# ansonb/RECON

Measured on NVIDIA B200. Metric: SpKBGAT fwd+bwd edges/sec, higher is better.
Workload: dtype f32

## Files before the change

### include/spkbgat.h

```cpp
#ifndef SPKBGAT_H
#define SPKBGAT_H
#include <stdint.h>

#ifdef __cplusplus
extern "C" {
#endif

typedef void* spk_stream_t;

#define SPK_ABI_VERSION 6
int spk_abi_version(void);
const char* spk_last_error(void);
int64_t spk_launch_count(void);

typedef struct {
    int32_t n_heads;
    int32_t d_head;
    int32_t d_pad;
    int32_t width;
} spk_geom;

typedef struct {
    const int32_t* task_seg;
    const int32_t* task_beg;
    const int32_t* task_end;
    const int32_t* hub_seg;
    const int32_t* hub_task_ptr;
    float* partial;
    int64_t ldpart;
    int32_t n_tasks;
    int32_t n_hubs;
    int32_t hub_thresh;
    int32_t reserved;
    const int32_t* task_order;
} spk_hub_tasks;

int spk_edges_concat(const int64_t* edge , int64_t e1, const int64_t* edge_type ,
                     const int64_t* nhop , int64_t e2,
                     int32_t* row, int32_t* col, int32_t* t1, int32_t* t2 ,
                     int64_t n_nodes, int64_t n_rel, int32_t* err_flag, spk_stream_t stream);
int spk_pack_index_host(const int64_t* src, int64_t n, int64_t stride, int64_t lo, int64_t hi, int32_t* dst, int32_t n_threads);
int spk_iota_i32(int32_t* v, int64_t n, spk_stream_t stream);
int64_t spk_sort_workspace_bytes(int64_t n);
int spk_sort_pairs(int32_t* keys, int32_t* vals, int32_t* keys_tmp, int32_t* vals_tmp, int64_t n, int32_t key_bits,
                   void* workspace, int32_t* result_in_tmp, spk_stream_t stream);
int spk_segment_ptr(const int32_t* sorted_keys, int64_t n, int32_t n_seg, int32_t* ptr , spk_stream_t stream);
int spk_gather_i32(const int32_t* src, const int32_t* idx, int64_t n, int32_t* out, spk_stream_t stream);
int spk_rel_incidence(const int32_t* t1, const int32_t* t2, int64_t e, int32_t n_rel, int32_t* keys, int32_t* vals,
                      spk_stream_t stream);

int spk_gemm_nn(const float* A, int64_t lda, const float* B, int64_t ldb, float* C, int64_t ldc,
                int64_t M, int32_t N, int32_t K, int32_t accumulate, spk_stream_t stream);
int64_t spk_gemm_tn_workspace_floats(int64_t M, int32_t Ka, int32_t Nb);
int spk_gemm_tn(const float* A, int64_t lda, const float* B, int64_t ldb, float* C, int64_t ldc,
                int64_t M, int32_t Ka, int32_t Nb, int32_t accumulate, float* workspace, spk_stream_t stream);

int32_t spk_gemm_nn_tc_supported(const float* A, int64_t lda, int64_t M, int32_t N, int32_t K);
int64_t spk_gemm_tc_workspace_floats(int32_t N, int32_t K);
int spk_gemm_nn_tc(const float* A, int64_t lda, const float* B, int64_t ldb, float* C, int64_t ldc,
                   int64_t M, int32_t N, int32_t K, int32_t accumulate, float* workspace, spk_stream_t stream);

int spk_gemm_nn_tc_act(const float* A, int64_t lda, const float* B, int64_t ldb, float* C, int64_t ldc,
                       int64_t M, int32_t N, int32_t K, int32_t accumulate, int32_t act, float* workspace,
                       spk_stream_t stream);
int spk_elu_inplace(float* x, int64_t ldx, int64_t n_rows, int32_t width, spk_stream_t stream);

int32_t spk_gemm_tn_tc_supported(const float* A, int64_t lda, const float* B, int64_t ldb, int64_t M, int32_t Ka, int32_t Nb);
int64_t spk_gemm_tn_tc_workspace_floats(int64_t M, int32_t Ka, int32_t Nb);
int spk_gemm_tn_tc(const float* A, int64_t lda, const float* B, int64_t ldb, float* C, int64_t ldc,
                   int64_t M, int32_t Ka, int32_t Nb, int32_t accumulate, float* workspace, spk_stream_t stream);

typedef struct {
    const int32_t* segptr; const int32_t* col; const int32_t* t1; const int32_t* t2;
    const float* P1; int64_t ld1;
    const float* P2; int64_t ld2;
    const float* P3; int64_t ld3;
    const float* mask; int64_t mask_stride;
    float* out; int64_t ldo;
    float* den; float* sw;
    int32_t* nanflag;
    int32_t n_rows; int32_t apply_elu; float alpha;
    int32_t elu_rows;
    spk_geom geom;
    spk_hub_tasks hub;
} spk_edge_fwd_args;
int spk_edge_attn_fwd(const spk_edge_fwd_args* args, spk_stream_t stream);

typedef struct {
    const int32_t* segptr; const int32_t* col; const int32_t* t1; const int32_t* t2;
    const float* P1; int64_t ld1;
    const float* P2; int64_t ld2;
    const float* P3; int64_t ld3;
    const float* mask; int64_t mask_stride;
    const float* out; const float* dout; int64_t ldo;
    const float* den;
    float* G; int64_t ldg;
    float* dP1; int64_t ldd1;
    float* rec;
    int32_t n_rows; int32_t apply_elu; float alpha; int32_t reserved;
    spk_geom geom;
    spk_hub_tasks hub;
} spk_edge_bwd_rows_args;
int spk_edge_attn_bwd_rows(const spk_edge_bwd_rows_args* args, spk_stream_t stream);

typedef struct {
    const int32_t* segptr; const int32_t* src; const int32_t* pos;
    const float* G; int64_t ldg;
    const float* rec;
    float* out; int64_t ldout;
    int32_t n_seg;
    int32_t flags;
    spk_geom geom;
    spk_hub_tasks hub;
} spk_seg_gather_args;
int spk_edge_attn_bwd_segments(const spk_seg_gather_args* args, spk_stream_t stream);

typedef struct {
    const int32_t* rowptr;
    const int32_t* colptr; const int32_t* csc_row; const int32_t* csc_pos; const int32_t* csc_t1; const int32_t* csc_t2;
    const float* P1; int64_t ld1;
    const float* P2; int64_t ld2;
    const float* P3; int64_t ld3;
    const float* mask; int64_t mask_stride;
    const float* out; const float* dout; int64_t ldo;
    const float* den; const float* sw;
    float* G; int64_t ldg;
    float* rowsc;
    float* dP1; int64_t ldd1;
    float* dP2; int64_t ldd2;
    float* rec;
    int32_t n_rows; int32_t n_cols; int32_t apply_elu; float alpha;
    spk_geom geom;
    spk_hub_tasks row_hub;
    spk_hub_tasks col_hub;
} spk_edge_bwd_fused_args;
int spk_edge_attn_bwd_fused(const spk_edge_bwd_fused_args* args, spk_stream_t stream);

typedef struct {
    spk_edge_bwd_fused_args base;
    const int32_t* relptr; const int32_t* rel_row; const int32_t* rel_pos;
    float* rec4; float* dsv;
    float* dP3; int64_t ldd3;
    int32_t n_rel; int32_t phases;
    spk_hub_tasks rel_hub;
    float* colsum; int64_t ld_colsum;
    float* rowsum; int64_t ld_rowsum;
    const float* G_rel; int64_t ldg_rel;
// ... 152 lines not shown
```

### recon_b200/_lib.py

```python
import ctypes as C
import os

import torch

_HERE = os.path.dirname(os.path.abspath(__file__))
LIB_PATH = os.environ.get("SPK_LIB") or os.path.join(_HERE, "libspkbgat.so")

c_i32p = C.POINTER(C.c_int32)
c_i64p = C.POINTER(C.c_int64)
c_f32p = C.POINTER(C.c_float)
ABI_VERSION = 6


class Geom(C.Structure):
    _fields_ = [("n_heads", C.c_int32), ("d_head", C.c_int32), ("d_pad", C.c_int32), ("width", C.c_int32)]


class HubTasks(C.Structure):
    _fields_ = [("task_seg", C.c_void_p), ("task_beg", C.c_void_p), ("task_end", C.c_void_p),
                ("hub_seg", C.c_void_p), ("hub_task_ptr", C.c_void_p),
                ("partial", C.c_void_p), ("ldpart", C.c_int64),
                ("n_tasks", C.c_int32), ("n_hubs", C.c_int32), ("hub_thresh", C.c_int32), ("reserved", C.c_int32),
                ("task_order", C.c_void_p)]

# ... 59 lines not shown
                ("dup", C.c_int32), ("reserved", C.c_int32)]


class AggGeom(C.Structure):
    _fields_ = [("n_heads", C.c_int32), ("f_chunks", C.c_int32), ("r_chunks", C.c_int32), ("lz", C.c_int32)]


class AggFwdArgs(C.Structure):
    _fields_ = [("segptr", C.c_void_p), ("col", C.c_void_p), ("t1", C.c_void_p), ("t2", C.c_void_p),
                ("xrow", C.c_void_p), ("ldxr", C.c_int64), ("xcol", C.c_void_p), ("ldxc", C.c_int64),
                ("rel", C.c_void_p), ("ldr", C.c_int64),
                ("mask", C.c_void_p), ("mask_stride", C.c_int64),
                ("z", C.c_void_p), ("ldz", C.c_int64), ("den", C.c_void_p), ("sw", C.c_void_p),
                ("nanflag", C.c_void_p),
                ("n_rows", C.c_int32), ("alpha", C.c_float),
                ("geom", AggGeom), ("hub", HubTasks)]


class AggBwdArgs(C.Structure):
    _fields_ = [("segptr", C.c_void_p), ("col", C.c_void_p), ("t1", C.c_void_p), ("t2", C.c_void_p),
                ("xrow", C.c_void_p), ("ldxr", C.c_int64), ("xcol", C.c_void_p), ("ldxc", C.c_int64),
                ("rel", C.c_void_p), ("ldr", C.c_int64),
                ("mask", C.c_void_p), ("mask_stride", C.c_int64),
                ("dz", C.c_void_p), ("ldz", C.c_int64),
                ("den", C.c_void_p), ("sw", C.c_void_p), ("dden", C.c_void_p),
                ("gx", C.c_void_p), ("ldgx", C.c_int64), ("gr", C.c_void_p), ("ldgr", C.c_int64),
                ("rowout", C.c_void_p), ("ldro", C.c_int64), ("rowsc", C.c_void_p), ("rec", C.c_void_p),
                ("n_rows", C.c_int32), ("alpha", C.c_float),
                ("geom", AggGeom), ("hub", HubTasks)]


_VP, _I64, _I32 = C.c_void_p, C.c_int64, C.c_int32

ALLOC_FN = C.CFUNCTYPE(C.c_void_p, C.c_void_p, C.c_int64)


class TripleGraphArgs(C.Structure):
    _fields_ = [("uptr", C.c_void_p), ("ut", C.c_void_p), ("ur0", C.c_void_p), ("ugs", C.c_void_p), ("uge", C.c_void_p),
                ("rs", C.c_void_p), ("n_nodes", C.c_int32), ("n_pairs", C.c_int32), ("n_triples", C.c_int32),
                ("reserved", C.c_int32)]


class NhopResult(C.Structure):
    _fields_ = [("adj_idx", C.c_void_p), ("adj_val", C.c_void_p), ("nhop", C.c_void_p), ("e1", C.c_int64), ("e2", C.c_int64)]


class LossBwdArgs(C.Structure):
    _fields_ = [("segptr", C.c_void_p), ("inc", C.c_void_p), ("coef", C.c_void_p), ("sgn", C.c_void_p),
                ("gscale", C.c_void_p), ("out", C.c_void_p), ("ldo", C.c_int64),
                ("n_seg", C.c_int32), ("width", C.c_int32), ("mode", C.c_int32), ("reserved", C.c_int32),
                ("hub", HubTasks)]


class SgdArgs(C.Structure):
    _fields_ = [("param", C.c_void_p * 16), ("grad", C.c_void_p * 16), ("numel", C.c_int64 * 16),
                ("count", C.c_int32), ("lr", C.c_float)]


class AttnWeightsArgs(C.Structure):
    _fields_ = [("a", C.c_void_p * 4), ("a2", C.c_void_p * 4), ("da", C.c_void_p * 4), ("da2", C.c_void_p * 4),
                ("n_heads", C.c_int32), ("F", C.c_int32), ("Rd", C.c_int32), ("D", C.c_int32),
                ("mode", C.c_int32), ("d_pad", C.c_int32), ("width", C.c_int32),
                ("f_pad", C.c_int32), ("lz", C.c_int32), ("reserved", C.c_int32),
                ("W0", C.c_void_p), ("ld0", C.c_int64), ("W1", C.c_void_p), ("ld1", C.c_int64), ("W2", C.c_void_p)]


SIGNATURES = {
    "spk_abi_version": (_I32, []),
    "spk_last_error": (C.c_char_p, []),
    "spk_launch_count": (_I64, []),
    "spk_edges_concat": (_I32, [_VP, _I64, _VP, _VP, _I64, _VP, _VP, _VP, _VP, _I64, _I64, _VP, _VP]),
    "spk_pack_index_host": (_I32, [_VP, _I64, _I64, _I64, _I64, _VP, _I32]),
    "spk_iota_i32": (_I32, [_VP, _I64, _VP]),
    "spk_sort_workspace_bytes": (_I64, [_I64]),
    "spk_sort_pairs": (_I32, [_VP, _VP, _VP, _VP, _I64, _I32, _VP, C.POINTER(_I32), _VP]),
    "spk_segment_ptr": (_I32, [_VP, _I64, _I32, _VP, _VP]),
    "spk_gather_i32": (_I32, [_VP, _VP, _I64, _VP, _VP]),
    "spk_rel_incidence": (_I32, [_VP, _VP, _I64, _I32, _VP, _VP, _VP]),
    "spk_gemm_nn": (_I32, [_VP, _I64, _VP, _I64, _VP, _I64, _I64, _I32, _I32, _I32, _VP]),
    "spk_gemm_nn_tc_supported": (_I32, [_VP, _I64, _I64, _I32, _I32]),
    "spk_gemm_tc_workspace_floats": (_I64, [_I32, _I32]),
    "spk_gemm_nn_tc": (_I32, [_VP, _I64, _VP, _I64, _VP, _I64, _I64, _I32, _I32, _I32, _VP, _VP]),
    "spk_gemm_nn_tc_act": (_I32, [_VP, _I64, _VP, _I64, _VP, _I64, _I64, _I32, _I32, _I32, _I32, _VP, _VP]),
    "spk_elu_inplace": (_I32, [_VP, _I64, _I64, _I32, _VP]),
    "spk_agg_table": (_I32, [_VP, _I64, _VP, _VP, _I64, _I64, _I32, _I32, _VP]),
    "spk_agg_fwd": (_I32, [C.POINTER(AggFwdArgs), _VP]),
    "spk_agg_bwd_pre": (_I32, [_VP, _VP, _I64, _VP, _I32, _I32, _I32, _VP, _I64, _VP, _I64, _VP]),
    "spk_agg_bwd_rows": (_I32, [C.POINTER(AggBwdArgs), _VP]),
    "spk_agg_bwd_ctx": (_I32, [C.POINTER(AggBwdArgs), _VP]),
    "spk_agg_dx": (_I32, [_VP, _I64, _VP, _I64, _VP, _I64, _I32, _I32, _I32, _VP, _I64, _VP, _VP]),
    "spk_gemm_tn_tc_supported": (_I32, [_VP, _I64, _VP, _I64, _I64, _I32, _I32]),
    "spk_gemm_tn_tc_workspace_floats": (_I64, [_I64, _I32, _I32]),
    "spk_gemm_tn_tc": (_I32, [_VP, _I64, _VP, _I64, _VP, _I64, _I64, _I32, _I32, _I32, _VP, _VP]),
    "spk_gemm_tn_workspace_floats": (_I64, [_I64, _I32, _I32]),
    "spk_gemm_tn": (_I32, [_VP, _I64, _VP, _I64, _VP, _I64, _I64, _I32, _I32, _I32, _VP, _VP]),
    "spk_edge_attn_fwd": (_I32, [C.POINTER(EdgeFwdArgs), _VP]),
    "spk_edge_attn_bwd_rows": (_I32, [C.POINTER(EdgeBwdRowsArgs), _VP]),
    "spk_edge_attn_bwd_segments": (_I32, [C.POINTER(SegGatherArgs), _VP]),
    "spk_edge_attn_bwd_fused": (_I32, [C.POINTER(EdgeBwdFusedArgs), _VP]),
    "spk_edge_attn_bwd_split": (_I32, [C.POINTER(EdgeBwdSplitArgs), _VP]),
    "spk_spmm_rowsum_fwd": (_I32, [_VP, _VP, _VP, _I64, _I32, _VP, _I64, _I32, _VP]),
    "spk_spmm_rowsum_bwd": (_I32, [_VP, _VP, _I64, _I32, _VP, _I64, _I64, _VP]),
    "spk_rownorm": (_I32, [_VP, _I64, _VP, _I64, _I64, _I32, _VP]),
    "spk_residual_norm_fwd": (_I32, [_VP, _I64, _VP, _I64, _VP, _VP, _I64, _VP, _I64, _I32, _VP]),
    "spk_residual_norm_bwd": (_I32, [_VP, _I64, _VP, _I64, _VP, _VP, _VP, _I64, _VP, _I64, _I64, _I32, _VP]),
    "spk_mask_from_index": (_I32, [_VP, _I64, _VP, _I64, _VP, _VP]),
    "spk_attn_weights_fwd": (_I32, [_VP, _VP]),
    "spk_attn_weights_bwd": (_I32, [_VP, _VP]),
    "spk_inner_product_workspace_bytes": (_I64, []),
    "spk_inner_product": (_I32, [_VP, _VP, _I64, _VP, _VP, _I32, _VP]),
    "spk_margin_loss_partials": (_I64, [_I64]),
    "spk_margin_loss_fwd": (_I32, [_VP, _I64, _I64, _VP, _I64, _I64, _VP, _I64, _I64, _I32, C.c_float, _I32,
                                   _VP, _VP, _VP, _VP, _VP, _VP, _VP]),
    "spk_triple_incidence": (_I32, [_VP, _I64, _I64, _I64, _VP, _VP, _VP, _VP, _VP, _VP]),
    "spk_margin_loss_bwd": (_I32, [C.POINTER(LossBwdArgs), _VP]),
    "spk_sgd_step": (_I32, [C.POINTER(SgdArgs), _VP]),
    "spk_triple_keys": (_I32, [_VP, _I64, _I64, _I64, _VP, _VP, _VP]),
    "spk_corrupt_triples": (_I32, [_VP, _I64, _I32, _VP, _I64, _I64, _I64, _VP, _VP, C.c_uint64, _VP, _VP, _VP]),
    "spk_nhop_build": (_I32, [C.POINTER(TripleGraphArgs), _VP, _I64, _I32, ALLOC_FN, _VP, C.POINTER(NhopResult), _VP]),
    "spk_gather_concat": (_I32, [_VP, _VP, _VP, _VP, _VP, _I32, _I64, _I32, _VP, _I64, _VP, _VP]),
    "spk_mlp_head_fwd": (_I32, [_VP, _I64, _VP, _VP, _VP, C.c_float, _I64, _I32, _VP, _VP]),
    "spk_mlp_head_bwd": (_I32, [_VP, _I64, _VP, _VP, C.c_float, _VP, _I64, _I32, _VP, _I64, _VP, _I64, _VP]),
    "spk_tanh_fwd": (_I32, [_VP, _I64, _I64, _I32, _VP]),
    "spk_tanh_bwd": (_I32, [_VP, _I64, _VP, _I64, _I64, _I32, _VP, _I64, _VP]),
    "spk_rank_scores": (_I32, [_VP, _I64, _VP, _I64, _VP, _VP, C.c_float, _I64, _I32, _I32, _VP, _I64, _VP]),
    "spk_linkpred_count": (_I32, [_VP, _I64, _I64, _VP, _I64, _I64, _VP, _VP, C.c_float, _I32, _VP, _VP, _I64, _I32,
                                  _VP, _I64, _VP, _VP, _VP, _VP, _VP]),
    "spk_linkpred_filter": (_I32, [_VP, _I64, _I64, _I64, _VP, C.c_float, _I32, _VP, _I64, _I32, _VP, _I64, _VP, _VP,
                                   _VP, _I64, _VP, _VP, _VP, _VP]),
    "spk_export_json": (_I32, [_VP, _I64, _I64, _I64, C.c_char_p, _I32]),
    "spk_export_bin": (_I32, [_VP, _I64, _I64, _I64, C.c_char_p]),
    "spk_import_json_shape": (_I32, [C.c_char_p, C.POINTER(_I64), C.POINTER(_I64)]),
    "spk_import_json": (_I32, [C.c_char_p, _VP, _I64, _I64, _I64, _I32]),
}

_lib = None
current_tag = ""


class _Lib:

    def __init__(self, cdll):
        self._cdll = cdll
        self.timing = None

    def __getattr__(self, name):
        fn = getattr(self._cdll, name)
        if self.timing is None or SIGNATURES[name][1][-1:] != [_VP] or "workspace" in name or "supported" in name:
            return fn

        def timed(*args):
            e0 = torch.cuda.Event(enable_timing=True)
            e1 = torch.cuda.Event(enable_timing=True)
            e0.record()
            rc = fn(*args)
            e1.record()
            global current_tag
            self.timing.append((name[4:] + (":" + current_tag if current_tag else ""), e0, e1))
            if "gemm" in name:
                current_tag = ""
            return rc
        return timed


def load():
    global _lib
# ... 38 lines not shown
```

### recon_b200/csrc/spk_agg.cu

```cuda
#include <stdlib.h>
#include "spk_agg.cuh"
#include "spk_stream.cuh"

namespace spk {
namespace {

constexpr unsigned FULL = 0xffffffffu;

__device__ __forceinline__ float agg_exp(float x) { return exp2f(x * 1.4426950408889634f); }
__device__ __forceinline__ float4 f4scale(float4 v, float s) { return make_float4(v.x * s, v.y * s, v.z * s, v.w * s); }
__device__ __forceinline__ bool f4nan(float4 v) { return (v.x != v.x) | (v.y != v.y) | (v.z != v.z) | (v.w != v.w); }
__device__ __forceinline__ void st4(float* p, float4 v) { *reinterpret_cast<float4*>(p) = v; }

__global__ void __launch_bounds__(256)
agg_table_kernel(const float* __restrict__ X, long ldx, const float* __restrict__ V, float* __restrict__ T, long ldt,
                 long n, int F, int F4) {
    const int lane = threadIdx.x & 31;
    const long row = (long)blockIdx.x * 8 + (threadIdx.x >> 5);
    if (row >= n) return;
    const float* x = X + row * ldx;
    float xv[2];
    float q[4] = {0.f, 0.f, 0.f, 0.f};
#pragma unroll
    for (int r = 0; r < 2; ++r) {
// ... 768 lines not shown
            for (int u = 0; u < G; ++u) {
                const int n = n0 + u;
                float4 v = make_float4(0.f, 0.f, 0.f, 0.f);
                if (n < T) {
                    const uint32_t slot = wbase + (uint32_t)(grp * G + u) * slot_bytes;
                    if (active) v = lds4(slot + loff);
                    if (HAS2) {
                        const int k2 = __shfl_sync(FULL, cur.t2, n - nb);
                        if (active && !isx && k2 >= 0) v = f4add(v, lds4(slot + loff + rbr));
                    }
                }
#pragma unroll
                for (int h = 0; h < HT; ++h) pd[u * HT + h] = f4dot(Y[h], v);
                if (!TASKS && n + 1 == row_end && rn >= 0) {
#pragma unroll
                    for (int h = 0; h < HT; ++h) Y[h] = Yn[h];
                    r = rn;
                    row_end = __shfl_sync(FULL, st.pre + st.deg, r);
                    rn = -1;
                    if (act) { rn = __ffs(act) - 1; act &= act - 1; load_y(rn, Yn); }
                }
            }
            const float tot = transposed_warp_sum<NV>(pd, lane);
            const bool mine = (lane >> 3) == ((n0 - nb) >> 3);
#pragma unroll
            for (int h = 0; h < HT; ++h) {
                const float t = __shfl_sync(FULL, tot, (((lane & 7) * HT + h) * 32) / NV);
                if (mine) tt[h] = t;
            }
            __syncwarp();
            if (n0 + S < T)
                ags_issue_group<HT, HAS2, G, NG>(a.Xcol, a.ldxc, a.Rt, a.ldr, rbx, rbr, slot_bytes, wbase, bars, T, nb, n0 + S, lane, cur, b1);
        }
        batch_epilogue();
    }
    if (TASKS) {
        const int task = blockIdx.x * AGS_WARPS + wid;
        if (lane == 0) {
            float* part = a.hub.partial + (long)task * a.hub.ldpart;
#pragma unroll
            for (int h = 0; h < 4; ++h) part[h] = h < HT ? usum[h < HT ? h : 0] : 0.f;
        }
    } else if (row_valid) {
        st4(a.rowout + (row0 + lane) * a.ldro + 4 * a.g.Fx4, make_float4(usum[0], HT > 1 ? usum[HT - 1] : 0.f, 0.f, 0.f));
    }
}

__global__ void __launch_bounds__(SPK_CTA_THREADS)
agg_bwd_hub_finalize_kernel(const AggBwdArgs a) {
    __shared__ float red[SPK_WARPS_PER_CTA][8];
    const int hub = blockIdx.x;
    const int row = __ldg(a.hub.hub_seg + hub);
    const int t0 = __ldg(a.hub.hub_task_ptr + hub), t1 = __ldg(a.hub.hub_task_ptr + hub + 1);
    cta_sum_partials<1>(a.hub.partial, a.hub.ldpart, t0, t1, 4, &red[0][0], 8);
    if (threadIdx.x == 0)
        st4(a.rowout + (long)row * a.ldro + 4 * a.g.Fx4, make_float4(red[0][0], red[0][1], 0.f, 0.f));
}

template <int HT, bool HAS2>
int launch_agg_bwd_t(const AggBwdArgs& a, cudaStream_t s) {
    constexpr int G = 8, NG = 2;
    const uint32_t rbx = (uint32_t)(a.g.Fx4 + 1) * 16u, rbr = (uint32_t)(a.g.Fr4 + 1) * 16u;
    const size_t smem = (size_t)AGS_WARPS * ags_warp_bytes_c<HAS2, G, NG>(rbx, rbr);
    static SmemLimit lim_rows, lim_tasks;
    if (a.n_rows > 0) {
        agg_bwd_ctx_kernel<false><<<(a.n_rows + SPK_WARPS_PER_CTA - 1) / SPK_WARPS_PER_CTA, SPK_CTA_THREADS, 0, s>>>(a);
        if (int rc = check_launch("agg_bwd_ctx")) return rc;
        lim_rows.ensure(agg_bwd_stream_kernel<HT, HAS2, false>, smem);
        const unsigned grid = (unsigned)((a.n_rows + 32L * AGS_WARPS - 1) / (32L * AGS_WARPS));
        agg_bwd_stream_kernel<HT, HAS2, false><<<grid, AGS_WARPS * 32, smem, s>>>(a);
        if (int rc = check_launch("agg_bwd_stream_rows")) return rc;
    }
    if (a.hub.n_tasks > 0) {
        lim_tasks.ensure(agg_bwd_stream_kernel<HT, HAS2, true>, smem);
        const unsigned grid = (a.hub.n_tasks + AGS_WARPS - 1) / AGS_WARPS;
        agg_bwd_stream_kernel<HT, HAS2, true><<<grid, AGS_WARPS * 32, smem, s>>>(a);
        if (int rc = check_launch("agg_bwd_stream_tasks")) return rc;
        agg_bwd_hub_finalize_kernel<<<a.hub.n_hubs, SPK_CTA_THREADS, 0, s>>>(a);
        if (int rc = check_launch("agg_bwd_hub_finalize")) return rc;
    }
    return 0;
}

__device__ __forceinline__ void bwd_pre_elem(float ov, float gv, int apply_elu, float& dh, float& p) {
    float hv = ov;
    dh = gv;
    if (apply_elu) {
        const bool pos = ov > 0.f;
        dh = pos ? gv : gv * (ov + 1.f);
        hv = pos ? ov : (ov > -1.f ? fast_log1p(ov) : 0.f);
    }
    p = fmaf(dh, hv, p);
}

__global__ void __launch_bounds__(256)
agg_bwd_pre_vec_kernel(const float* __restrict__ out, const float* __restrict__ dout, long ldo, const float* __restrict__ den,
                       int H, int D4, int apply_elu, float* __restrict__ dhn, long ldd, float* __restrict__ dden, long n) {
    const int lane = threadIdx.x & 31;
    const long row = (long)blockIdx.x * 8 + (threadIdx.x >> 5);
    if (row >= n) return;
    const float* o = out + row * ldo;
    const float* g = dout + row * ldo;
    float* d = dhn + row * ldd;
    const int n4 = H * D4;
    float p[4] = {0.f, 0.f, 0.f, 0.f};
    for (int c4 = lane; c4 < n4; c4 += 32) {
        const float4 ov = ldg4_stream(o + c4 * 4), gv = ldg4_stream(g + c4 * 4);
        float4 dh;
        float acc = 0.f;
        bwd_pre_elem(ov.x, gv.x, apply_elu, dh.x, acc);
        bwd_pre_elem(ov.y, gv.y, apply_elu, dh.y, acc);
        bwd_pre_elem(ov.z, gv.z, apply_elu, dh.z, acc);
        bwd_pre_elem(ov.w, gv.w, apply_elu, dh.w, acc);
        st4(d + c4 * 4, dh);
        const int h = c4 / D4;
#pragma unroll
        for (int k = 0; k < 4; ++k) p[k] += (h == k) ? acc : 0.f;
    }
#pragma unroll
    for (int k = 0; k < 4; ++k) {
        if (k >= H) break;
        const float t = warp_sum(p[k]);
        if (lane == 0) dden[row * H + k] = -t / __ldg(den + row * H + k);
    }
}

__global__ void __launch_bounds__(256)
agg_bwd_pre_kernel(const float* __restrict__ out, const float* __restrict__ dout, long ldo, const float* __restrict__ den,
                   int H, int D, int apply_elu, float* __restrict__ dhn, long ldd, float* __restrict__ dden, long n) {
    const int lane = threadIdx.x & 31;
    const long row = (long)blockIdx.x * 8 + (threadIdx.x >> 5);
    if (row >= n) return;
    const float* o = out + row * ldo;
    const float* g = dout + row * ldo;
    float* d = dhn + row * ldd;
    for (int h = 0; h < H; ++h) {
        float p = 0.f;
        for (int c = lane; c < D; c += 32) {
            float dh;
            bwd_pre_elem(__ldg(o + h * D + c), __ldg(g + h * D + c), apply_elu, dh, p);
            d[h * D + c] = dh;
        }
        p = warp_sum(p);
        if (lane == 0) dden[row * H + h] = -p / __ldg(den + row * H + h);
    }
}

constexpr int DX_R = 2;
__global__ void __launch_bounds__(256)
agg_dx_kernel(const float* __restrict__ rowout, long ldro, const float* __restrict__ dxc, long ldc,
              const float* __restrict__ V, long n, int F, int F4, int H, float* __restrict__ dX, long lddx,
              float* __restrict__ dq) {
    const int lane = threadIdx.x & 31;
    const long i0 = ((long)blockIdx.x * 8 + (threadIdx.x >> 5)) * DX_R;
    float q[DX_R][4], r0[DX_R][2], c0[DX_R][2], c1[DX_R][2];
    float4 v[2];
#pragma unroll
    for (int k = 0; k < 2; ++k) v[k] = (lane + 32 * k < F) ? ldg4(V + (lane + 32 * k) * 4) : make_float4(0.f, 0.f, 0.f, 0.f);
#pragma unroll
    for (int r = 0; r < DX_R; ++r) {
        const long i = i0 + r < n ? i0 + r : n - 1;
        const float* ro = rowout + i * ldro;
        const float* xc = dxc + i * ldc;
        q[r][0] = __ldg(xc + H * 4 * F4); q[r][1] = H > 1 ? __ldg(xc + H * 4 * F4 + 1) : 0.f;
        q[r][2] = __ldg(ro + 4 * F4); q[r][3] = H > 1 ? __ldg(ro + 4 * F4 + 1) : 0.f;
#pragma unroll
        for (int k = 0; k < 2; ++k) {
            const int f = lane + 32 * k;
            r0[r][k] = f < F ? __ldg(ro + f) : 0.f;
            c0[r][k] = f < F ? __ldg(xc + f) : 0.f;
            c1[r][k] = (f < F && H > 1) ? __ldg(xc + 4 * F4 + f) : 0.f;
        }
    }
#pragma unroll
    for (int r = 0; r < DX_R; ++r) {
        const long i = i0 + r;
// ... 85 lines not shown
```

### recon_b200/csrc/spk_api.cu

```cuda
#include "../../include/spkbgat.h"
#include "spk_common.cuh"
#include "spk_edge.cuh"
#include "spk_edge_bwd_fused.cuh"
#include "spk_agg.cuh"
#include "spk_gemm.cuh"
#include "spk_graph.cuh"
#include "spk_rowops.cuh"

namespace spk {

static thread_local char g_err[512] = "";
static unsigned long long g_launches = 0;

void set_error(const char* fmt, ...) {
    va_list ap;
    va_start(ap, fmt);
    vsnprintf(g_err, sizeof(g_err), fmt, ap);
    va_end(ap);
}

int check_launch(const char* what) {
    const cudaError_t e = cudaGetLastError();
    __atomic_fetch_add(&g_launches, 1ULL, __ATOMIC_RELAXED);
    if (e == cudaSuccess) return 0;
// ... 44 lines not shown
        for (int e = beg; e < end; ++e) s += w[(long)perm[e] * ldw + c];
        out[(long)row * ldo + c] = s;
    }
}

__global__ void spmm_rowsum_bwd_kernel(const long long* __restrict__ edge_row, const float* __restrict__ g, long ldg,
                                       int width, float* __restrict__ gw, long ldw, long n_edges) {
    const long i = (long)blockIdx.x * blockDim.x + threadIdx.x;
    if (i >= n_edges * width) return;
    const long e = i / width; const int c = (int)(i % width);
    gw[e * ldw + c] = g[(long)edge_row[e] * ldg + c];
}

}

using namespace spk;

extern "C" {

int spk_abi_version(void) { return SPK_ABI_VERSION; }
const char* spk_last_error(void) { return g_err; }
int64_t spk_launch_count(void) { return (int64_t)__atomic_load_n(&g_launches, __ATOMIC_RELAXED); }

int spk_edges_concat(const int64_t* edge, int64_t e1, const int64_t* edge_type, const int64_t* nhop, int64_t e2,
                     int32_t* row, int32_t* col, int32_t* t1, int32_t* t2, int64_t n_nodes, int64_t n_rel,
                     int32_t* err_flag, spk_stream_t stream) {
    if (e1 + e2 >= (1LL << 31) || n_nodes >= (1LL << 31)) { set_error("edges_concat: sizes exceed int32"); return 1; }
    if (e2 > 0 && !t2) { set_error("edges_concat: t2 required when 2-hop rows are given"); return 1; }
    return edges_concat(reinterpret_cast<const long long*>(edge), e1, reinterpret_cast<const long long*>(edge_type),
                        reinterpret_cast<const long long*>(nhop), e2, row, col, t1, t2, n_nodes, n_rel, err_flag,
                        (cudaStream_t)stream);
}
int spk_iota_i32(int32_t* v, int64_t n, spk_stream_t stream) { return iota_i32(v, n, (cudaStream_t)stream); }
int64_t spk_sort_workspace_bytes(int64_t n) { return radix_sort_workspace_bytes(n); }
int spk_sort_pairs(int32_t* keys, int32_t* vals, int32_t* keys_tmp, int32_t* vals_tmp, int64_t n, int32_t key_bits,
                   void* workspace, int32_t* result_in_tmp, spk_stream_t stream) {
    if (key_bits < 1 || key_bits > 31) { set_error("sort_pairs: key_bits %d out of range", key_bits); return 1; }
    return radix_sort_pairs(keys, vals, keys_tmp, vals_tmp, n, key_bits, workspace, result_in_tmp, (cudaStream_t)stream);
}
int spk_segment_ptr(const int32_t* sorted_keys, int64_t n, int32_t n_seg, int32_t* ptr, spk_stream_t stream) {
    return segment_ptr(sorted_keys, n, n_seg, ptr, (cudaStream_t)stream);
}
int spk_gather_i32(const int32_t* src, const int32_t* idx, int64_t n, int32_t* out, spk_stream_t stream) {
    return gather_i32(src, idx, n, out, (cudaStream_t)stream);
}
int spk_rel_incidence(const int32_t* t1, const int32_t* t2, int64_t e, int32_t n_rel, int32_t* keys, int32_t* vals,
                      spk_stream_t stream) {
    return rel_incidence(t1, t2, e, n_rel, keys, vals, (cudaStream_t)stream);
}

int spk_gemm_nn(const float* A, int64_t lda, const float* B, int64_t ldb, float* C, int64_t ldc,
                int64_t M, int32_t N, int32_t K, int32_t accumulate, spk_stream_t stream) {
    if (lda < K || ldb < N || ldc < N) { set_error("gemm_nn: leading dimension too small"); return 1; }
    return gemm_nn_simt(A, lda, B, ldb, C, ldc, M, N, K, accumulate, (cudaStream_t)stream);
}
int64_t spk_gemm_tn_workspace_floats(int64_t M, int32_t Ka, int32_t Nb) { return gemm_tn_workspace_floats(M, Ka, Nb); }
int spk_gemm_tn(const float* A, int64_t lda, const float* B, int64_t ldb, float* C, int64_t ldc,
                int64_t M, int32_t Ka, int32_t Nb, int32_t accumulate, float* workspace, spk_stream_t stream) {
    if (lda < Ka || ldb < Nb || ldc < Nb) { set_error("gemm_tn: leading dimension too small"); return 1; }
    if (!workspace) { set_error("gemm_tn: workspace required"); return 1; }
    return gemm_tn_simt(A, lda, B, ldb, C, ldc, M, Ka, Nb, accumulate, workspace, (cudaStream_t)stream);
}

int32_t spk_gemm_nn_tc_supported(const float* A, int64_t lda, int64_t M, int32_t N, int32_t K) {
    return gemm_nn_tc_supported(A, lda, M, N, K);
}
int64_t spk_gemm_tc_workspace_floats(int32_t N, int32_t K) { return 2LL * N * gemm_tc_ldt(K); }
int spk_gemm_nn_tc(const float* A, int64_t lda, const float* B, int64_t ldb, float* C, int64_t ldc,
                   int64_t M, int32_t N, int32_t K, int32_t accumulate, float* workspace, spk_stream_t stream) {
    if (lda < K || ldb < N || ldc < N) { set_error("gemm_nn_tc: leading dimension too small"); return 1; }
    if (!gemm_nn_tc_supported(A, lda, M, N, K)) { set_error("gemm_nn_tc: A must be 16-byte aligned with lda %% 4 == 0"); return 1; }
    if (!workspace || (reinterpret_cast<uintptr_t>(workspace) & 15)) { set_error("gemm_nn_tc: aligned workspace required"); return 1; }
    return gemm_nn_tc(A, lda, B, ldb, C, ldc, M, N, K, accumulate, workspace, (cudaStream_t)stream);
}

int spk_gemm_nn_tc_act(const float* A, int64_t lda, const float* B, int64_t ldb, float* C, int64_t ldc,
                       int64_t M, int32_t N, int32_t K, int32_t accumulate, int32_t act, float* workspace, spk_stream_t stream) {
    if (lda < K || ldb < N || ldc < N) { set_error("gemm_nn_tc_act: leading dimension too small"); return 1; }
    if (!gemm_nn_tc_supported(A, lda, M, N, K)) { set_error("gemm_nn_tc_act: A must be 16-byte aligned with lda %% 4 == 0"); return 1; }
    if (!workspace || (reinterpret_cast<uintptr_t>(workspace) & 15)) { set_error("gemm_nn_tc_act: aligned workspace required"); return 1; }
    if (act < 0 || act > 2) { set_error("gemm_nn_tc_act: unknown activation %d", act); return 1; }
    return gemm_nn_tc(A, lda, B, ldb, C, ldc, M, N, K, accumulate, workspace, (cudaStream_t)stream, act);
}
int spk_elu_inplace(float* x, int64_t ldx, int64_t n_rows, int32_t width, spk_stream_t stream) {
    if (ldx < width) { set_error("elu_inplace: leading dimension too small"); return 1; }
    return launch_elu_inplace(x, ldx, n_rows, width, (cudaStream_t)stream);
}

int32_t spk_gemm_tn_tc_supported(const float* A, int64_t lda, const float* B, int64_t ldb, int64_t M, int32_t Ka, int32_t Nb) {
    return gemm_tn_tc_supported(A, lda, B, ldb, M, Ka, Nb);
}
int64_t spk_gemm_tn_tc_workspace_floats(int64_t M, int32_t Ka, int32_t Nb) { return gemm_tn_tc_workspace_floats(M, Ka, Nb); }
int spk_gemm_tn_tc(const float* A, int64_t lda, const float* B, int64_t ldb, float* C, int64_t ldc,
                   int64_t M, int32_t Ka, int32_t Nb, int32_t accumulate, float* workspace, spk_stream_t stream) {
    if (ldc < Nb) { set_error("gemm_tn_tc: leading dimension too small"); return 1; }
    if (!gemm_tn_tc_supported(A, lda, B, ldb, M, Ka, Nb)) { set_error("gemm_tn_tc: operands must be 16-byte aligned with ld %% 4 == 0"); return 1; }
    if (!workspace) { set_error("gemm_tn_tc: workspace required"); return 1; }
    return gemm_tn_tc(A, lda, B, ldb, C, ldc, M, Ka, Nb, accumulate, workspace, (cudaStream_t)stream);
}

int spk_edge_attn_fwd(const spk_edge_fwd_args* p, spk_stream_t stream) {
    EdgeFwdArgs a;
    if (!geom_ok(p->geom, &a.g, "edge_attn_fwd")) return 1;
    if ((p->ld1 & 3) || (p->ld2 & 3) || (p->ld3 & 3) || p->ld1 < p->geom.width || p->ld2 < p->geom.width ||
        p->ld3 < p->geom.width || !aligned16(p->P1) || !aligned16(p->P2) || !aligned16(p->P3)) {
        set_error("edge_attn_fwd: projected tables must be 16-byte aligned with ld >= width, ld %% 4 == 0");
        return 1;
    }
    a.segptr = p->segptr; a.col = p->col; a.t1 = p->t1; a.t2 = p->t2;
    a.P1 = p->P1; a.ld1 = p->ld1; a.P2 = p->P2; a.ld2 = p->ld2; a.P3 = p->P3; a.ld3 = p->ld3;
    a.mask = p->mask; a.mask_stride = p->mask_stride;
    a.out = p->out; a.ldo = p->ldo; a.den = p->den; a.sw = p->sw; a.nanflag = p->nanflag;
    a.n_rows = p->n_rows; a.alpha = p->alpha; a.apply_elu = p->apply_elu;
    a.elu_rows = p->elu_rows > 0 ? p->elu_rows : 0x7fffffff;
    a.out_vec = (p->geom.d_head % 4 == 0) && (p->ldo % 4 == 0) && aligned16(p->out);
    a.hub = hub_of(p->hub);
    if (a.hub.n_tasks > 0 && (a.hub.ldpart < p->geom.width + 2 * SPK_MAX_HEADS || (a.hub.ldpart & 3) || !aligned16(a.hub.partial))) {
        set_error("edge_attn_fwd: hub partial buffer needs ldpart >= width+8, ldpart %% 4 == 0");
        return 1;
    }
    return launch_edge_fwd(a, (cudaStream_t)stream);
}

int spk_edge_attn_bwd_rows(const spk_edge_bwd_rows_args* p, spk_stream_t stream) {
    EdgeBwdRowsArgs a;
    if (!geom_ok(p->geom, &a.g, "edge_attn_bwd_rows")) return 1;
    if ((p->ld1 & 3) || (p->ld2 & 3) || (p->ld3 & 3) || (p->ldg & 3) || (p->ldd1 & 3) || p->ldg < p->geom.n_heads * p->geom.d_pad ||
        p->ldd1 < p->geom.width || !aligned16(p->P1) || !aligned16(p->P2) || !aligned16(p->P3) || !aligned16(p->G) ||
        !aligned16(p->dP1) || (reinterpret_cast<uintptr_t>(p->rec) & 7)) {
        set_error("edge_attn_bwd_rows: bad leading dimension or alignment");
        return 1;
    }
    a.segptr = p->segptr; a.col = p->col; a.t1 = p->t1; a.t2 = p->t2;
    a.P1 = p->P1; a.ld1 = p->ld1; a.P2 = p->P2; a.ld2 = p->ld2; a.P3 = p->P3; a.ld3 = p->ld3;
    a.mask = p->mask; a.mask_stride = p->mask_stride;
    a.out = p->out; a.dout = p->dout; a.ldo = p->ldo; a.den = p->den;
    a.G = p->G; a.ldg = p->ldg; a.dP1 = p->dP1; a.ldd1 = p->ldd1; a.rec = p->rec;
    a.n_rows = p->n_rows; a.alpha = p->alpha; a.apply_elu = p->apply_elu;
    a.out_vec = (p->geom.d_head % 4 == 0) && (p->ldo % 4 == 0) && aligned16(p->out) && aligned16(p->dout);
    a.hub = hub_of(p->hub);
    if (a.hub.n_tasks > 0 && a.hub.ldpart < 2 * SPK_MAX_HEADS) { set_error("edge_attn_bwd_rows: hub ldpart must be >= 8"); return 1; }
    return launch_edge_bwd_rows(a, (cudaStream_t)stream);
}

int spk_edge_attn_bwd_segments(const spk_seg_gather_args* p, spk_stream_t stream) {
    SegGatherArgs a;
    if (!geom_ok(p->geom, &a.g, "edge_attn_bwd_segments")) return 1;
    if ((p->ldg & 3) || (p->ldout & 3) || p->ldout < p->geom.width || p->ldg < p->geom.n_heads * p->geom.d_pad ||
        !aligned16(p->G) || !aligned16(p->out) || (reinterpret_cast<uintptr_t>(p->rec) & 7)) {
        set_error("edge_attn_bwd_segments: bad leading dimension or alignment");
        return 1;
    }
    a.segptr = p->segptr; a.src = p->src; a.pos = p->pos; a.G = p->G; a.ldg = p->ldg; a.rec = p->rec;
    a.outp = p->out; a.ldout = p->ldout; a.n_seg = p->n_seg; a.prefer_stream = p->flags & 1;
    a.hub = hub_of(p->hub);
    if (a.hub.n_tasks > 0 && (a.hub.ldpart < p->geom.width || (a.hub.ldpart & 3) || !aligned16(a.hub.partial))) {
        set_error("edge_attn_bwd_segments: hub partial buffer needs ldpart >= width");
        return 1;
    }
    return launch_seg_gather(a, (cudaStream_t)stream);
}

static int fused_args_of(const spk_edge_bwd_fused_args* p, BwdFusedArgs& a, const char* who, int dup = 0);

int spk_edge_attn_bwd_fused(const spk_edge_bwd_fused_args* p, spk_stream_t stream) {
    BwdFusedArgs a;
// ... 246 lines not shown
```

### recon_b200/csrc/spk_common.cuh

```cuda
#pragma once
#include <cuda_runtime.h>
#include <stdint.h>
#include <stdio.h>
#include <stdarg.h>

#define SPK_MAX_HEADS 4
#define SPK_WARPS_PER_CTA 8
#define SPK_CTA_THREADS (SPK_WARPS_PER_CTA * 32)

namespace spk {

void set_error(const char* fmt, ...);
int check_launch(const char* what);

struct SmemLimit {
    size_t set[64] = {};
    template <class K>
    cudaError_t ensure(K kernel, size_t bytes) {
        int dev = 0;
        const bool keyed = cudaGetDevice(&dev) == cudaSuccess && dev >= 0 && dev < 64;
        if (keyed && set[dev] >= bytes) return cudaSuccess;
        const cudaError_t e = cudaFuncSetAttribute(kernel, cudaFuncAttributeMaxDynamicSharedMemorySize, (int)bytes);
        if (e == cudaSuccess && keyed) set[dev] = bytes;
        return e;
    }
};

__device__ __forceinline__ float warp_sum(float v) {
#pragma unroll
    for (int o = 16; o > 0; o >>= 1) v += __shfl_xor_sync(0xffffffffu, v, o);
    return v;
}

template <int N>
__device__ __forceinline__ float transposed_warp_sum(float (&p)[N], int lane) {
    int off = 16;
#pragma unroll
    for (int n = N; n > 1; n >>= 1, off >>= 1) {
        const bool up = (lane & off) != 0;
        const int half = n >> 1;
#pragma unroll
        for (int k = 0; k < half; ++k) {
            const float keep = up ? p[k + half] : p[k];
            const float send = up ? p[k] : p[k + half];
            p[k] = keep + __shfl_xor_sync(0xffffffffu, send, off);
        }
    }
    float r = p[0];
    for (; off > 0; off >>= 1) r += __shfl_xor_sync(0xffffffffu, r, off);
    return r;
}

__device__ __forceinline__ float fast_log1p(float x) {
    const float u = 1.0f + x;
    const float d = u - 1.0f;
    return d == 0.f ? x : __logf(u) * __fdividef(x, d);
}

__device__ __forceinline__ float4 ldg4(const float* p) {
    return __ldg(reinterpret_cast<const float4*>(p));
}
__device__ __forceinline__ float4 ldg4_stream(const float* p) {
    float4 r;
    asm volatile("ld.global.nc.L1::no_allocate.v4.f32 {%0,%1,%2,%3}, [%4];"
                 : "=f"(r.x), "=f"(r.y), "=f"(r.z), "=f"(r.w) : "l"(p));
    return r;
}
__device__ __forceinline__ float4 f4add(float4 a, float4 b) {
    return make_float4(a.x + b.x, a.y + b.y, a.z + b.z, a.w + b.w);
}
__device__ __forceinline__ void f4fma(float4& acc, float w, float4 v) {
    acc.x = fmaf(w, v.x, acc.x); acc.y = fmaf(w, v.y, acc.y);
    acc.z = fmaf(w, v.z, acc.z); acc.w = fmaf(w, v.w, acc.w);
}
__device__ __forceinline__ float f4dot(float4 a, float4 b) {
    return fmaf(a.x, b.x, fmaf(a.y, b.y, fmaf(a.z, b.z, a.w * b.w)));
}
__device__ __forceinline__ float f4get(const float4& v, int k) {
    return k == 0 ? v.x : (k == 1 ? v.y : (k == 2 ? v.z : v.w));
}
__device__ __forceinline__ float sel4(int h, float a, float b, float c, float d) {
    return h == 0 ? a : (h == 1 ? b : (h == 2 ? c : d));
}

template <int HT>
__device__ __forceinline__ float selh(int h, const float (&v)[HT]) {
    float r = v[0];
#pragma unroll
    for (int i = 1; i < HT; ++i) r = (h == i) ? v[i] : r;
    return r;
}

template <int NREG, int NW = SPK_WARPS_PER_CTA>
__device__ __forceinline__ void cta_sum_partials(const float* __restrict__ part, long ld, int t0, int t1, int len,
                                                 float* red, int red_ld) {
    const int lane = threadIdx.x & 31, wid = threadIdx.x >> 5;
    float acc[NREG];
#pragma unroll
    for (int k = 0; k < NREG; ++k) acc[k] = 0.f;
    int t = t0 + wid;
    for (; t + 3 * NW < t1; t += 4 * NW) {
        float v[4][NREG];
#pragma unroll
        for (int u = 0; u < 4; ++u)
#pragma unroll
            for (int k = 0; k < NREG; ++k) {
                const int c = lane + 32 * k;
                v[u][k] = c < len ? part[(long)(t + u * NW) * ld + c] : 0.f;
            }
#pragma unroll
        for (int u = 0; u < 4; ++u)
#pragma unroll
            for (int k = 0; k < NREG; ++k) acc[k] += v[u][k];
    }
    for (; t < t1; t += NW) {
#pragma unroll
        for (int k = 0; k < NREG; ++k) {
            const int c = lane + 32 * k;
            if (c < len) acc[k] += part[(long)t * ld + c];
        }
    }
#pragma unroll
    for (int k = 0; k < NREG; ++k) {
        const int c = lane + 32 * k;
        if (c < len) red[wid * red_ld + c] = acc[k];
    }
    __syncthreads();
    for (int c = threadIdx.x; c < len; c += (NW * 32)) {
        float s = 0.f;
#pragma unroll
        for (int w = 0; w < NW; ++w) s += red[w * red_ld + c];
        red[c] = s;
    }
    __syncthreads();
}

struct LayerGeom {
    int H;
    int D;
// ... 7 lines not shown
```

### recon_b200/csrc/spk_gemm.cuh

```cuda
#pragma once
#include <cuda_runtime.h>

namespace spk {
int gemm_nn_simt(const float* A, long lda, const float* B, long ldb, float* C, long ldc,
                 long M, int N, int K, int accumulate, cudaStream_t s);
int gemm_tn_splits(long M, int Ka, int Nb);
long gemm_tn_workspace_floats(long M, int Ka, int Nb);
int gemm_tn_simt(const float* A, long lda, const float* B, long ldb, float* C, long ldc,
                 long M, int Ka, int Nb, int accumulate, float* workspace, cudaStream_t s);
}

namespace spk {
int gemm_tc_ldt(int K);
int gemm_nn_tc_supported(const float* A, long lda, long M, int N, int K);
int gemm_nn_tc(const float* A, long lda, const float* B, long ldb, float* C, long ldc, long M, int N, int K,
               int accumulate, float* workspace, cudaStream_t s, int act = 0);
int gemm_tn_tc_supported(const float* A, long lda, const float* B, long ldb, long M, int Ka, int Nb);
long gemm_tn_tc_workspace_floats(long M, int Ka, int Nb);
int gemm_tn_tc(const float* A, long lda, const float* B, long ldb, float* C, long ldc, long M, int Ka, int Nb,
               int accumulate, float* workspace, cudaStream_t s);
}
```

### recon_b200/csrc/spk_gemm_tc.cu

```cuda
#include <cuda.h>
#include <stdlib.h>
#include "spk_common.cuh"
#include "spk_gemm.cuh"

namespace spk {
namespace {

constexpr int TC_BM = 128;
constexpr int TC_BK = 32;
constexpr int TC_A_TILE = TC_BM * TC_BK * 4;
constexpr int TC_THREADS = 320;
constexpr int TC_MAX_STAGES = 4;

__device__ __forceinline__ uint32_t smem_u32(const void* p) { return (uint32_t)__cvta_generic_to_shared(p); }

__device__ __forceinline__ void mbar_init(uint32_t bar, uint32_t count) {
    asm volatile("mbarrier.init.shared::cta.b64 [%0], %1;" ::"r"(bar), "r"(count) : "memory");
}
__device__ __forceinline__ void mbar_arrive(uint32_t bar) {
    asm volatile("mbarrier.arrive.shared::cta.b64 _, [%0];" ::"r"(bar) : "memory");
}
__device__ __forceinline__ void mbar_arrive_expect_tx(uint32_t bar, uint32_t bytes) {
    asm volatile("mbarrier.arrive.expect_tx.shared::cta.b64 _, [%0], %1;" ::"r"(bar), "r"(bytes) : "memory");
}
__device__ __forceinline__ void mbar_wait(uint32_t bar, uint32_t parity) {
    asm volatile(
        "{\n\t"
        ".reg .pred P1;\n\t"
        "LAB_WAIT:\n\t"
        "mbarrier.try_wait.parity.shared::cta.b64 P1, [%0], %1;\n\t"
        "@P1 bra DONE;\n\t"
        "bra LAB_WAIT;\n\t"
        "DONE:\n\t"
        "}" ::"r"(bar), "r"(parity) : "memory");
}
__device__ __forceinline__ void tma_load_2d(uint32_t dst, const CUtensorMap* tm, uint32_t bar, int c0, int c1) {
    asm volatile(
        "cp.async.bulk.tensor.2d.shared::cluster.global.mbarrier::complete_tx::bytes [%0], [%1, {%3, %4}], [%2];"
        ::"r"(dst), "l"(tm), "r"(bar), "r"(c0), "r"(c1) : "memory");
}
__device__ __forceinline__ void tma_load_2d_mc(uint32_t dst, const CUtensorMap* tm, uint32_t bar, int c0, int c1, uint16_t mask) {
    asm volatile(
        "cp.async.bulk.tensor.2d.shared::cluster.global.mbarrier::complete_tx::bytes.multicast::cluster [%0], [%1, {%3, %4}], [%2], %5;"
        ::"r"(dst), "l"(tm), "r"(bar), "r"(c0), "r"(c1), "h"(mask) : "memory");
}
__device__ __forceinline__ uint32_t cluster_ctarank() {
    uint32_t r;
    asm volatile("mov.u32 %0, %%cluster_ctarank;" : "=r"(r));
    return r;
}
__device__ __forceinline__ void cluster_sync_all() {
    asm volatile("barrier.cluster.arrive.release.aligned;" ::: "memory");
    asm volatile("barrier.cluster.wait.acquire.aligned;" ::: "memory");
}
__device__ __forceinline__ void tc_fence_before() { asm volatile("tcgen05.fence::before_thread_sync;" ::: "memory"); }
__device__ __forceinline__ void tc_fence_after() { asm volatile("tcgen05.fence::after_thread_sync;" ::: "memory"); }
__device__ __forceinline__ void tc_commit(uint32_t bar) {
    asm volatile("tcgen05.commit.cta_group::1.mbarrier::arrive::one.shared::cluster.b64 [%0];" ::"r"(bar) : "memory");
}
__device__ __forceinline__ void tc_commit_mc(uint32_t bar, uint16_t mask) {
    asm volatile("tcgen05.commit.cta_group::1.mbarrier::arrive::one.shared::cluster.multicast::cluster.b64 [%0], %1;"
                 ::"r"(bar), "h"(mask) : "memory");
}
__device__ __forceinline__ void tc_mma_tf32(uint32_t d_tmem, uint64_t adesc, uint64_t bdesc, uint32_t idesc, uint32_t accum) {
    asm volatile(
        "{\n\t"
        ".reg .pred p;\n\t"
        "setp.ne.b32 p, %4, 0;\n\t"
        "tcgen05.mma.cta_group::1.kind::tf32 [%0], %1, %2, %3, p;\n\t"
        "}" ::"r"(d_tmem), "l"(adesc), "l"(bdesc), "r"(idesc), "r"(accum) : "memory");
}
__device__ __forceinline__ uint64_t make_kmajor_sw128_desc(uint32_t saddr) {
    const uint32_t lo = ((saddr >> 4) & 0x3fffu) | (1u << 16);
    const uint32_t hi = (1024u >> 4) | (1u << 14) | (2u << 29);
    return ((uint64_t)hi << 32) | lo;
}

struct TcParams {
    float* C; long ldc; long M; int N; int K; int BN; int n_tiles_n; int stages; int accumulate; int c_vec;
    int act;
    int c_tma;
    int raw_hi;
    int cs;
};

__device__ __forceinline__ float tc_elu(float x) {
    const float big = exp2f(x * 1.4426950408889634f) - 1.0f;
    const float small = x * (1.0f + x * (0.5f + x * (0.16666667f + x * (0.041666668f + x * 0.0083333338f))));
    const float neg = x > -0.125f ? small : big;
    return x > 0.f ? x : neg;
}

__device__ __forceinline__ float tc_act(float x, int act) { return act == 2 ? tanhf(x) : tc_elu(x); }

__global__ void __launch_bounds__(TC_THREADS, 1)
gemm_nn_tc_kernel(const __grid_constant__ CUtensorMap tmA, const __grid_constant__ CUtensorMap tmBhi,
                  const __grid_constant__ CUtensorMap tmBlo, const __grid_constant__ CUtensorMap tmC, const TcParams p) {
    extern __shared__ uint8_t smem_raw[];
    __shared__ __align__(8) uint64_t bars[3 * TC_MAX_STAGES + 4];
    __shared__ uint32_t tmem_slot;

    const int warp = threadIdx.x >> 5, lane = threadIdx.x & 31;
    const uint32_t base = (smem_u32(smem_raw) + 1023u) & ~1023u;
    const uint32_t b_tile = (uint32_t)p.BN * 128u;
    const uint32_t stage_bytes = 2u * TC_A_TILE + 2u * b_tile;
    auto a_hi = [&](int s) { return base + (uint32_t)s * stage_bytes; };
    auto a_lo = [&](int s) { return base + (uint32_t)s * stage_bytes + TC_A_TILE; };
    auto b_hi = [&](int s) { return base + (uint32_t)s * stage_bytes + 2u * TC_A_TILE; };
    auto b_lo = [&](int s) { return base + (uint32_t)s * stage_bytes + 2u * TC_A_TILE + b_tile; };
    const uint32_t bar0 = smem_u32(bars);
    auto full = [&](int s) { return bar0 + 8u * s; };
    auto conv = [&](int s) { return bar0 + 8u * (TC_MAX_STAGES + s); };
    auto empty = [&](int s) { return bar0 + 8u * (2 * TC_MAX_STAGES + s); };
    auto tfull = [&](int a) { return bar0 + 8u * (3 * TC_MAX_STAGES + a); };
    auto tempty = [&](int a) { return bar0 + 8u * (3 * TC_MAX_STAGES + 2 + a); };

    const int num_kb = (p.K + TC_BK - 1) / TC_BK;
    const long m_tiles = (p.M + TC_BM - 1) / TC_BM;
    const int cs = p.cs;
    const uint32_t crank = cs > 1 ? cluster_ctarank() : 0u;
    const uint16_t cmask = (uint16_t)((1u << cs) - 1u);
    const long total = ((m_tiles + cs - 1) / cs) * p.n_tiles_n;
    const long first = blockIdx.x / cs, stride = gridDim.x / cs;
    const uint32_t b_slice = b_tile / (uint32_t)cs;
    const int b_rows = p.BN / cs;

    if (threadIdx.x == 0) {
        asm volatile("prefetch.tensormap [%0];" ::"l"(&tmA) : "memory");
        asm volatile("prefetch.tensormap [%0];" ::"l"(&tmBhi) : "memory");
        asm volatile("prefetch.tensormap [%0];" ::"l"(&tmBlo) : "memory");
        for (int s = 0; s < TC_MAX_STAGES; ++s) { mbar_init(full(s), 1); mbar_init(conv(s), 128); mbar_init(empty(s), (uint32_t)cs); }
        for (int a = 0; a < 2; ++a) { mbar_init(tfull(a), 1); mbar_init(tempty(a), 4); }
        asm volatile("fence.mbarrier_init.release.cluster;" ::: "memory");
    }
    if (warp == 1) {
        asm volatile("tcgen05.alloc.cta_group::1.sync.aligned.shared::cta.b32 [%0], %1;" ::"r"(smem_u32(&tmem_slot)), "r"(512u) : "memory");
        asm volatile("tcgen05.relinquish_alloc_permit.cta_group::1.sync.aligned;" ::: "memory");
    }
    tc_fence_before();
    __syncthreads();
    if (cs > 1) cluster_sync_all();
    tc_fence_after();
    const uint32_t tmem_base = tmem_slot;

    if (warp == 0) {
        if (lane == 0) {
            uint32_t it = 0;
            for (long tile = first; tile < total; tile += stride) {
                const int m0 = (int)((tile / p.n_tiles_n) * cs + crank) * TC_BM, n0 = (int)(tile % p.n_tiles_n) * p.BN;
                for (int kb = 0; kb < num_kb; ++kb, ++it) {
                    const int s = it % p.stages;
                    const uint32_t ph = (it / p.stages) & 1u;
                    mbar_wait(empty(s), ph ^ 1u);
                    mbar_arrive_expect_tx(full(s), TC_A_TILE + 2u * b_tile);
                    tma_load_2d(a_hi(s), &tmA, full(s), kb * TC_BK, m0);
                    if (cs == 1) {
                        tma_load_2d(b_hi(s), &tmBhi, full(s), kb * TC_BK, n0);
                        tma_load_2d(b_lo(s), &tmBlo, full(s), kb * TC_BK, n0);
                    } else {
                        tma_load_2d_mc(b_hi(s) + crank * b_slice, &tmBhi, full(s), kb * TC_BK, n0 + (int)crank * b_rows, cmask);
                        tma_load_2d_mc(b_lo(s) + crank * b_slice, &tmBlo, full(s), kb * TC_BK, n0 + (int)crank * b_rows, cmask);
                    }
                }
            }
        }
    } else if (warp == 1) {
        if (lane == 0) {
            const uint32_t idesc = (1u << 4) | (2u << 7) | (2u << 10) | ((uint32_t)(p.BN >> 3) << 17) | ((uint32_t)(TC_BM >> 4) << 24);
            uint32_t it = 0, tl = 0;
            for (long tile = first; tile < total; tile += stride, ++tl) {
                const uint32_t acc = tl & 1u, aph = (tl >> 1) & 1u;
                mbar_wait(tempty(acc), aph ^ 1u);
                tc_fence_after();
                const uint32_t d_tmem = tmem_base + acc * 256u;
                for (int kb = 0; kb < num_kb; ++kb, ++it) {
                    const int s = it % p.stages;
                    const uint32_t ph = (it / p.stages) & 1u;
                    mbar_wait(full(s), ph);
                    mbar_wait(conv(s), ph);
                    tc_fence_after();
                    const uint64_t dah = make_kmajor_sw128_desc(a_hi(s)), dal = make_kmajor_sw128_desc(a_lo(s));
                    const uint64_t dbh = make_kmajor_sw128_desc(b_hi(s)), dbl = make_kmajor_sw128_desc(b_lo(s));
#pragma unroll
                    for (int ks = 0; ks < TC_BK / 8; ++ks) {
                        if (kb * TC_BK + ks * 8 >= p.K) break;
                        const uint64_t o = (uint64_t)(2 * ks);
                        tc_mma_tf32(d_tmem, dal + o, dbh + o, idesc, (kb | ks) != 0);
                        tc_mma_tf32(d_tmem, dah + o, dbl + o, idesc, 1u);
                        tc_mma_tf32(d_tmem, dah + o, dbh + o, idesc, 1u);
                    }
                    if (cs == 1) tc_commit(empty(s));
                    else tc_commit_mc(empty(s), cmask);
                }
                tc_commit(tfull(acc));
            }
        }
    } else if (warp < 6) {
        const int t = threadIdx.x - 64;
        uint32_t it = 0;
        for (long tile = first; tile < total; tile += stride) {
            for (int kb = 0; kb < num_kb; ++kb, ++it) {
                const int s = it % p.stages;
                const uint32_t ph = (it / p.stages) & 1u;
                mbar_wait(full(s), ph);
                const uint32_t hi0 = a_hi(s), lo0 = a_lo(s);
#pragma unroll
                for (int i = 0; i < TC_A_TILE / 16 / 128; ++i) {
                    const uint32_t off = (uint32_t)(t + 128 * i) * 16u;
                    float4 x;
                    asm volatile("ld.shared.v4.f32 {%0,%1,%2,%3}, [%4];" : "=f"(x.x), "=f"(x.y), "=f"(x.z), "=f"(x.w) : "r"(hi0 + off));
                    float4 h, l;
                    h.x = __uint_as_float(__float_as_uint(x.x) & 0xffffe000u); l.x = x.x - h.x;
                    h.y = __uint_as_float(__float_as_uint(x.y) & 0xffffe000u); l.y = x.y - h.y;
                    h.z = __uint_as_float(__float_as_uint(x.z) & 0xffffe000u); l.z = x.z - h.z;
                    h.w = __uint_as_float(__float_as_uint(x.w) & 0xffffe000u); l.w = x.w - h.w;
                    if (!p.raw_hi)
                        asm volatile("st.shared.v4.f32 [%0], {%1,%2,%3,%4};" ::"r"(hi0 + off), "f"(h.x), "f"(h.y), "f"(h.z), "f"(h.w) : "memory");
                    asm volatile("st.shared.v4.f32 [%0], {%1,%2,%3,%4};" ::"r"(lo0 + off), "f"(l.x), "f"(l.y), "f"(l.z), "f"(l.w) : "memory");
                }
                asm volatile("fence.proxy.async.shared::cta;" ::: "memory");
                mbar_arrive(conv(s));
            }
        }
    } else if (p.c_tma) {
        const int q = warp & 3;
        const uint32_t stg0 = base + (uint32_t)p.stages * stage_bytes + (uint32_t)q * 8192u;
        uint32_t tl = 0, sb = 0;
        for (long tile = first; tile < total; tile += stride, ++tl) {
            const uint32_t acc = tl & 1u, aph = (tl >> 1) & 1u;
            const int row0 = (int)((tile / p.n_tiles_n) * cs + crank) * TC_BM + q * 32;
            const int n0 = (int)(tile % p.n_tiles_n) * p.BN;
            mbar_wait(tfull(acc), aph);
            tc_fence_after();
            for (int c0 = 0; c0 < p.BN && row0 < p.M; c0 += 32) {
                if (n0 + c0 >= p.N) break;
                uint32_t r[32];
                const uint32_t taddr = tmem_base + acc * 256u + (uint32_t)c0 + ((uint32_t)(q * 32) << 16);
                asm volatile(
                    "tcgen05.ld.sync.aligned.32x32b.x32.b32 {%0,%1,%2,%3,%4,%5,%6,%7,%8,%9,%10,%11,%12,%13,%14,%15,"
                    "%16,%17,%18,%19,%20,%21,%22,%23,%24,%25,%26,%27,%28,%29,%30,%31}, [%32];"
                    : "=r"(r[0]), "=r"(r[1]), "=r"(r[2]), "=r"(r[3]), "=r"(r[4]), "=r"(r[5]), "=r"(r[6]), "=r"(r[7]),
                      "=r"(r[8]), "=r"(r[9]), "=r"(r[10]), "=r"(r[11]), "=r"(r[12]), "=r"(r[13]), "=r"(r[14]), "=r"(r[15]),
                      "=r"(r[16]), "=r"(r[17]), "=r"(r[18]), "=r"(r[19]), "=r"(r[20]), "=r"(r[21]), "=r"(r[22]), "=r"(r[23]),
                      "=r"(r[24]), "=r"(r[25]), "=r"(r[26]), "=r"(r[27]), "=r"(r[28]), "=r"(r[29]), "=r"(r[30]), "=r"(r[31])
                    : "r"(taddr));
                asm volatile("tcgen05.wait::ld.sync.aligned;" ::: "memory");
                if (p.act == 2) {
#pragma unroll
                    for (int j = 0; j < 32; ++j) r[j] = __float_as_uint(tanhf(__uint_as_float(r[j])));
                } else if (p.act) {
#pragma unroll
                    for (int j = 0; j < 32; ++j) r[j] = __float_as_uint(tc_elu(__uint_as_float(r[j])));
                }
                if (lane == 0) asm volatile("cp.async.bulk.wait_group.read 1;" ::: "memory");
                __syncwarp();
                const uint32_t stg = stg0 + sb * 4096u;
                const uint32_t rowaddr = stg + (uint32_t)lane * 128u;
#pragma unroll
                for (int j = 0; j < 8; ++j) {
                    const uint32_t a = rowaddr + (uint32_t)((j ^ (lane & 7)) << 4);
                    asm volatile("st.shared.v4.b32 [%0], {%1,%2,%3,%4};" ::"r"(a), "r"(r[4 * j]), "r"(r[4 * j + 1]),
                                 "r"(r[4 * j + 2]), "r"(r[4 * j + 3]) : "memory");
                }
                asm volatile("fence.proxy.async.shared::cta;" ::: "memory");
                __syncwarp();
                if (lane == 0 && row0 < p.M) {
                    if (p.accumulate)
                        asm volatile("cp.reduce.async.bulk.tensor.2d.global.shared::cta.add.tile.bulk_group [%0, {%1, %2}], [%3];"
                                     ::"l"(&tmC), "r"(n0 + c0), "r"(row0), "r"(stg) : "memory");
                    else
                        asm volatile("cp.async.bulk.tensor.2d.global.shared::cta.tile.bulk_group [%0, {%1, %2}], [%3];"
                                     ::"l"(&tmC), "r"(n0 + c0), "r"(row0), "r"(stg) : "memory");
                    asm volatile("cp.async.bulk.commit_group;" ::: "memory");
                }
                sb ^= 1u;
            }
            tc_fence_before();
            __syncwarp();
            if (lane == 0) mbar_arrive(tempty(acc));
        }
        if (lane == 0) asm volatile("cp.async.bulk.wait_group 0;" ::: "memory");
    } else {
        const int q = warp & 3;
        uint32_t tl = 0;
        for (long tile = first; tile < total; tile += stride, ++tl) {
            const uint32_t acc = tl & 1u, aph = (tl >> 1) & 1u;
            const long row = ((tile / p.n_tiles_n) * cs + crank) * TC_BM + q * 32 + lane;
            const int n0 = (int)(tile % p.n_tiles_n) * p.BN;
            mbar_wait(tfull(acc), aph);
            tc_fence_after();
            for (int c0 = 0; c0 < p.BN; c0 += 16) {
                uint32_t r[16];
                const uint32_t taddr = tmem_base + acc * 256u + (uint32_t)c0 + ((uint32_t)(q * 32) << 16);
                asm volatile(
                    "tcgen05.ld.sync.aligned.32x32b.x16.b32 {%0,%1,%2,%3,%4,%5,%6,%7,%8,%9,%10,%11,%12,%13,%14,%15}, [%16];"
                    : "=r"(r[0]), "=r"(r[1]), "=r"(r[2]), "=r"(r[3]), "=r"(r[4]), "=r"(r[5]), "=r"(r[6]), "=r"(r[7]),
                      "=r"(r[8]), "=r"(r[9]), "=r"(r[10]), "=r"(r[11]), "=r"(r[12]), "=r"(r[13]), "=r"(r[14]), "=r"(r[15])
                    : "r"(taddr));
                asm volatile("tcgen05.wait::ld.sync.aligned;" ::: "memory");
                if (row < p.M) {
                    float* crow = p.C + row * p.ldc;
#pragma unroll
                    for (int j = 0; j < 16; j += 4) {
                        const int col = n0 + c0 + j;
                        if (col >= p.N) break;
                        float4 o = make_float4(__uint_as_float(r[j]), __uint_as_float(r[j + 1]), __uint_as_float(r[j + 2]), __uint_as_float(r[j + 3]));
// ... 232 lines not shown
                    asm volatile("cp.async.bulk.commit_group;" ::: "memory");
                }
                sb ^= 1u;
            }
            tc_fence_before();
            __syncwarp();
            if (lane == 0) mbar_arrive_remote(tempty(acc), 0u);
        }
        if (lane == 0) asm volatile("cp.async.bulk.wait_group 0;" ::: "memory");
    }
    tc_fence_before();
    __syncthreads();
    cluster_sync_all();
    if (warp == 1) {
        tc_fence_after();
        asm volatile("tcgen05.dealloc.cta_group::2.sync.aligned.b32 %0, %1;" ::"r"(tmem_base), "r"(512u) : "memory");
    }
}

__global__ void tc_prepare_b_kernel(const float* __restrict__ B, long ldb, int K, int N, float* __restrict__ hi,
                                    float* __restrict__ lo, int ldt) {
    const long i = (long)blockIdx.x * blockDim.x + threadIdx.x;
    if (i >= (long)N * ldt) return;
    const int n = (int)(i / ldt), k = (int)(i % ldt);
    const float x = k < K ? B[(long)k * ldb + n] : 0.f;
    const float h = __uint_as_float(__float_as_uint(x) & 0xffffe000u);
    hi[i] = h;
    lo[i] = x - h;
}

typedef CUresult (*EncodeTiledFn)(CUtensorMap*, CUtensorMapDataType, cuuint32_t, void*, const cuuint64_t*, const cuuint64_t*,
                                  const cuuint32_t*, const cuuint32_t*, CUtensorMapInterleave, CUtensorMapSwizzle,
                                  CUtensorMapL2promotion, CUtensorMapFloatOOBfill);

EncodeTiledFn encode_fn() {
    static EncodeTiledFn fn = nullptr;
    if (!fn) {
        void* p = nullptr;
        cudaDriverEntryPointQueryResult q;
        if (cudaGetDriverEntryPoint("cuTensorMapEncodeTiled", &p, cudaEnableDefault, &q) == cudaSuccess && q == cudaDriverEntryPointSuccess)
            fn = reinterpret_cast<EncodeTiledFn>(p);
    }
    return fn;
}

int make_map(CUtensorMap* tm, const float* ptr, long rows, long cols, long ld, int box_rows,
             CUtensorMapSwizzle swz = CU_TENSOR_MAP_SWIZZLE_128B) {
    EncodeTiledFn fn = encode_fn();
    if (!fn) { set_error("gemm_tc: cuTensorMapEncodeTiled unavailable"); return 3; }
    cuuint64_t dims[2] = {(cuuint64_t)cols, (cuuint64_t)rows};
    cuuint64_t strides[1] = {(cuuint64_t)ld * 4};
    cuuint32_t box[2] = {(cuuint32_t)TC_BK, (cuuint32_t)box_rows};
    cuuint32_t estr[2] = {1, 1};
    const CUresult r = fn(tm, CU_TENSOR_MAP_DATA_TYPE_FLOAT32, 2, const_cast<float*>(ptr), dims, strides, box, estr,
                          CU_TENSOR_MAP_INTERLEAVE_NONE, swz, CU_TENSOR_MAP_L2_PROMOTION_L2_128B,
                          CU_TENSOR_MAP_FLOAT_OOB_FILL_NONE);
    if (r != CUDA_SUCCESS) { set_error("gemm_tc: cuTensorMapEncodeTiled failed (%d)", (int)r); return 3; }
    return 0;
}
}

int gemm_tc_ldt(int K) { return (K + 3) / 4 * 4; }

static int tc_cluster() {
    const char* e = getenv("SPK_TC_CLUSTER");
    return (e && e[0] == '2') ? 2 : 1;
}

static int tc_pair() {
    const char* e = getenv("SPK_TC_PAIR");
    return (e && e[0] == '1') ? 1 : 0;
}

static int tc_raw_hi() {
    static int v = -1;
    if (v < 0) { const char* e = getenv("SPK_TC_RAW_HI"); v = (e && e[0] == '0') ? 0 : 1; }
    return v;
}

int gemm_nn_tc_supported(const float* A, long lda, long M, int N, int K) {
    return M >= 1 && N >= 1 && K >= 1 && (lda % 4 == 0) && ((reinterpret_cast<uintptr_t>(A) & 15) == 0) && lda >= K;
}

int gemm_nn_tc(const float* A, long lda, const float* B, long ldb, float* C, long ldc, long M, int N, int K,
               int accumulate, float* workspace, cudaStream_t s, int act) {
    const int ldt = gemm_tc_ldt(K);
    float* bhi = workspace;
    float* blo = workspace + (long)N * ldt;
    const long nb = (long)N * ldt;
    tc_prepare_b_kernel<<<(unsigned)((nb + 255) / 256), 256, 0, s>>>(B, ldb, K, N, bhi, blo, ldt);
    if (int rc = check_launch("tc_prepare_b")) return rc;

    const int n_tiles_n = (N + 255) / 256;
    const int bn_round = n_tiles_n > 1 ? 32 : 16;
    int BN = ((N + n_tiles_n - 1) / n_tiles_n + bn_round - 1) / bn_round * bn_round;
    if (BN < 16) BN = 16;
    const int b_tile = BN * 128;
    const int stage_bytes = 2 * TC_A_TILE + 2 * b_tile;
    const int c_vec = (ldc % 4 == 0) && ((reinterpret_cast<uintptr_t>(C) & 15) == 0);
    const int c_tma = c_vec && !(act && accumulate);
    const int staging = c_tma ? 4 * 8192 : 0;
    int stages = (225 * 1024 - 1024 - staging) / stage_bytes;
    if (stages > TC_MAX_STAGES) stages = TC_MAX_STAGES;
    if (stages < 1) { set_error("gemm_tc: tile does not fit shared memory"); return 3; }
    const int smem = stages * stage_bytes + staging + 1024;

    int dev = 0, sms = 148;
    cudaGetDevice(&dev);
    cudaDeviceGetAttribute(&sms, cudaDevAttrMultiProcessorCount, dev);
    const long m_tiles = (M + TC_BM - 1) / TC_BM;
    const bool pair = tc_pair() && c_tma && tc_raw_hi() && (BN % 16 == 0) && m_tiles * n_tiles_n >= 2L * sms;
    if (pair) {
        const int half_tile = BN / 2 * 128;
        const int stage2 = 2 * TC_A_TILE + 2 * half_tile;
        int stages2 = (225 * 1024 - 1024 - staging) / stage2;
        if (stages2 > TC_MAX_STAGES) stages2 = TC_MAX_STAGES;
        const int smem2 = stages2 * stage2 + staging + 1024;
        CUtensorMap tA, tBh, tBl, tC;
        if (int rc = make_map(&tA, A, M, K, lda, TC_BM)) return rc;
        if (int rc = make_map(&tBh, bhi, N, K, ldt, BN / 2)) return rc;
        if (int rc = make_map(&tBl, blo, N, K, ldt, BN / 2)) return rc;
        if (int rc = make_map(&tC, C, M, N, ldc, 32)) return rc;
        TcParams q;
        q.C = C; q.ldc = ldc; q.M = M; q.N = N; q.K = K; q.BN = BN; q.n_tiles_n = n_tiles_n; q.stages = stages2;
        q.accumulate = accumulate; q.act = act; q.c_vec = c_vec; q.c_tma = 1; q.raw_hi = 1; q.cs = 2;
        static SmemLimit lim2;
        if (lim2.ensure(gemm_nn_tc2_kernel, 226 * 1024) != cudaSuccess) {
            set_error("gemm_tc: cannot raise dynamic shared memory limit");
            (void)cudaGetLastError();
            return 3;
        }
        cudaLaunchConfig_t cfg = {};
        cfg.gridDim = dim3((unsigned)sms / 2 * 2); cfg.blockDim = dim3(TC_THREADS); cfg.dynamicSmemBytes = (size_t)smem2; cfg.stream = s;
        cudaLaunchAttribute attr[1];
        attr[0].id = cudaLaunchAttributeClusterDimension;
        attr[0].val.clusterDim.x = 2; attr[0].val.clusterDim.y = 1; attr[0].val.clusterDim.z = 1;
        cfg.attrs = attr; cfg.numAttrs = 1;
        static int pairs_resident[64] = {};
        int nc = (dev >= 0 && dev < 64) ? pairs_resident[dev] : 0;
        if (nc == 0) {
            if (cudaOccupancyMaxActiveClusters(&nc, gemm_nn_tc2_kernel, &cfg) != cudaSuccess || nc < 1) { (void)cudaGetLastError(); nc = sms / 4; }
            if (dev >= 0 && dev < 64) pairs_resident[dev] = nc;
        }
        const long pair_tiles = ((m_tiles + 1) / 2) * n_tiles_n;
        const long np = pair_tiles < nc ? pair_tiles : nc;
        cfg.gridDim = dim3((unsigned)(2 * np));
        (void)cudaLaunchKernelEx(&cfg, gemm_nn_tc2_kernel, tA, tBh, tBl, tC, q);
        return check_launch("gemm_nn_tc2");
    }
    const int cs = (tc_cluster() == 2 && !accumulate && m_tiles * n_tiles_n >= 2L * sms) ? 2 : 1;

    CUtensorMap tmA, tmBhi, tmBlo, tmC;
    if (int rc = make_map(&tmA, A, M, K, lda, TC_BM)) return rc;
    if (int rc = make_map(&tmBhi, bhi, N, K, ldt, BN / cs)) return rc;
    if (int rc = make_map(&tmBlo, blo, N, K, ldt, BN / cs)) return rc;
    if (c_tma) { if (int rc = make_map(&tmC, C, M, N, ldc, 32)) return rc; }
    else tmC = tmA;

    TcParams p;
    p.C = C; p.ldc = ldc; p.M = M; p.N = N; p.K = K; p.BN = BN; p.n_tiles_n = n_tiles_n; p.stages = stages;
    p.accumulate = accumulate; p.act = act;
    p.c_vec = c_vec; p.c_tma = c_tma; p.raw_hi = tc_raw_hi(); p.cs = cs;
    static SmemLimit lim;
    if (lim.ensure(gemm_nn_tc_kernel, 226 * 1024) != cudaSuccess) {
        set_error("gemm_tc: cannot raise dynamic shared memory limit");
        (void)cudaGetLastError();
        return 3;
    }
    const long total = ((m_tiles + cs - 1) / cs) * n_tiles_n * cs;
    cudaLaunchConfig_t cfg = {};
    cfg.gridDim = dim3((unsigned)sms / cs * cs); cfg.blockDim = dim3(TC_THREADS); cfg.dynamicSmemBytes = (size_t)smem; cfg.stream = s;
    cudaLaunchAttribute attr[1];
    attr[0].id = cudaLaunchAttributeClusterDimension;
    attr[0].val.clusterDim.x = (unsigned)cs; attr[0].val.clusterDim.y = 1; attr[0].val.clusterDim.z = 1;
    cfg.attrs = attr; cfg.numAttrs = 1;
    long resident = sms;
    if (cs > 1) {
        static int clusters[64] = {};
        int nc = (dev >= 0 && dev < 64) ? clusters[dev] : 0;
        if (nc == 0) {
            if (cudaOccupancyMaxActiveClusters(&nc, gemm_nn_tc_kernel, &cfg) != cudaSuccess || nc < 1) { (void)cudaGetLastError(); nc = sms / cs / 2; }
            if (dev >= 0 && dev < 64) clusters[dev] = nc;
        }
        resident = (long)nc * cs;
    }
    unsigned grid = (unsigned)(total < resident ? total : resident);
    grid = grid / cs * cs;
    if (grid < (unsigned)cs) grid = (unsigned)cs;
    cfg.gridDim = dim3(grid);
    (void)cudaLaunchKernelEx(&cfg, gemm_nn_tc_kernel, tmA, tmBhi, tmBlo, tmC, p);
    return check_launch("gemm_nn_tc");
}


namespace {

constexpr int TN_BKM = 32;
constexpr int TN_CHUNK = TN_BKM * 128;
constexpr int TN_ACH = 4;

__device__ __forceinline__ uint64_t make_mnmajor_sw128_desc(uint32_t saddr) {
    const uint32_t lo = ((saddr >> 4) & 0x3fffu) | ((uint32_t)(TN_CHUNK >> 4) << 16);
    const uint32_t hi = (512u >> 4) | (1u << 14) | (1u << 29);
    return ((uint64_t)hi << 32) | lo;
}

struct TnParams {
    float* part; long M; int Ka; int Nb; int BN; int n_tiles_n; int n_tiles_k; int splits; long m_per_split; int stages;
    int raw_hi;
};

constexpr int TN_LO_SLOTS = 2;
constexpr int TN_SPLIT_WARPS = 8;
constexpr int TN_THREADS = (2 + TN_SPLIT_WARPS + 4) * 32;

__global__ void __launch_bounds__(TN_THREADS, 1)
gemm_tn_tc_kernel(const __grid_constant__ CUtensorMap tmX, const __grid_constant__ CUtensorMap tmG, const TnParams p) {
    extern __shared__ uint8_t smem_raw[];
    __shared__ __align__(8) uint64_t bars[2 * TC_MAX_STAGES + 2 * TN_LO_SLOTS + 1];
    __shared__ uint32_t tmem_slot;

    const int warp = threadIdx.x >> 5, lane = threadIdx.x & 31;
    const uint32_t base = (smem_u32(smem_raw) + 1023u) & ~1023u;
    const int nbc = p.BN / 32;
    const uint32_t half = (uint32_t)(TN_ACH + nbc) * TN_CHUNK;
    const uint32_t b_off = TN_ACH * TN_CHUNK;
    auto raw = [&](int s) { return base + (uint32_t)s * half; };
    auto lo = [&](int l) { return base + (uint32_t)(p.stages + l) * half; };
    const uint32_t bar0 = smem_u32(bars);
    auto full = [&](int s) { return bar0 + 8u * s; };
    auto rawfree = [&](int s) { return bar0 + 8u * (TC_MAX_STAGES + s); };
    auto conv = [&](int l) { return bar0 + 8u * (2 * TC_MAX_STAGES + l); };
    auto lofree = [&](int l) { return bar0 + 8u * (2 * TC_MAX_STAGES + TN_LO_SLOTS + l); };
    const uint32_t tfull = bar0 + 8u * (2 * TC_MAX_STAGES + 2 * TN_LO_SLOTS);

    const int tile = blockIdx.x % (p.n_tiles_k * p.n_tiles_n);
    const int split = blockIdx.x / (p.n_tiles_k * p.n_tiles_n);
    const int ka0 = (tile / p.n_tiles_n) * 128, nb0 = (tile % p.n_tiles_n) * p.BN;
    const long mbeg = (long)split * p.m_per_split;
    long mend = mbeg + p.m_per_split;
    if (mend > p.M) mend = p.M;
    const int num_kb = mend > mbeg ? (int)((mend - mbeg + TN_BKM - 1) / TN_BKM) : 0;

    if (threadIdx.x == 0) {
        asm volatile("prefetch.tensormap [%0];" ::"l"(&tmX) : "memory");
        asm volatile("prefetch.tensormap [%0];" ::"l"(&tmG) : "memory");
        for (int s = 0; s < TC_MAX_STAGES; ++s) { mbar_init(full(s), 1); mbar_init(rawfree(s), 1); }
        for (int l = 0; l < TN_LO_SLOTS; ++l) { mbar_init(conv(l), TN_SPLIT_WARPS * 32); mbar_init(lofree(l), 1); }
        mbar_init(tfull, 1);
        asm volatile("fence.mbarrier_init.release.cluster;" ::: "memory");
    }
    if (warp == 1) {
        asm volatile("tcgen05.alloc.cta_group::1.sync.aligned.shared::cta.b32 [%0], %1;" ::"r"(smem_u32(&tmem_slot)), "r"(256u) : "memory");
        asm volatile("tcgen05.relinquish_alloc_permit.cta_group::1.sync.aligned;" ::: "memory");
    }
    tc_fence_before();
    __syncthreads();
    tc_fence_after();
    const uint32_t tmem_base = tmem_slot;

    if (warp == 0) {
        if (lane == 0) {
            for (int kb = 0; kb < num_kb; ++kb) {
                const int s = kb % p.stages;
                const uint32_t ph = (kb / p.stages) & 1u;
                mbar_wait(rawfree(s), ph ^ 1u);
                mbar_arrive_expect_tx(full(s), half);
                const int m0 = (int)(mbeg + (long)kb * TN_BKM);
                for (int c = 0; c < TN_ACH; ++c) tma_load_2d(raw(s) + c * TN_CHUNK, &tmX, full(s), ka0 + 32 * c, m0);
                for (int c = 0; c < nbc; ++c) tma_load_2d(raw(s) + b_off + c * TN_CHUNK, &tmG, full(s), nb0 + 32 * c, m0);
            }
        }
    } else if (warp == 1) {
        if (lane == 0) {
// ... 165 lines not shown
```

### recon_b200/functional.py

```python
import ctypes as C
import os
import weakref

import torch

from . import _lib
from .graph import KGraph

MAX_HEADS = 4
USE_TC = True
TC_MIN_ROWS = 1


WD_ALIGN = int(os.environ.get("SPK_WD_ALIGN", "8"))


class Geometry:

    def __init__(self, n_heads, d_head):
        assert 1 <= n_heads <= MAX_HEADS
        self.H, self.D = n_heads, d_head
        self.Dp = (d_head + 3) // 4 * 4
        self.Dt = self.H * self.Dp
        self.Wd = (self.Dt + self.H + WD_ALIGN - 1) // WD_ALIGN * WD_ALIGN
# ... 360 lines not shown
    d = den[n:]
    d0 = torch.where(sw[n:] == 0, torch.zeros_like(d), d)
    buf = torch.cat(((v * d0.unsqueeze(-1)).reshape(ng, H * W), d0), dim=1)
    ghost.sum_partials(buf)
    dg = buf[:, H * W:]
    dg = torch.where(dg == 0, torch.full_like(dg, 1e-12), dg)
    vals[n:] = (buf[:, :H * W].view(ng, H, W) / dg.unsqueeze(-1)).reshape(ng, H * W)
    den[n:] = dg


def _ghost_dout(ghost, dout, n, n_ext):
    ext = torch.empty(n_ext, dout.shape[1], dtype=dout.dtype, device=dout.device)
    ext[:n] = dout
    ext[n:] = ghost.gather_rows(dout)
    ext[ghost.mine_local] = 0
    return ext


class AttentionGroupFn(torch.autograd.Function):

    @staticmethod
    def forward(ctx, X, Wn, Rel, Wr, graph, geom, alpha, apply_elu, mask_csr, nanflag):
        X = tc_friendly(X.contiguous()); Wn = Wn.contiguous(); Rel = Rel.contiguous(); Wr = Wr.contiguous()
        dist = getattr(graph, "dist", None)
        ghost = dist.ghost if dist is not None else None
        Wd = geom.Wd
        mode = "local"
        X_all = None
        if dist is None:
            P3 = gemm_nn(Rel, Wr)
            P = gemm_nn(X, Wn)
            P1, P2 = P[:, :Wd], P[:, Wd:]
        elif 2 * X.shape[1] <= Wd:
            mode = "input"
            Fp = (X.shape[1] + 3) // 4 * 4
            X_all, mine = dist.gather_buffer(Fp, X.device)
            mine[:, :X.shape[1]].copy_(X)
            if Fp != X.shape[1]:
                mine[:, X.shape[1]:].zero_()
            h = dist.all_gather_start(X_all)
            P3 = gemm_nn(Rel, Wr)
            P1 = gemm_nn(X, Wn[:, :Wd])
            h.wait()
            X_all = X_all[:, :X.shape[1]]
            P2 = gemm_nn(X_all, Wn[:, Wd:])
        else:
            mode = "proj"
            P2, mine = dist.gather_buffer(Wd, X.device)
            gemm_nn(X, Wn[:, Wd:], out=mine)
            h = dist.all_gather_start(P2)
            n = X.shape[0]
            if ghost is None:
                P1 = gemm_nn(X, Wn[:, :Wd])
            else:
                P1 = torch.empty(n + ghost.n, Wd, dtype=torch.float32, device=X.device)
                gemm_nn(X, Wn[:, :Wd], out=P1[:n])
                gemm_nn(tc_friendly(ghost.gather_rows(X)), Wn[:, :Wd], out=P1[n:])
            P3 = gemm_nn(Rel, Wr)
            h.wait()
        if ghost is not None and mode != "proj":
            raise NotImplementedError("hub rows split across ranks need the projected exchange (or the aggregate-then-project path)")
        if ghost is None:
            out, den, sw = edge_attn_forward(graph, P1, P2, P3, geom, alpha, apply_elu, mask_csr, nanflag)
            out_ret = out
        else:
            n = X.shape[0]
            k_elu = bool(apply_elu) and n > 0
            out, den, sw = edge_attn_forward(graph, P1, P2, P3, geom, alpha, k_elu, mask_csr, nanflag, elu_rows=n if k_elu else 0)
            _ghost_combine(ghost, out, den, sw, n, geom.H)
            nanflag.bitwise_or_(torch.isnan(out[n:]).any().to(torch.int32))
            if apply_elu and out.shape[0] > n:
                tail = out[n:]
                _lib.check(_lib.load().spk_elu_inplace(_lib.ptr(tail), tail.stride(0), tail.shape[0], tail.shape[1],
                                                       _lib.stream_ptr()), "elu_inplace")
            out[ghost.mine_local] = out[n:][ghost.mine]
            out_ret = out[:n]
        ctx.save_for_backward(X, Wn, Rel, Wr, P1, P2, P3, out, den, sw, X_all if X_all is not None else X.new_empty(0))
        ctx.graph, ctx.geom, ctx.alpha, ctx.apply_elu, ctx.mask_csr, ctx.mode = graph, geom, alpha, apply_elu, mask_csr, mode
        ctx.mark_non_differentiable(den, sw)
        return out_ret, den, sw

    @staticmethod
    def backward(ctx, dout, _dden, _dsw):
        geom, graph, mode = ctx.geom, ctx.graph, ctx.mode
        dist = getattr(graph, "dist", None)
        X, Wn, Rel, Wr, P1, P2, P3, out, den, sw, X_all = ctx.saved_tensors
        Wd = geom.Wd
        dout = dout.contiguous()
        n = X.shape[0]
        dev = X.device
        dP3 = torch.empty_like(P3)
        WnT = Wn.t().contiguous()
        need_x, need_w = ctx.needs_input_grad[0], ctx.needs_input_grad[1]
        dX = dWn = None
        if mode == "local":
            dP = torch.empty(n, 2 * Wd, dtype=torch.float32, device=dev)
            edge_attn_backward(graph, P1, P2, P3, geom, ctx.alpha, ctx.apply_elu, ctx.mask_csr, out, dout, den, sw,
                               dP[:, :Wd], dP[:, Wd:], dP3)
            if need_x:
                dX = gemm_nn(dP, WnT)
            if need_w:
                dWn = gemm_tn(X, dP)
        else:
            mr = dist.part.max_rows
            ghost = dist.ghost
            n_ext = n + (ghost.n if ghost is not None else 0)
            if ghost is not None:
                dout = _ghost_dout(ghost, dout, n, n_ext)
            dP1 = torch.empty(n_ext, Wd, dtype=torch.float32, device=dev)
            dP2_all = torch.empty_like(P2)
            colsum = torch.empty(P2.shape[0], geom.H, dtype=torch.float32, device=dev)
            pend = {}

            def start_main():
                if mode == "proj":
                    pend["pad"] = torch.empty(mr, Wd, dtype=torch.float32, device=dev)
                    pend["h"] = dist.reduce_scatter_start(dP2_all, pend["pad"])

            split = edge_attn_backward(graph, P1, P2, P3, geom, ctx.alpha, ctx.apply_elu, ctx.mask_csr, out, dout, den, sw,
                                       dP1, dP2_all, dP3, after_columns=start_main if mode == "proj" else None, colsum=colsum)
            if mode == "proj":
                if split:
                    qs_pad = torch.empty(mr, geom.H, dtype=torch.float32, device=dev)
                    hq = dist.reduce_scatter_start(colsum, qs_pad)
                else:
                    start_main()
                h3 = dist.all_reduce_start(dP3)
                if ghost is not None:
                    gsum = ghost.sum_partials(dP1[n:].contiguous())
                    dP1[ghost.mine_local] = gsum[ghost.mine]
                    dP1 = dP1[:n]
                if need_x:
                    dX = gemm_nn(dP1, WnT[:Wd])
                if need_w:
                    dWn = torch.empty_like(Wn)
                    gemm_tn(X, dP1, out=dWn[:, :Wd])
                pend["h"].wait()
                dP2 = pend["pad"][:n]
                if split:
                    hq.wait()
                    dP2[:, geom.Dt:geom.Dt + geom.H].copy_(qs_pad[:n])
                del dP2_all
                if need_x:
                    gemm_nn(dP2, WnT[Wd:], out=dX, accumulate=True)
                if need_w:
                    gemm_tn(X, dP2, out=dWn[:, Wd:])
                    dist.all_reduce(dWn)
                h3.wait()
            else:
                h3 = dist.all_reduce_start(dP3)
                F = X.shape[1]
                Fp = (F + 3) // 4 * 4
                if need_x:
                    dX2_all = torch.empty(P2.shape[0], Fp, dtype=torch.float32, device=dev)
                    gemm_nn(dP2_all, WnT[Wd:], out=dX2_all[:, :F])
                    if Fp != F:
                        dX2_all[:, F:].zero_()
                    pad = torch.empty(mr, Fp, dtype=torch.float32, device=dev)
                    h = dist.reduce_scatter_start(dX2_all, pad)
                    dX1 = gemm_nn(dP1, WnT[:Wd])
                    h.wait()
                    dX = dX1.add_(pad[:n, :F])
                    del dX2_all
                if need_w:
                    dWn = torch.empty_like(Wn)
                    gemm_tn(X, dP1, out=dWn[:, :Wd])
                    gemm_tn(X_all, dP2_all, out=dWn[:, Wd:])
                    dist.all_reduce(dWn)
                h3.wait()
        dRel = gemm_nn(dP3, Wr.t().contiguous()) if ctx.needs_input_grad[2] else None
        dWr = gemm_tn(Rel, dP3) if ctx.needs_input_grad[3] else None
        return dX, dWn, dRel, dWr, None, None, None, None, None, None



AGG_MODE = "auto"
AGG_BWD_MODE = os.environ.get("SPK_AGG_BWD_MODE", "split")
AGG_MAX_HEADS = 2


G_ALIGN = int(os.environ.get("SPK_G_ALIGN", "8"))
GX_ALIGN = int(os.environ.get("SPK_GX_ALIGN", "8"))
LX_ALIGN = int(os.environ.get("SPK_LX_ALIGN", "8"))


def _row_stride(width, align):
    return (width + align - 1) // align * align


class AggGeometry:

    def __init__(self, n_heads, in_features, nrela_dim, d_head):
        self.H, self.F, self.Rd, self.D = n_heads, in_features, nrela_dim, d_head
        self.Fx4, self.Fr4 = (in_features + 3) // 4, (nrela_dim + 3) // 4
        self.Fp, self.Rp = 4 * self.Fx4, 4 * self.Fr4
        self.LX = _row_stride(self.Fp + 4, LX_ALIGN)
        self.LR = _row_stride(self.Rp + 4, LX_ALIGN)
        self.LZ = 2 * self.Fp + self.Rp

    @staticmethod
    def supported(n_heads, in_features, nrela_dim):
        return 1 <= n_heads <= AGG_MAX_HEADS and 1 <= in_features <= 60 and 1 <= nrela_dim <= 60

    def struct(self):
        return _lib.AggGeom(self.H, self.Fx4, self.Fr4, self.LZ)


def use_agg_path(n_heads, in_features, nrela_dim, d_head, graph):
    if AGG_MODE == "off" or (getattr(graph, "dist", None) is None and graph.n_cols != graph.n_nodes):
        return False
    if not AggGeometry.supported(n_heads, in_features, nrela_dim):
        return False
    if AGG_MODE == "force":
        return True
    g = AggGeometry(n_heads, in_features, nrela_dim, d_head)
    return g.LX + g.LR < n_heads * d_head


def agg_weights(a_list, a2_list, geom):
    if _on_library(list(a_list) + list(a2_list)):
        dims = dict(F=geom.F, Rd=geom.Rd, D=geom.D, Fp=geom.Fp, LZ=geom.LZ)
        return AttnWeightsFn.apply(1, dims, *a_list, *a2_list)
    return _agg_weights_torch(a_list, a2_list, geom)


def _agg_weights_torch(a_list, a2_list, geom):
    F, Rd, Fp = geom.F, geom.Rd, geom.Fp
    a0 = a_list[0]
    Wa = a0.new_zeros(geom.H, geom.LZ, geom.D)
    V = a0.new_zeros(F, 4)
    V3 = a0.new_zeros(Rd, 4)
    for h, (a, a2) in enumerate(zip(a_list, a2_list)):
        at = a.t()
        qa = (at * a2).sum(dim=1)
        Wa[h, :F] = at[:F]
        Wa[h, Fp:Fp + F] = at[F:2 * F]
        Wa[h, 2 * Fp:2 * Fp + Rd] = at[2 * F:]
        V[:, 2 + h] = qa[:F]
        V[:, h] = qa[F:2 * F]
        V3[:, h] = qa[2 * F:]
    return Wa, V, V3


def _agg_table(X, V, ld, chunks, out=None):
    T = torch.empty(X.shape[0], ld, dtype=torch.float32, device=X.device) if out is None else out
    assert T.shape[0] == X.shape[0] and T.stride(1) == 1 and T.stride(0) >= ld
    ld = T.stride(0)
    if X.shape[0]:
        _lib.check(_lib.load().spk_agg_table(_lib.ptr(X), X.stride(0), _lib.ptr(V), _lib.ptr(T), ld, X.shape[0],
                                             X.shape[1], chunks, _lib.stream_ptr()), "agg_table")
    return T


class AggGroupFn(torch.autograd.Function):

    @staticmethod
    def forward(ctx, X, Rel, Wa, V, V3, graph, geom, alpha, apply_elu, mask_csr, nanflag):
        lib = _lib.load()
        X = X.contiguous(); Rel = Rel.contiguous(); Wa = Wa.contiguous(); V = V.contiguous(); V3 = V3.contiguous()
        n, dev = graph.n_nodes, X.device
        n_loc = X.shape[0]
        H, D, LZ = geom.H, geom.D, geom.LZ
        dist = getattr(graph, "dist", None)
        ghost = dist.ghost if dist is not None else None
        if dist is None:
            Xt = _agg_table(X, V, geom.LX, geom.Fx4)
            Xc = Xt
            Rt = _agg_table(Rel, V3, geom.LR, geom.Fr4)
            _X_TABLE["key"], _X_TABLE["table"] = _x_key(X), weakref.ref(Xt)
        else:
            Xc, Xt = dist.gather_buffer(geom.LX, dev)
            _agg_table(X, V, geom.LX, geom.Fx4, out=Xt)
            hx = dist.all_gather_start(Xc)
            Rt = _agg_table(Rel, V3, geom.LR, geom.Fr4)
            hx.wait()
            if ghost is not None:
                lo = dist.rank * dist.part.max_rows
                Xc[lo + n_loc:lo + n] = Xc[ghost.padded_ids]
                Xt = Xc[lo:lo + n]
        Z = torch.empty(n, H * LZ, dtype=torch.float32, device=dev)
        den = torch.empty(n, H, dtype=torch.float32, device=dev)
        sw = torch.empty(n, H, dtype=torch.float32, device=dev)
        a = _lib.AggFwdArgs()
        a.segptr = graph.rowptr.data_ptr(); a.col = graph.col.data_ptr(); a.t1 = graph.t1.data_ptr()
        a.t2 = graph.t2.data_ptr() if graph.t2 is not None else None
        a.xrow = Xt.data_ptr(); a.ldxr = Xt.stride(0); a.xcol = Xc.data_ptr(); a.ldxc = Xc.stride(0)
        a.rel = Rt.data_ptr(); a.ldr = Rt.stride(0)
        if mask_csr is not None:
            a.mask = mask_csr.data_ptr(); a.mask_stride = mask_csr.stride(0)
        a.z = Z.data_ptr(); a.ldz = Z.stride(0); a.den = den.data_ptr(); a.sw = sw.data_ptr()
        a.nanflag = nanflag.data_ptr(); a.n_rows = n; a.alpha = float(alpha); a.geom = geom.struct()
        partial = _hub_partial(graph.row_hubs, 264, dev)
        graph.row_hubs.fill(a.hub, partial, 264)
        _lib.check(lib.spk_agg_fwd(C.byref(a), _lib.stream_ptr()), "agg_fwd")
        if ghost is not None:
            _ghost_combine(ghost, Z, den, sw, n_loc, H)
        out = torch.empty(n, H * D, dtype=torch.float32, device=dev)
        for h in range(H):
            gemm_nn(Z[:, h * LZ:(h + 1) * LZ], Wa[h], out=out[:, h * D:(h + 1) * D], act=int(apply_elu))
        if ghost is not None:
            nanflag.bitwise_or_(torch.isnan(out[n_loc:]).any().to(torch.int32))
            out[ghost.mine_local] = out[n_loc:][ghost.mine]
        ctx.save_for_backward(X, Rel, Wa, V, V3, Xt, Rt, Z, out, den, sw, Xc)
        ctx.graph, ctx.geom, ctx.alpha, ctx.apply_elu, ctx.mask_csr = graph, geom, alpha, apply_elu, mask_csr
        return out[:n_loc] if ghost is not None else out

    @staticmethod
    def backward(ctx, dout):
        lib = _lib.load()
        geom, graph = ctx.geom, ctx.graph
        X, Rel, Wa, V, V3, Xt, Rt, Z, out, den, sw, Xc = ctx.saved_tensors
        dist = getattr(graph, "dist", None)
        graph.build_backward()
        n, dev = graph.n_nodes, X.device
        n_loc = X.shape[0]
        ghost = dist.ghost if dist is not None else None
        H, D, LZ, Fp, Rp = geom.H, geom.D, geom.LZ, geom.Fp, geom.Rp
        f32 = dict(dtype=torch.float32, device=dev)
        dout = dout.contiguous()
        if ghost is not None:
            dout = _ghost_dout(ghost, dout, n_loc, n)
        dhn = torch.empty(n, H * D, **f32)
        dden = torch.empty(n, H, **f32)
        _lib.check(lib.spk_agg_bwd_pre(_lib.ptr(out), _lib.ptr(dout), out.stride(0), _lib.ptr(den), H, D,
                                       int(ctx.apply_elu), _lib.ptr(dhn), dhn.stride(0), _lib.ptr(dden), n,
                                       _lib.stream_ptr()), "agg_bwd_pre")
        dZ = torch.empty(n, H * LZ, **f32)
        dWa = torch.empty_like(Wa)
        for h in range(H):
            dh = dhn[:, h * D:(h + 1) * D]
            gemm_nn(dh, Wa[h].t().contiguous(), out=dZ[:, h * LZ:(h + 1) * LZ])
            if ghost is None:
                gemm_tn(Z[:, h * LZ:(h + 1) * LZ], dh, out=dWa[h])
            else:
                gemm_tn(Z[:n_loc, h * LZ:(h + 1) * LZ], dh[:n_loc], out=dWa[h])
                gemm_tn((Z[n_loc:, h * LZ:(h + 1) * LZ] * ghost.mine.unsqueeze(1)).contiguous(), dh[n_loc:], out=dWa[h],
                        accumulate=True)
        Gx = torch.empty(n, _row_stride(H * Fp, GX_ALIGN), **f32)[:, :H * Fp]
        Gr = torch.empty(n, _row_stride(H * Rp, GX_ALIGN), **f32)[:, :H * Rp]
        rowout = torch.empty(n, Fp + 4, **f32)
        a = _lib.AggBwdArgs()
        a.xrow = Xt.data_ptr(); a.ldxr = Xt.stride(0)
        a.dz = dZ.data_ptr(); a.ldz = dZ.stride(0)
        a.den = den.data_ptr(); a.sw = sw.data_ptr(); a.dden = dden.data_ptr()
        a.gx = Gx.data_ptr(); a.ldgx = Gx.stride(0); a.gr = Gr.data_ptr(); a.ldgr = Gr.stride(0)
        a.rowout = rowout.data_ptr(); a.ldro = rowout.stride(0)
        a.n_rows = n; a.alpha = float(ctx.alpha); a.geom = geom.struct()
        gx_geom, gr_geom = Geometry(H, Fp), Geometry(H, Rp)
        dXc = torch.empty(graph.n_cols, gx_geom.Wd, **f32)
        dRc = torch.empty(graph.n_rel, gr_geom.Wd, **f32)
        split = AGG_BWD_MODE == "split" and graph.t2 is None and Fp == Rp
        if split:
            rowsc = torch.empty(max(1, n), H, 4, **f32)
            a.rowsc = rowsc.data_ptr()
            _lib.check(lib.spk_agg_bwd_ctx(C.byref(a), _lib.stream_ptr()), "agg_bwd_ctx")
            del dZ
            ne = max(1, graph.n_edges)
            q = _lib.EdgeBwdSplitArgs()
            b = q.base
            b.rowptr = graph.rowptr.data_ptr()
            b.colptr = graph.colptr.data_ptr(); b.csc_row = graph.csc_row.data_ptr(); b.csc_pos = graph.csc_pos.data_ptr()
            b.csc_t1 = graph.csc_t1.data_ptr()
            b.P1 = Xc.data_ptr(); b.ld1 = Xc.stride(0)
            b.P2 = Xc.data_ptr(); b.ld2 = Xc.stride(0); b.P3 = Rt.data_ptr(); b.ld3 = Rt.stride(0)
            if ctx.mask_csr is not None:
                b.mask = ctx.mask_csr.data_ptr(); b.mask_stride = ctx.mask_csr.stride(0)
            b.G = Gx.data_ptr(); b.ldg = Gx.stride(0); b.rowsc = rowsc.data_ptr()
            b.dP1 = dXc.data_ptr(); b.ldd1 = dXc.stride(0)
            b.dP2 = dXc.data_ptr(); b.ldd2 = dXc.stride(0)
            b.n_rows = n; b.n_cols = graph.n_cols; b.apply_elu = 0; b.alpha = float(ctx.alpha)
            b.geom = gx_geom.struct()
            graph.row_hubs.fill(b.row_hub, None, 0)
            partc = _hub_partial(graph.col_hubs, gx_geom.Wd, dev)
            graph.col_hubs.fill(b.col_hub, partc, gx_geom.Wd)
            q.relptr = graph.relptr.data_ptr(); q.rel_row = graph.rel_row.data_ptr(); q.rel_pos = graph.rel_pos.data_ptr()
            rec4 = torch.empty(ne, H, 4, **f32); dsv = torch.empty(ne, H, **f32)
            q.rec4 = rec4.data_ptr(); q.dsv = dsv.data_ptr()
            q.dP3 = dRc.data_ptr(); q.ldd3 = dRc.stride(0); q.n_rel = graph.n_rel
            part3 = _hub_partial(graph.rel_hubs, gr_geom.Wd, dev)
            graph.rel_hubs.fill(q.rel_hub, part3, gr_geom.Wd)
            part1 = _hub_partial(graph.row_hubs, 4, dev)
            graph.row_hubs.fill(q.base.row_hub, part1, 4)
            rowsum = torch.empty(max(1, n), H, **f32)
            q.rowsum = rowsum.data_ptr(); q.ld_rowsum = H
            q.G_rel = Gr.data_ptr(); q.ldg_rel = Gr.stride(0)
            q.dup = 1

            def run(phases, tag):
                q.phases = phases
                _lib.current_tag = tag + f":w{gx_geom.Wd}"
                try:
                    _lib.check(lib.spk_edge_attn_bwd_split(C.byref(q), _lib.stream_ptr()), "edge_attn_bwd_split")
                finally:
                    _lib.current_tag = ""
        else:
            rec = torch.empty(max(1, graph.n_edges), 2 * H, **f32)
            a.segptr = graph.rowptr.data_ptr(); a.col = graph.col.data_ptr(); a.t1 = graph.t1.data_ptr()
            a.t2 = graph.t2.data_ptr() if graph.t2 is not None else None
            a.xcol = Xc.data_ptr(); a.ldxc = Xc.stride(0)
            a.rel = Rt.data_ptr(); a.ldr = Rt.stride(0)
            if ctx.mask_csr is not None:
                a.mask = ctx.mask_csr.data_ptr(); a.mask_stride = ctx.mask_csr.stride(0)
            rowsc = torch.empty(max(1, n), 8, **f32)
            a.rowsc = rowsc.data_ptr(); a.rec = rec.data_ptr()
            part = _hub_partial(graph.row_hubs, 8, dev)
            graph.row_hubs.fill(a.hub, part, 8)
            _lib.check(lib.spk_agg_bwd_rows(C.byref(a), _lib.stream_ptr()), "agg_bwd_rows")
            del dZ
        if split:
            run(2, "cols")
        else:
            seg_gather(graph.colptr, graph.csc_row, graph.csc_pos, graph.col_hubs, Gx, Gx.stride(0), rec, gx_geom, dXc,
                       graph.n_cols, "cols")
        if dist is not None:
            dXc_all = dXc
            dXc_pad = torch.empty(dist.part.max_rows, gx_geom.Wd, **f32)
            hx = dist.reduce_scatter_start(dXc_all, dXc_pad)
        if split:
            run(4, "rels")
            rowout[:, Fp:Fp + H] = rowsum[:n]
            if dist is not None:
                colsum = torch.empty(graph.n_cols, H, **f32)
                q.colsum = colsum.data_ptr(); q.ld_colsum = H
            run(8, "colsums")
            if dist is not None:
                qs_pad = torch.empty(dist.part.max_rows, H, **f32)
                hq = dist.reduce_scatter_start(colsum, qs_pad)
        else:
            seg_gather(graph.relptr, graph.rel_row, graph.rel_pos, graph.rel_hubs, Gr, Gr.stride(0), rec, gr_geom, dRc,
                       graph.n_rel, "rels")
        if dist is not None:
            dist.all_reduce(dRc)
            dist.all_reduce(dWa)
            if ghost is not None:
                gsum = ghost.sum_partials(rowout[n_loc:].contiguous())
                rowout[ghost.mine_local] = gsum[ghost.mine]
            hx.wait()
            dXc = dXc_pad[:n_loc]
            del dXc_all
            if split:
                hq.wait()
                dXc[:, H * Fp:H * Fp + H].copy_(qs_pad[:n_loc])
        n = n_loc
        dX = torch.empty(n, geom.F, **f32)
        dq = torch.empty(n, 4, **f32)
        _lib.check(lib.spk_agg_dx(_lib.ptr(rowout), rowout.stride(0), _lib.ptr(dXc), dXc.stride(0), _lib.ptr(V), n,
                                  geom.F, geom.Fx4, H, _lib.ptr(dX), dX.stride(0), _lib.ptr(dq), _lib.stream_ptr()),
                   "agg_dx")
        dV = gemm_tn(Xt[:n, :geom.F], dq) if ctx.needs_input_grad[3] else None
        if dV is not None and dist is not None:
            dist.all_reduce(dV)
        dq3 = dRc[:, H * Rp:H * Rp + H].contiguous()
        dRel = None
        if ctx.needs_input_grad[1]:
            dRel = dRc[:, :geom.Rd].clone()
            for h in range(1, H):
                dRel += dRc[:, h * Rp:h * Rp + geom.Rd]
            dRel = gemm_nn(dq3, V3[:, :H].t().contiguous(), out=dRel, accumulate=True)
        dV3 = None
        if ctx.needs_input_grad[4]:
            dV3 = torch.zeros_like(V3)
            dV3[:, :H] = gemm_tn(Rel, dq3)
        return dX, dRel, dWa, dV, dV3, None, None, None, None, None, None


def attention_group(X, Rel, a_list, a2_list, graph, alpha, apply_elu, mask_csr, nanflag):
    outs = []
    if X.shape[0] != graph.n_nodes - getattr(graph, "n_ghost", 0):
        raise IndexError(f"entity table has {X.shape[0]} rows but the graph was built for "
                         f"{graph.n_nodes - getattr(graph, 'n_ghost', 0)} nodes")
    if getattr(graph, "dist", None) is None and graph.n_cols > X.shape[0]:
        raise IndexError(f"graph gathers from {graph.n_cols} nodes but the entity table has {X.shape[0]} rows")
    if Rel.shape[0] < graph.n_rel:
        raise IndexError(f"relation table has {Rel.shape[0]} rows but the graph uses {graph.n_rel} relations")
    if X.device != graph.device or Rel.device != graph.device:
        raise RuntimeError(f"tables on {X.device} / {Rel.device} but the graph layouts live on {graph.device}")
    F = X.shape[1]
    D = a_list[0].shape[0]
    Rd = a_list[0].shape[1] - 2 * F
    if use_agg_path(min(len(a_list), AGG_MAX_HEADS), F, Rd, D, graph):
        for g0 in range(0, len(a_list), AGG_MAX_HEADS):
            al, a2l = a_list[g0:g0 + AGG_MAX_HEADS], a2_list[g0:g0 + AGG_MAX_HEADS]
            geom = AggGeometry(len(al), F, Rd, D)
            Wa, V, V3 = agg_weights(al, a2l, geom)
            m = None if mask_csr is None else mask_csr[g0:g0 + AGG_MAX_HEADS].contiguous()
            outs.append(AggGroupFn.apply(X, Rel, Wa, V, V3, graph, geom, alpha, apply_elu, m, nanflag))
        return outs[0] if len(outs) == 1 else torch.cat(outs, dim=1)
    for g0 in range(0, len(a_list), MAX_HEADS):
        al, a2l = a_list[g0:g0 + MAX_HEADS], a2_list[g0:g0 + MAX_HEADS]
        geom = Geometry(len(al), D)
        Wn, Wr = extended_weights(al, a2l, F, geom)
        m = None if mask_csr is None else mask_csr[g0:g0 + MAX_HEADS].contiguous()
        out, _, _ = AttentionGroupFn.apply(X, Wn, Rel, Wr, graph, geom, alpha, apply_elu, m, nanflag)
        outs.append(out)
    return outs[0] if len(outs) == 1 else torch.cat(outs, dim=1)



def rownorm_(x):
    assert x.dim() == 2 and x.stride(1) == 1
    _lib.check(_lib.load().spk_rownorm(_lib.ptr(x), x.stride(0), _lib.ptr(x), x.stride(0), x.shape[0], x.shape[1],
                                       _lib.stream_ptr()), "rownorm")
    return x


def rownorm(x):
    x = x.contiguous()
    y = torch.empty_like(x)
    _lib.check(_lib.load().spk_rownorm(_lib.ptr(x), x.stride(0), _lib.ptr(y), y.stride(0), x.shape[0], x.shape[1],
                                       _lib.stream_ptr()), "rownorm")
    return y


def mask_from_index(idx, n_rows, device, flag=None):
    mask = torch.zeros(n_rows, dtype=torch.float32, device=device)
    if idx.numel() and not idx.is_cuda:
        if int(idx.min()) < -n_rows or int(idx.max()) >= n_rows:
            raise IndexError("batch_entities index out of range")
    idx = idx.to(device=device, dtype=torch.int64).contiguous()
    if idx.numel():
        own = flag is None
        if own:
            flag = torch.zeros(1, dtype=torch.int32, device=device)
        _lib.check(_lib.load().spk_mask_from_index(_lib.ptr(idx), idx.numel(), _lib.ptr(mask), n_rows, _lib.ptr(flag),
                                                   _lib.stream_ptr()), "mask_from_index")
        if own and int(flag.item()) & 2:
            raise IndexError("batch_entities index out of range")
    return mask


class ResidualNormFn(torch.autograd.Function):

    @staticmethod
    def forward(ctx, EW, x2, mask):
        EW = EW.contiguous(); x2 = x2.contiguous()
        n, w = EW.shape
        out = torch.empty_like(EW)
        inv = torch.empty(n, dtype=torch.float32, device=EW.device)
        _lib.check(_lib.load().spk_residual_norm_fwd(_lib.ptr(EW), EW.stride(0), _lib.ptr(x2), x2.stride(0),
                                                     _lib.ptr(mask), _lib.ptr(out), out.stride(0), _lib.ptr(inv),
                                                     n, w, _lib.stream_ptr()), "residual_norm_fwd")
        ctx.save_for_backward(out, mask, inv)
        return out

    @staticmethod
    def backward(ctx, g):
        out, mask, inv = ctx.saved_tensors
        g = g.contiguous()
        n, w = out.shape
        dew = torch.empty_like(out)
        dx2 = torch.empty_like(out)
        _lib.check(_lib.load().spk_residual_norm_bwd(_lib.ptr(g), g.stride(0), _lib.ptr(out), out.stride(0),
                                                     _lib.ptr(mask), _lib.ptr(inv), _lib.ptr(dew), dew.stride(0),
                                                     _lib.ptr(dx2), dx2.stride(0), n, w, _lib.stream_ptr()),
                   "residual_norm_bwd")
        return dew, dx2, None



class InnerProductFn(torch.autograd.Function):

    @staticmethod
    def forward(ctx, *tensors):
        k = len(tensors) // 2
        a_list = [t.contiguous() for t in tensors[:k]]
        b_list = [t.contiguous() for t in tensors[k:]]
        lib = _lib.load()
        dev = a_list[0].device
        out = torch.empty(1, dtype=torch.float32, device=dev)
        ws = torch.empty(lib.spk_inner_product_workspace_bytes(), dtype=torch.uint8, device=dev)
        for i, (a, b) in enumerate(zip(a_list, b_list)):
            assert a.shape == b.shape and a.dtype == b.dtype == torch.float32
            _lib.check(lib.spk_inner_product(_lib.ptr(a), _lib.ptr(b), a.numel(), _lib.ptr(ws), _lib.ptr(out), int(i > 0),
                                             _lib.stream_ptr()), "inner_product")
        ctx.save_for_backward(*a_list, *b_list)
        return out.reshape(())

    @staticmethod
    def backward(ctx, g):
        t = ctx.saved_tensors
        k = len(t) // 2
        grads = [g * t[k + i] if ctx.needs_input_grad[i] else None for i in range(k)]
        grads += [g * t[i] if ctx.needs_input_grad[k + i] else None for i in range(k)]
        return tuple(grads)


def inner_product(a_list, b_list):
    return InnerProductFn.apply(*a_list, *b_list)


def linear_loss_backward(outs, grads):
    with torch.no_grad():
        loss = inner_product([o.detach() for o in outs], list(grads))
    torch.autograd.backward(list(outs), [g.to(o.dtype) for o, g in zip(outs, grads)])
    return loss
```

### recon_b200/models.py

```python
import torch
import torch.nn as nn

from . import functional as SF
from .graph import KGraph
from .layers import SpGraphAttentionLayer, ConvKB, check_nanflag, edge_dropout_mask


def _fingerprint(t):
    if t.is_cuda or t.numel() == 0:
        return None
    flat = t.reshape(-1)
    n = flat.numel()
    return tuple(int(flat[i]) for i in sorted({0, n // 3, n // 2, (2 * n) // 3, n - 1}))


def _nhop_rows(edge_list_nhop, edge_type_nhop):
    if edge_type_nhop is None or edge_type_nhop.numel() == 0:
        return None
    el = edge_list_nhop.long()
    et = edge_type_nhop.long().to(el.device)
    return torch.stack((el[1], et[:, 0], et[:, 1], el[0]), dim=1)


class SpGAT(nn.Module):
    def __init__(self, num_nodes, nfeat, nhid, relation_dim, dropout, alpha, nheads):
        super().__init__()
        self.dropout = dropout
        self.alpha = alpha
        self.dropout_layer = nn.Dropout(self.dropout)
        self.attentions = [SpGraphAttentionLayer(num_nodes, nfeat, nhid, relation_dim, dropout=dropout,
                                                 alpha=alpha, concat=True) for _ in range(nheads)]
        for i, attention in enumerate(self.attentions):
            self.add_module('attention_{}'.format(i), attention)
        self.W = nn.Parameter(torch.zeros(size=(relation_dim, nheads * nhid)))
        nn.init.xavier_uniform_(self.W.data, gain=1.414)
        self.out_att = SpGraphAttentionLayer(num_nodes, nhid * nheads, nheads * nhid, nheads * nhid,
                                             dropout=dropout, alpha=alpha, concat=False)

    def forward(self, Corpus_, entity_embeddings, relation_embed, edge_list, edge_type, edge_embed,
                edge_list_nhop, edge_type_nhop, graph=None, dropout_masks=None, nanflag=None):
        x = entity_embeddings
        if not x.is_cuda:
            raise RuntimeError("recon_b200.SpGAT needs CUDA tensors (no CPU fallback)")
        dev = x.device
        with torch.cuda.device(dev):
            return self._forward(x, relation_embed, edge_list, edge_type, edge_list_nhop, edge_type_nhop, graph,
                                 dropout_masks, nanflag)

    def _forward(self, x, relation_embed, edge_list, edge_type, edge_list_nhop, edge_type_nhop, graph, dropout_masks, nanflag):
        dev = x.device
        if graph is None:
            graph = KGraph(edge_list, edge_type, _nhop_rows(edge_list_nhop, edge_type_nhop), x.shape[0],
                           relation_embed.shape[0], device=dev)
        own_flag = nanflag is None
        if own_flag:
            nanflag = torch.zeros(1, dtype=torch.int32, device=dev)
        nheads = len(self.attentions)
        e = graph.n_edges
        p = self.dropout
        m_att = m_out = m_x = None
        if dropout_masks is not None:
            if dropout_masks.get("att") is not None:
                m_att = graph.to_csr_order(dropout_masks["att"].to(dev, torch.float32).reshape(nheads, e))
            if dropout_masks.get("out") is not None:
                m_out = graph.to_csr_order(dropout_masks["out"].to(dev, torch.float32).reshape(1, e))
            if dropout_masks.get("x") is not None:
                m_x = dropout_masks["x"].to(dev, torch.float32)
        elif self.training and p > 0:
            m_att = edge_dropout_mask(p, nheads, e, dev)
            m_out = edge_dropout_mask(p, 1, e, dev)
            m_x = (torch.rand(x.shape[0], nheads * self.attentions[0].out_features, device=dev) >= p).float().mul_(1.0 / (1.0 - p))

        x = SF.attention_group(x, relation_embed, [att.a for att in self.attentions],
                               [att.a_2 for att in self.attentions], graph, self.alpha, True, m_att, nanflag)
        if m_x is not None:
            x = x * m_x
        out_relation_1 = SF.matmul(relation_embed, self.W)
        x = SF.attention_group(x, out_relation_1, [self.out_att.a], [self.out_att.a_2], graph, self.alpha,
                               True, m_out, nanflag)
        if own_flag:
            check_nanflag(nanflag)
        return x, out_relation_1


class SpKBGATModified(nn.Module):
    def __init__(self, initial_entity_emb, initial_relation_emb, entity_out_dim, relation_out_dim,
                 drop_GAT, alpha, nheads_GAT, initial_entity_emb_params=None, *, sep_space=False):
        super().__init__()
        self.num_nodes = initial_entity_emb.shape[0]
        self.entity_in_dim = initial_entity_emb.shape[1]
        self.entity_out_dim_1 = entity_out_dim[0]
        self.nheads_GAT_1 = nheads_GAT[0]
        self.entity_out_dim_2 = entity_out_dim[1]
        self.nheads_GAT_2 = nheads_GAT[1]
        self.num_relation = initial_relation_emb.shape[0]
        self.relation_dim = initial_relation_emb.shape[1]
        self.relation_out_dim_1 = relation_out_dim[0]
        self.drop_GAT = drop_GAT
        self.alpha = alpha
        hd = self.entity_out_dim_1 * self.nheads_GAT_1
        self.final_entity_embeddings = nn.Parameter(torch.randn(self.num_nodes, hd))
        self.final_relation_embeddings = nn.Parameter(torch.randn(self.num_relation, hd))
        self.entity_embeddings = nn.Parameter(initial_entity_emb)
        self.relation_embeddings = nn.Parameter(initial_relation_emb)
        self.sparse_gat_1 = SpGAT(self.num_nodes, self.entity_in_dim, self.entity_out_dim_1, self.relation_dim,
                                  self.drop_GAT, self.alpha, self.nheads_GAT_1)
        self.W_entities = nn.Parameter(torch.zeros(size=(self.entity_in_dim, hd)))
        nn.init.xavier_uniform_(self.W_entities.data, gain=1.414)
        self.nonlinearity_ent2rel = torch.tanh
        if sep_space:
            self.W_ent2rel = nn.Parameter(torch.zeros(size=(self.num_relation, hd, hd)))
            nn.init.xavier_uniform_(self.W_ent2rel.data, gain=1.414)
        self._graph_cache = {}
        self.graph_cache = True

    def load_state_dict(self, state_dict, strict=True, **kw):
        has = "W_ent2rel" in self._parameters
        if "W_ent2rel" in state_dict and not has:
            w = state_dict["W_ent2rel"]
            self.W_ent2rel = nn.Parameter(torch.empty_like(w, device=self.W_entities.device))
        elif has and "W_ent2rel" not in state_dict:
            state_dict = dict(state_dict)
            state_dict["W_ent2rel"] = self.W_ent2rel.detach()
        return super().load_state_dict(state_dict, strict=strict, **kw)

    def _graph_key(self, adj, train_indices_nhop):
        edge_list, edge_type = adj[0], adj[1]
        has2 = train_indices_nhop is not None and train_indices_nhop.numel() > 0
        tensors = (edge_list, edge_type, train_indices_nhop) if has2 else (edge_list, edge_type)
        dev = self.entity_embeddings.device
        return (str(dev),) + tuple((t.data_ptr(), tuple(t.shape), t._version, str(t.device), _fingerprint(t)) for t in tensors)

    def _graph_is_cached(self, adj, train_indices_nhop):
        if isinstance(adj, KGraph):
            return True
        return bool(self.graph_cache) and self._graph_key(adj, train_indices_nhop) in self._graph_cache

    def prepare_graph(self, adj, train_indices_nhop=None):
        if isinstance(adj, KGraph):
            return adj
        edge_list, edge_type = adj[0], adj[1]
        has2 = train_indices_nhop is not None and train_indices_nhop.numel() > 0
        dev = self.entity_embeddings.device
        if dev.type != "cuda":
            raise RuntimeError("recon_b200.SpKBGATModified must live on a CUDA device (no CPU fallback)")
        key = self._graph_key(adj, train_indices_nhop)
        g = self._graph_cache.get(key) if self.graph_cache else None
        if g is None:
            nhop = train_indices_nhop if has2 else None
            with torch.cuda.device(dev):
                g = KGraph(edge_list, edge_type, nhop, self.num_nodes, self.num_relation, device=dev)
            self._graph_cache.clear()
            if self.graph_cache:
                self._graph_cache[key] = g
                g._keepalive = (edge_list, edge_type, train_indices_nhop)
        return g

    def _run(self, entity_embeddings, relation_embeddings, batch_entities, graph, dropout_masks, entities_upgraded=None):
        with torch.cuda.device(entity_embeddings.device):
            return self._run_on(entity_embeddings, relation_embeddings, batch_entities, graph, dropout_masks, entities_upgraded)

    def _run_on(self, entity_embeddings, relation_embeddings, batch_entities, graph, dropout_masks, entities_upgraded=None):
        dev = entity_embeddings.device
        nanflag = torch.zeros(1, dtype=torch.int32, device=dev)
        out_entity_1, out_relation_1 = self.sparse_gat_1(
            None, entity_embeddings, relation_embeddings, None, None, None, None, None,
            graph=graph, dropout_masks=dropout_masks, nanflag=nanflag)
        mask = SF.mask_from_index(torch.as_tensor(batch_entities), entity_embeddings.shape[0], dev, flag=nanflag)
        if entities_upgraded is None:
            entities_upgraded = SF.matmul(entity_embeddings, self.W_entities, getattr(graph, "dist", None))
        out_entity_1 = SF.ResidualNormFn.apply(entities_upgraded, out_entity_1, mask)
        check_nanflag(nanflag)
        return out_entity_1, out_relation_1, mask

    def forward(self, Corpus_, batch_entities, adj, train_indices_nhop, dropout_masks=None):
        if self.entity_embeddings.device.type != "cuda":
            raise RuntimeError("recon_b200.SpKBGATModified must live on a CUDA device (no CPU fallback)")
        pre = None
        with torch.cuda.device(self.entity_embeddings.device):
            self.entity_embeddings.data = SF.rownorm(self.entity_embeddings.data)
            if not self._graph_is_cached(adj, train_indices_nhop):
                pre = SF.matmul(self.entity_embeddings, self.W_entities, None)
        graph = self.prepare_graph(adj, train_indices_nhop)
        out_entity_1, out_relation_1, mask = self._run(self.entity_embeddings, self.relation_embeddings,
                                                       batch_entities, graph, dropout_masks, pre)
        self.final_entity_embeddings.data = out_entity_1.data
        self.final_relation_embeddings.data = out_relation_1.data
        return out_entity_1, out_relation_1, mask

    def batch_test(self, Corpus_, batch_entities, adj, train_indices_nhop, entity_embeddings, dropout_masks=None):
        graph = self.prepare_graph(adj, train_indices_nhop)
        relation_embeddings = self.relation_embeddings.detach()
        entity_embeddings = SF.rownorm(entity_embeddings.data.to(self.W_entities.device))
        return self._run(entity_embeddings, relation_embeddings, batch_entities, graph, dropout_masks)
```

Baseline: 496.0 million.

## Fuse residual-norm and aggregation-backward prologue into tcgen05 GEMM epilogues

Adds two new epilogue variants to the tensor-core NN GEMM kernel. One applies the masked residual add and row L2 normalisation straight from TMEM, using a TMA-staged second operand. The other computes the ELU backward and per-head denominator gradient while projecting dX in the attention backward. The model now routes the entity projection plus residual norm, and the two stacked attention layers, through these fused paths, which removes intermediate GEMM outputs and separate row kernels. The cost is more epilogue work per tile, extra shared-memory staging and barriers, and a new autograd function whose backward recomputes through separate kernels.

```diff
diff --git a/include/spkbgat.h b/include/spkbgat.h
--- a/include/spkbgat.h
+++ b/include/spkbgat.h
@@ -63,6 +63,13 @@
 int spk_gemm_nn_tc_act(const float* A, int64_t lda, const float* B, int64_t ldb, float* C, int64_t ldc,
                        int64_t M, int32_t N, int32_t K, int32_t accumulate, int32_t act, float* workspace,
                        spk_stream_t stream);
+int spk_gemm_nn_tc_resnorm(const float* A, int64_t lda, const float* B, int64_t ldb, float* C, int64_t ldc,
+                           int64_t M, int32_t N, int32_t K, const float* x2, int64_t ldx, const float* mask,
+                           float* inv_norm, float* workspace, spk_stream_t stream);
+int spk_gemm_nn_tc_aggpre(const float* A, int64_t lda, const float* B, int64_t ldb, float* dhn, int64_t ldd,
+                          int64_t M, int32_t N, int32_t K, const float* out, int64_t ldo, const float* den,
+                          int32_t n_heads, int32_t d_head, int32_t apply_elu, float* dden, float* workspace,
+                          spk_stream_t stream);
 int spk_elu_inplace(float* x, int64_t ldx, int64_t n_rows, int32_t width, spk_stream_t stream);
 
 int32_t spk_gemm_tn_tc_supported(const float* A, int64_t lda, const float* B, int64_t ldb, int64_t M, int32_t Ka, int32_t Nb);
diff --git a/recon_b200/_lib.py b/recon_b200/_lib.py
--- a/recon_b200/_lib.py
+++ b/recon_b200/_lib.py
@@ -165,6 +165,9 @@
     "spk_gemm_tc_workspace_floats": (_I64, [_I32, _I32]),
     "spk_gemm_nn_tc": (_I32, [_VP, _I64, _VP, _I64, _VP, _I64, _I64, _I32, _I32, _I32, _VP, _VP]),
     "spk_gemm_nn_tc_act": (_I32, [_VP, _I64, _VP, _I64, _VP, _I64, _I64, _I32, _I32, _I32, _I32, _VP, _VP]),
+    "spk_gemm_nn_tc_resnorm": (_I32, [_VP, _I64, _VP, _I64, _VP, _I64, _I64, _I32, _I32, _VP, _I64, _VP, _VP, _VP, _VP]),
+    "spk_gemm_nn_tc_aggpre": (_I32, [_VP, _I64, _VP, _I64, _VP, _I64, _I64, _I32, _I32, _VP, _I64, _VP, _I32, _I32, _I32,
+                                     _VP, _VP, _VP]),
     "spk_elu_inplace": (_I32, [_VP, _I64, _I64, _I32, _VP]),
     "spk_agg_table": (_I32, [_VP, _I64, _VP, _VP, _I64, _I64, _I32, _I32, _VP]),
     "spk_agg_fwd": (_I32, [C.POINTER(AggFwdArgs), _VP]),
diff --git a/recon_b200/csrc/spk_agg.cu b/recon_b200/csrc/spk_agg.cu
--- a/recon_b200/csrc/spk_agg.cu
+++ b/recon_b200/csrc/spk_agg.cu
@@ -874,16 +874,6 @@
     return 0;
 }
 
-__device__ __forceinline__ void bwd_pre_elem(float ov, float gv, int apply_elu, float& dh, float& p) {
-    float hv = ov;
-    dh = gv;
-    if (apply_elu) {
-        const bool pos = ov > 0.f;
-        dh = pos ? gv : gv * (ov + 1.f);
-        hv = pos ? ov : (ov > -1.f ? fast_log1p(ov) : 0.f);
-    }
-    p = fmaf(dh, hv, p);
-}
 
 __global__ void __launch_bounds__(256)
 agg_bwd_pre_vec_kernel(const float* __restrict__ out, const float* __restrict__ dout, long ldo, const float* __restrict__ den,
diff --git a/recon_b200/csrc/spk_api.cu b/recon_b200/csrc/spk_api.cu
--- a/recon_b200/csrc/spk_api.cu
+++ b/recon_b200/csrc/spk_api.cu
@@ -150,6 +150,24 @@
     if (act < 0 || act > 2) { set_error("gemm_nn_tc_act: unknown activation %d", act); return 1; }
     return gemm_nn_tc(A, lda, B, ldb, C, ldc, M, N, K, accumulate, workspace, (cudaStream_t)stream, act);
 }
+int spk_gemm_nn_tc_resnorm(const float* A, int64_t lda, const float* B, int64_t ldb, float* C, int64_t ldc,
+                           int64_t M, int32_t N, int32_t K, const float* x2, int64_t ldx, const float* mask,
+                           float* inv_norm, float* workspace, spk_stream_t stream) {
+    if (lda < K || ldb < N || ldc < N) { set_error("gemm_nn_tc_resnorm: leading dimension too small"); return 1; }
+    if (!gemm_nn_tc_supported(A, lda, M, N, K)) { set_error("gemm_nn_tc_resnorm: A must be 16-byte aligned with lda %% 4 == 0"); return 1; }
+    if (!workspace || (reinterpret_cast<uintptr_t>(workspace) & 15)) { set_error("gemm_nn_tc_resnorm: aligned workspace required"); return 1; }
+    return gemm_nn_tc_resnorm(A, lda, B, ldb, C, ldc, M, N, K, x2, ldx, mask, inv_norm, workspace, (cudaStream_t)stream);
+}
+int spk_gemm_nn_tc_aggpre(const float* A, int64_t lda, const float* B, int64_t ldb, float* dhn, int64_t ldd,
+                          int64_t M, int32_t N, int32_t K, const float* out, int64_t ldo, const float* den,
+                          int32_t n_heads, int32_t d_head, int32_t apply_elu, float* dden, float* workspace,
+                          spk_stream_t stream) {
+    if (lda < K || ldb < N || ldd < N) { set_error("gemm_nn_tc_aggpre: leading dimension too small"); return 1; }
+    if (!gemm_nn_tc_supported(A, lda, M, N, K)) { set_error("gemm_nn_tc_aggpre: A must be 16-byte aligned with lda %% 4 == 0"); return 1; }
+    if (!workspace || (reinterpret_cast<uintptr_t>(workspace) & 15)) { set_error("gemm_nn_tc_aggpre: aligned workspace required"); return 1; }
+    return gemm_nn_tc_aggpre(A, lda, B, ldb, dhn, ldd, M, N, K, out, ldo, den, n_heads, d_head, apply_elu, dden, workspace,
+                             (cudaStream_t)stream);
+}
 int spk_elu_inplace(float* x, int64_t ldx, int64_t n_rows, int32_t width, spk_stream_t stream) {
     if (ldx < width) { set_error("elu_inplace: leading dimension too small"); return 1; }
     return launch_elu_inplace(x, ldx, n_rows, width, (cudaStream_t)stream);
diff --git a/recon_b200/csrc/spk_common.cuh b/recon_b200/csrc/spk_common.cuh
--- a/recon_b200/csrc/spk_common.cuh
+++ b/recon_b200/csrc/spk_common.cuh
@@ -55,6 +55,17 @@
     const float u = 1.0f + x;
     const float d = u - 1.0f;
     return d == 0.f ? x : __logf(u) * __fdividef(x, d);
+}
+
+__device__ __forceinline__ void bwd_pre_elem(float ov, float gv, int apply_elu, float& dh, float& p) {
+    float hv = ov;
+    dh = gv;
+    if (apply_elu) {
+        const bool pos = ov > 0.f;
+        dh = pos ? gv : gv * (ov + 1.f);
+        hv = pos ? ov : (ov > -1.f ? fast_log1p(ov) : 0.f);
+    }
+    p = fmaf(dh, hv, p);
 }
 
 __device__ __forceinline__ float4 ldg4(const float* p) {
diff --git a/recon_b200/csrc/spk_gemm.cuh b/recon_b200/csrc/spk_gemm.cuh
--- a/recon_b200/csrc/spk_gemm.cuh
+++ b/recon_b200/csrc/spk_gemm.cuh
@@ -15,6 +15,11 @@
 int gemm_nn_tc_supported(const float* A, long lda, long M, int N, int K);
 int gemm_nn_tc(const float* A, long lda, const float* B, long ldb, float* C, long ldc, long M, int N, int K,
                int accumulate, float* workspace, cudaStream_t s, int act = 0);
+int gemm_nn_tc_resnorm(const float* A, long lda, const float* B, long ldb, float* C, long ldc, long M, int N, int K,
+                       const float* X, long ldx, const float* mask, float* inv_norm, float* workspace, cudaStream_t s);
+int gemm_nn_tc_aggpre(const float* A, long lda, const float* B, long ldb, float* dhn, long ldd, long M, int N, int K,
+                      const float* out, long ldo, const float* den, int heads, int d_head, int apply_elu, float* dden,
+                      float* workspace, cudaStream_t s);
 int gemm_tn_tc_supported(const float* A, long lda, const float* B, long ldb, long M, int Ka, int Nb);
 long gemm_tn_tc_workspace_floats(long M, int Ka, int Nb);
 int gemm_tn_tc(const float* A, long lda, const float* B, long ldb, float* C, long ldc, long M, int Ka, int Nb,
diff --git a/recon_b200/csrc/spk_gemm_tc.cu b/recon_b200/csrc/spk_gemm_tc.cu
--- a/recon_b200/csrc/spk_gemm_tc.cu
+++ b/recon_b200/csrc/spk_gemm_tc.cu
@@ -82,7 +82,16 @@
     int c_tma;
     int raw_hi;
     int cs;
+    const float* mask;
+    float* inv_norm;
+    const float* den;
+    float* dden;
+    int heads, d4, apply_elu;
 };
+
+constexpr int EPI_PLAIN = 0;
+constexpr int EPI_RESNORM = 1;
+constexpr int EPI_AGGPRE = 2;
 
 __device__ __forceinline__ float tc_elu(float x) {
     const float big = exp2f(x * 1.4426950408889634f) - 1.0f;
@@ -93,11 +102,53 @@
 
 __device__ __forceinline__ float tc_act(float x, int act) { return act == 2 ? tanhf(x) : tc_elu(x); }
 
+__device__ __forceinline__ void tmem_ld32(uint32_t taddr, uint32_t (&r)[32]) {
+    asm volatile(
+        "tcgen05.ld.sync.aligned.32x32b.x32.b32 {%0,%1,%2,%3,%4,%5,%6,%7,%8,%9,%10,%11,%12,%13,%14,%15,"
+        "%16,%17,%18,%19,%20,%21,%22,%23,%24,%25,%26,%27,%28,%29,%30,%31}, [%32];"
+        : "=r"(r[0]), "=r"(r[1]), "=r"(r[2]), "=r"(r[3]), "=r"(r[4]), "=r"(r[5]), "=r"(r[6]), "=r"(r[7]),
+          "=r"(r[8]), "=r"(r[9]), "=r"(r[10]), "=r"(r[11]), "=r"(r[12]), "=r"(r[13]), "=r"(r[14]), "=r"(r[15]),
+          "=r"(r[16]), "=r"(r[17]), "=r"(r[18]), "=r"(r[19]), "=r"(r[20]), "=r"(r[21]), "=r"(r[22]), "=r"(r[23]),
+          "=r"(r[24]), "=r"(r[25]), "=r"(r[26]), "=r"(r[27]), "=r"(r[28]), "=r"(r[29]), "=r"(r[30]), "=r"(r[31])
+        : "r"(taddr));
+    asm volatile("tcgen05.wait::ld.sync.aligned;" ::: "memory");
+}
+__device__ __forceinline__ void tmem_st32(uint32_t taddr, const uint32_t (&r)[32]) {
+    asm volatile(
+        "tcgen05.st.sync.aligned.32x32b.x32.b32 [%0], {%1,%2,%3,%4,%5,%6,%7,%8,%9,%10,%11,%12,%13,%14,%15,%16,"
+        "%17,%18,%19,%20,%21,%22,%23,%24,%25,%26,%27,%28,%29,%30,%31,%32};"
+        ::"r"(taddr), "r"(r[0]), "r"(r[1]), "r"(r[2]), "r"(r[3]), "r"(r[4]), "r"(r[5]), "r"(r[6]), "r"(r[7]),
+          "r"(r[8]), "r"(r[9]), "r"(r[10]), "r"(r[11]), "r"(r[12]), "r"(r[13]), "r"(r[14]), "r"(r[15]),
+          "r"(r[16]), "r"(r[17]), "r"(r[18]), "r"(r[19]), "r"(r[20]), "r"(r[21]), "r"(r[22]), "r"(r[23]),
+          "r"(r[24]), "r"(r[25]), "r"(r[26]), "r"(r[27]), "r"(r[28]), "r"(r[29]), "r"(r[30]), "r"(r[31])
+        : "memory");
+}
+__device__ __forceinline__ void stg_store_row(uint32_t stg, int lane, const uint32_t (&r)[32]) {
+    const uint32_t rowaddr = stg + (uint32_t)lane * 128u;
+#pragma unroll
+    for (int j = 0; j < 8; ++j) {
+        const uint32_t a = rowaddr + (uint32_t)((j ^ (lane & 7)) << 4);
+        asm volatile("st.shared.v4.b32 [%0], {%1,%2,%3,%4};" ::"r"(a), "r"(r[4 * j]), "r"(r[4 * j + 1]),
+                     "r"(r[4 * j + 2]), "r"(r[4 * j + 3]) : "memory");
+    }
+}
+__device__ __forceinline__ void stg_load_row(uint32_t stg, int lane, float (&x)[32]) {
+    const uint32_t rowaddr = stg + (uint32_t)lane * 128u;
+#pragma unroll
+    for (int j = 0; j < 8; ++j) {
+        const uint32_t a = rowaddr + (uint32_t)((j ^ (lane & 7)) << 4);
+        asm volatile("ld.shared.v4.f32 {%0,%1,%2,%3}, [%4];" : "=f"(x[4 * j]), "=f"(x[4 * j + 1]), "=f"(x[4 * j + 2]),
+                     "=f"(x[4 * j + 3]) : "r"(a) : "memory");
+    }
+}
+
+template <int EPI>
 __global__ void __launch_bounds__(TC_THREADS, 1)
 gemm_nn_tc_kernel(const __grid_constant__ CUtensorMap tmA, const __grid_constant__ CUtensorMap tmBhi,
-                  const __grid_constant__ CUtensorMap tmBlo, const __grid_constant__ CUtensorMap tmC, const TcParams p) {
+                  const __grid_constant__ CUtensorMap tmBlo, const __grid_constant__ CUtensorMap tmC,
+                  const __grid_constant__ CUtensorMap tmX, const TcParams p) {
     extern __shared__ uint8_t smem_raw[];
-    __shared__ __align__(8) uint64_t bars[3 * TC_MAX_STAGES + 4];
+    __shared__ __align__(8) uint64_t bars[3 * TC_MAX_STAGES + 4 + (EPI != EPI_PLAIN ? 8 : 0)];
     __shared__ uint32_t tmem_slot;
 
     const int warp = threadIdx.x >> 5, lane = threadIdx.x & 31;
@@ -131,6 +182,10 @@
         asm volatile("prefetch.tensormap [%0];" ::"l"(&tmBlo) : "memory");
         for (int s = 0; s < TC_MAX_STAGES; ++s) { mbar_init(full(s), 1); mbar_init(conv(s), 128); mbar_init(empty(s), (uint32_t)cs); }
         for (int a = 0; a < 2; ++a) { mbar_init(tfull(a), 1); mbar_init(tempty(a), 4); }
+        if constexpr (EPI != EPI_PLAIN) {
+            asm volatile("prefetch.tensormap [%0];" ::"l"(&tmX) : "memory");
+            for (int b = 0; b < 8; ++b) mbar_init(bar0 + 8u * (3 * TC_MAX_STAGES + 4 + b), 1);
+        }
         asm volatile("fence.mbarrier_init.release.cluster;" ::: "memory");
     }
     if (warp == 1) {
@@ -222,6 +277,127 @@
                 mbar_arrive(conv(s));
             }
         }
+    } else if constexpr (EPI != EPI_PLAIN) {
+        const int q = warp & 3;
+        const uint32_t stg0 = base + (uint32_t)p.stages * stage_bytes + (uint32_t)q * 8192u;
+        const uint32_t xbar0 = bar0 + 8u * (3 * TC_MAX_STAGES + 4 + 2 * q);
+        const int nch = (p.N + 31) / 32;
+        auto prefetch_x = [&](long tile) {
+            const int r0 = (int)tile * TC_BM + q * 32;
+            if (lane == 0 && tile < total && r0 < p.M)
+                for (int k = 0; k < nch; ++k)
+                    asm volatile("cp.async.bulk.prefetch.tensor.2d.L2.global.tile [%0, {%1, %2}];"
+                                 ::"l"(&tmX), "r"(32 * k), "r"(r0) : "memory");
+        };
+        auto load_x = [&](int k, int r0) {
+            const uint32_t s = (uint32_t)k & 1u;
+            mbar_arrive_expect_tx(xbar0 + 8u * s, 4096u);
+            tma_load_2d(stg0 + s * 4096u, &tmX, xbar0 + 8u * s, 32 * k, r0);
+        };
+        prefetch_x(first);
+        uint32_t tl = 0, sb = 0, xph = 0;
+        for (long tile = first; tile < total; tile += stride, ++tl) {
+            const uint32_t acc = tl & 1u, aph = (tl >> 1) & 1u;
+            const int row0 = (int)tile * TC_BM + q * 32;
+            const long row = (long)row0 + lane;
+            prefetch_x(tile + stride);
+            mbar_wait(tfull(acc), aph);
+            tc_fence_after();
+            if (row0 < p.M) {
+                float m = 0.f;
+                if constexpr (EPI == EPI_RESNORM) m = row < p.M ? p.mask[row] : 0.f;
+                if (lane == 0) {
+                    asm volatile("cp.async.bulk.wait_group.read 0;" ::: "memory");
+                    load_x(0, row0);
+                    if (nch > 1) load_x(1, row0);
+                }
+                __syncwarp();
+                float pa[32], pb[32];
+#pragma unroll
+                for (int j = 0; j < 32; ++j) { pa[j] = 0.f; pb[j] = 0.f; }
+                const uint32_t tacc = tmem_base + acc * 256u + ((uint32_t)(q * 32) << 16);
+#pragma unroll
+                for (int k = 0; k < 8; ++k) {
+                    if (k >= nch) break;
+                    const uint32_t s = (uint32_t)k & 1u;
+                    uint32_t r[32];
+                    tmem_ld32(tacc + 32u * k, r);
+                    mbar_wait(xbar0 + 8u * s, (xph >> s) & 1u);
+                    xph ^= 1u << s;
+                    float x[32];
+                    stg_load_row(stg0 + s * 4096u, lane, x);
+                    __syncwarp();
+                    if (lane == 0 && k + 2 < nch) {
+                        asm volatile("fence.proxy.async.shared::cta;" ::: "memory");
+                        load_x(k + 2, row0);
+                    }
+                    if constexpr (EPI == EPI_RESNORM) {
+#pragma unroll
+                        for (int j = 0; j < 32; ++j) {
+                            const float v = fmaf(m, x[j], __uint_as_float(r[j]));
+                            if (32 * k + j < p.N) pa[j] = fmaf(v, v, pa[j]);
+                            r[j] = __float_as_uint(v);
+                        }
+                    } else {
+#pragma unroll
+                        for (int i = 0; i < 8; ++i) {
+                            const int c4 = 8 * k + i;
+                            if (c4 < p.heads * p.d4) {
+                                float a4 = 0.f, dh;
+#pragma unroll
+                                for (int e = 0; e < 4; ++e) {
+                                    bwd_pre_elem(x[4 * i + e], __uint_as_float(r[4 * i + e]), p.apply_elu, dh, a4);
+                                    r[4 * i + e] = __float_as_uint(dh);
+                                }
+                                if (c4 < p.d4) pa[c4 & 31] += a4;
+                                else pb[c4 & 31] += a4;
+                            }
+                        }
+                    }
+                    tmem_st32(tacc + 32u * k, r);
+                }
+                asm volatile("tcgen05.wait::st.sync.aligned;" ::: "memory");
+#pragma unroll
+                for (int o = 16; o > 0; o >>= 1)
+#pragma unroll
+                    for (int j = 0; j < o; ++j) {
+                        pa[j] = pa[j] + pa[j + o];
+                        if constexpr (EPI == EPI_AGGPRE) pb[j] = pb[j] + pb[j + o];
+                    }
+                float inv = 1.f;
+                if constexpr (EPI == EPI_RESNORM) {
+                    inv = 1.f / fmaxf(sqrtf(pa[0]), 1e-12f);
+                    if (row < p.M) p.inv_norm[row] = inv;
+                } else if (row < p.M) {
+                    p.dden[row * p.heads] = -pa[0] / p.den[row * p.heads];
+                    if (p.heads > 1) p.dden[row * p.heads + 1] = -pb[0] / p.den[row * p.heads + 1];
+                }
+                for (int k = 0; k < nch; ++k) {
+                    uint32_t r[32];
+                    tmem_ld32(tacc + 32u * k, r);
+                    if constexpr (EPI == EPI_RESNORM) {
+#pragma unroll
+                        for (int j = 0; j < 32; ++j) r[j] = __float_as_uint(__uint_as_float(r[j]) * inv);
+                    }
+                    if (lane == 0) asm volatile("cp.async.bulk.wait_group.read 1;" ::: "memory");
+                    __syncwarp();
+                    const uint32_t stg = stg0 + sb * 4096u;
+                    stg_store_row(stg, lane, r);
+                    asm volatile("fence.proxy.async.shared::cta;" ::: "memory");
+                    __syncwarp();
+                    if (lane == 0) {
+                        asm volatile("cp.async.bulk.tensor.2d.global.shared::cta.tile.bulk_group [%0, {%1, %2}], [%3];"
+                                     ::"l"(&tmC), "r"(32 * k), "r"(row0), "r"(stg) : "memory");
+                        asm volatile("cp.async.bulk.commit_group;" ::: "memory");
+                    }
+                    sb ^= 1u;
+                }
+            }
+            tc_fence_before();
+            __syncwarp();
+            if (lane == 0) mbar_arrive(tempty(acc));
+        }
+        if (lane == 0) asm volatile("cp.async.bulk.wait_group 0;" ::: "memory");
     } else if (p.c_tma) {
         const int q = warp & 3;
         const uint32_t stg0 = base + (uint32_t)p.stages * stage_bytes + (uint32_t)q * 8192u;
@@ -620,8 +796,29 @@
     return M >= 1 && N >= 1 && K >= 1 && (lda % 4 == 0) && ((reinterpret_cast<uintptr_t>(A) & 15) == 0) && lda >= K;
 }
 
-int gemm_nn_tc(const float* A, long lda, const float* B, long ldb, float* C, long ldc, long M, int N, int K,
-               int accumulate, float* workspace, cudaStream_t s, int act) {
+namespace {
+struct RowEpi {
+    int kind; const float* X; long ldx;
+    const float* mask; float* inv_norm;
+    const float* den; float* dden; int heads, d_head, apply_elu;
+};
+
+int gemm_nn_tc_launch(const float* A, long lda, const float* B, long ldb, float* C, long ldc, long M, int N, int K,
+                      int accumulate, float* workspace, cudaStream_t s, int act, const RowEpi* epi) {
+    const bool fused = epi != nullptr;
+    const char* name = !fused ? "gemm_nn_tc" : epi->kind == EPI_RESNORM ? "gemm_nn_tc_resnorm" : "gemm_nn_tc_aggpre";
+    if (fused) {
+        bool ok = N <= 256 && !accumulate && act == 0 && epi->X && epi->ldx >= N && ldc % 4 == 0 && epi->ldx % 4 == 0 &&
+                  ((reinterpret_cast<uintptr_t>(C) | reinterpret_cast<uintptr_t>(epi->X)) & 15) == 0;
+        if (epi->kind == EPI_RESNORM) ok = ok && epi->mask && epi->inv_norm;
+        else ok = ok && epi->den && epi->dden && epi->heads >= 1 && epi->heads <= 2 && epi->d_head % 4 == 0 &&
+                  epi->heads * epi->d_head == N;
+        if (!ok) {
+            set_error("%s: needs N <= 256 and 16-byte aligned C and X rows%s", name,
+                      epi->kind == EPI_RESNORM ? "" : ", 1-2 heads of a multiple of 4 columns");
+            return 2;
+        }
+    }
     const int ldt = gemm_tc_ldt(K);
     float* bhi = workspace;
     float* blo = workspace + (long)N * ldt;
@@ -647,7 +844,7 @@
     cudaGetDevice(&dev);
     cudaDeviceGetAttribute(&sms, cudaDevAttrMultiProcessorCount, dev);
     const long m_tiles = (M + TC_BM - 1) / TC_BM;
-    const bool pair = tc_pair() && c_tma && tc_raw_hi() && (BN % 16 == 0) && m_tiles * n_tiles_n >= 2L * sms;
+    const bool pair = !fused && tc_pair() && c_tma && tc_raw_hi() && (BN % 16 == 0) && m_tiles * n_tiles_n >= 2L * sms;
     if (pair) {
         const int half_tile = BN / 2 * 128;
         const int stage2 = 2 * TC_A_TILE + 2 * half_tile;
@@ -686,21 +883,29 @@
         (void)cudaLaunchKernelEx(&cfg, gemm_nn_tc2_kernel, tA, tBh, tBl, tC, q);
         return check_launch("gemm_nn_tc2");
     }
-    const int cs = (tc_cluster() == 2 && !accumulate && m_tiles * n_tiles_n >= 2L * sms) ? 2 : 1;
-
-    CUtensorMap tmA, tmBhi, tmBlo, tmC;
+    const int cs = (!fused && tc_cluster() == 2 && !accumulate && m_tiles * n_tiles_n >= 2L * sms) ? 2 : 1;
+
+    CUtensorMap tmA, tmBhi, tmBlo, tmC, tmX;
     if (int rc = make_map(&tmA, A, M, K, lda, TC_BM)) return rc;
     if (int rc = make_map(&tmBhi, bhi, N, K, ldt, BN / cs)) return rc;
     if (int rc = make_map(&tmBlo, blo, N, K, ldt, BN / cs)) return rc;
     if (c_tma) { if (int rc = make_map(&tmC, C, M, N, ldc, 32)) return rc; }
     else tmC = tmA;
+    if (fused) { if (int rc = make_map(&tmX, epi->X, M, N, epi->ldx, 32)) return rc; }
+    else tmX = tmA;
 
     TcParams p;
     p.C = C; p.ldc = ldc; p.M = M; p.N = N; p.K = K; p.BN = BN; p.n_tiles_n = n_tiles_n; p.stages = stages;
     p.accumulate = accumulate; p.act = act;
     p.c_vec = c_vec; p.c_tma = c_tma; p.raw_hi = tc_raw_hi(); p.cs = cs;
-    static SmemLimit lim;
-    if (lim.ensure(gemm_nn_tc_kernel, 226 * 1024) != cudaSuccess) {
+    p.mask = fused ? epi->mask : nullptr; p.inv_norm = fused ? epi->inv_norm : nullptr;
+    p.den = fused ? epi->den : nullptr; p.dden = fused ? epi->dden : nullptr;
+    p.heads = fused ? epi->heads : 0; p.d4 = fused ? epi->d_head / 4 : 0; p.apply_elu = fused ? epi->apply_elu : 0;
+    const int ek = fused ? epi->kind : EPI_PLAIN;
+    auto kernel = ek == EPI_RESNORM ? gemm_nn_tc_kernel<EPI_RESNORM>
+                : ek == EPI_AGGPRE ? gemm_nn_tc_kernel<EPI_AGGPRE> : gemm_nn_tc_kernel<EPI_PLAIN>;
+    static SmemLimit lim[3];
+    if (lim[ek].ensure(kernel, 226 * 1024) != cudaSuccess) {
         set_error("gemm_tc: cannot raise dynamic shared memory limit");
         (void)cudaGetLastError();
         return 3;
@@ -717,7 +922,7 @@
         static int clusters[64] = {};
         int nc = (dev >= 0 && dev < 64) ? clusters[dev] : 0;
         if (nc == 0) {
-            if (cudaOccupancyMaxActiveClusters(&nc, gemm_nn_tc_kernel, &cfg) != cudaSuccess || nc < 1) { (void)cudaGetLastError(); nc = sms / cs / 2; }
+            if (cudaOccupancyMaxActiveClusters(&nc, kernel, &cfg) != cudaSuccess || nc < 1) { (void)cudaGetLastError(); nc = sms / cs / 2; }
             if (dev >= 0 && dev < 64) clusters[dev] = nc;
         }
         resident = (long)nc * cs;
@@ -726,8 +931,27 @@
     grid = grid / cs * cs;
     if (grid < (unsigned)cs) grid = (unsigned)cs;
     cfg.gridDim = dim3(grid);
-    (void)cudaLaunchKernelEx(&cfg, gemm_nn_tc_kernel, tmA, tmBhi, tmBlo, tmC, p);
-    return check_launch("gemm_nn_tc");
+    (void)cudaLaunchKernelEx(&cfg, kernel, tmA, tmBhi, tmBlo, tmC, tmX, p);
+    return check_launch(name);
+}
+}
+
+int gemm_nn_tc(const float* A, long lda, const float* B, long ldb, float* C, long ldc, long M, int N, int K,
+               int accumulate, float* workspace, cudaStream_t s, int act) {
+    return gemm_nn_tc_launch(A, lda, B, ldb, C, ldc, M, N, K, accumulate, workspace, s, act, nullptr);
+}
+
+int gemm_nn_tc_resnorm(const float* A, long lda, const float* B, long ldb, float* C, long ldc, long M, int N, int K,
+                       const float* X, long ldx, const float* mask, float* inv_norm, float* workspace, cudaStream_t s) {
+    const RowEpi e = {EPI_RESNORM, X, ldx, mask, inv_norm, nullptr, nullptr, 0, 0, 0};
+    return gemm_nn_tc_launch(A, lda, B, ldb, C, ldc, M, N, K, 0, workspace, s, 0, &e);
+}
+
+int gemm_nn_tc_aggpre(const float* A, long lda, const float* B, long ldb, float* dhn, long ldd, long M, int N, int K,
+                      const float* out, long ldo, const float* den, int heads, int d_head, int apply_elu, float* dden,
+                      float* workspace, cudaStream_t s) {
+    const RowEpi e = {EPI_AGGPRE, out, ldo, nullptr, nullptr, den, dden, heads, d_head, apply_elu};
+    return gemm_nn_tc_launch(A, lda, B, ldb, dhn, ldd, M, N, K, 0, workspace, s, 0, &e);
 }
 
 
diff --git a/recon_b200/functional.py b/recon_b200/functional.py
--- a/recon_b200/functional.py
+++ b/recon_b200/functional.py
@@ -466,95 +466,99 @@
 
     @staticmethod
     def backward(ctx, dout, _dden, _dsw):
-        geom, graph, mode = ctx.geom, ctx.graph, ctx.mode
-        dist = getattr(graph, "dist", None)
-        X, Wn, Rel, Wr, P1, P2, P3, out, den, sw, X_all = ctx.saved_tensors
-        Wd = geom.Wd
-        dout = dout.contiguous()
-        n = X.shape[0]
-        dev = X.device
-        dP3 = torch.empty_like(P3)
-        WnT = Wn.t().contiguous()
-        need_x, need_w = ctx.needs_input_grad[0], ctx.needs_input_grad[1]
-        dX = dWn = None
-        if mode == "local":
-            dP = torch.empty(n, 2 * Wd, dtype=torch.float32, device=dev)
-            edge_attn_backward(graph, P1, P2, P3, geom, ctx.alpha, ctx.apply_elu, ctx.mask_csr, out, dout, den, sw,
-                               dP[:, :Wd], dP[:, Wd:], dP3)
+        return _attention_backward(ctx, dout)
+
+
+def _attention_backward(ctx, dout, project_dx=None):
+    geom, graph, mode = ctx.geom, ctx.graph, ctx.mode
+    dist = getattr(graph, "dist", None)
+    X, Wn, Rel, Wr, P1, P2, P3, out, den, sw, X_all = ctx.saved_tensors
+    Wd = geom.Wd
+    dout = dout.contiguous()
+    n = X.shape[0]
+    dev = X.device
+    dP3 = torch.empty_like(P3)
+    WnT = Wn.t().contiguous()
+    need_x, need_w = ctx.needs_input_grad[0], ctx.needs_input_grad[1]
+    dX = dWn = None
+    if mode == "local":
+        dP = torch.empty(n, 2 * Wd, dtype=torch.float32, device=dev)
+        edge_attn_backward(graph, P1, P2, P3, geom, ctx.alpha, ctx.apply_elu, ctx.mask_csr, out, dout, den, sw,
+                           dP[:, :Wd], dP[:, Wd:], dP3)
+        if need_x:
+            dX = gemm_nn(dP, WnT) if project_dx is None else project_dx(dP, WnT)
+        if need_w:
+            dWn = gemm_tn(X, dP)
+    else:
+        mr = dist.part.max_rows
+        ghost = dist.ghost
+        n_ext = n + (ghost.n if ghost is not None else 0)
+        if ghost is not None:
+            dout = _ghost_dout(ghost, dout, n, n_ext)
+        dP1 = torch.empty(n_ext, Wd, dtype=torch.float32, device=dev)
+        dP2_all = torch.empty_like(P2)
+        colsum = torch.empty(P2.shape[0], geom.H, dtype=torch.float32, device=dev)
+        pend = {}
+
+        def start_main():
+            if mode == "proj":
+                pend["pad"] = torch.empty(mr, Wd, dtype=torch.float32, device=dev)
+                pend["h"] = dist.reduce_scatter_start(dP2_all, pend["pad"])
+
+        split = edge_attn_backward(graph, P1, P2, P3, geom, ctx.alpha, ctx.apply_elu, ctx.mask_csr, out, dout, den, sw,
+                                   dP1, dP2_all, dP3, after_columns=start_main if mode == "proj" else None, colsum=colsum)
+        if mode == "proj":
+            if split:
+                qs_pad = torch.empty(mr, geom.H, dtype=torch.float32, device=dev)
+                hq = dist.reduce_scatter_start(colsum, qs_pad)
+            else:
+                start_main()
+            h3 = dist.all_reduce_start(dP3)
+            if ghost is not None:
+                gsum = ghost.sum_partials(dP1[n:].contiguous())
+                dP1[ghost.mine_local] = gsum[ghost.mine]
+                dP1 = dP1[:n]
             if need_x:
-                dX = gemm_nn(dP, WnT)
+                dX = gemm_nn(dP1, WnT[:Wd])
             if need_w:
-                dWn = gemm_tn(X, dP)
+                dWn = torch.empty_like(Wn)
+                gemm_tn(X, dP1, out=dWn[:, :Wd])
+            pend["h"].wait()
+            dP2 = pend["pad"][:n]
+            if split:
+                hq.wait()
+                dP2[:, geom.Dt:geom.Dt + geom.H].copy_(qs_pad[:n])
+            del dP2_all
+            if need_x:
+                gemm_nn(dP2, WnT[Wd:], out=dX, accumulate=True)
+            if need_w:
+                gemm_tn(X, dP2, out=dWn[:, Wd:])
+                dist.all_reduce(dWn)
+            h3.wait()
         else:
-            mr = dist.part.max_rows
-            ghost = dist.ghost
-            n_ext = n + (ghost.n if ghost is not None else 0)
-            if ghost is not None:
-                dout = _ghost_dout(ghost, dout, n, n_ext)
-            dP1 = torch.empty(n_ext, Wd, dtype=torch.float32, device=dev)
-            dP2_all = torch.empty_like(P2)
-            colsum = torch.empty(P2.shape[0], geom.H, dtype=torch.float32, device=dev)
-            pend = {}
-
-            def start_main():
-                if mode == "proj":
-                    pend["pad"] = torch.empty(mr, Wd, dtype=torch.float32, device=dev)
-                    pend["h"] = dist.reduce_scatter_start(dP2_all, pend["pad"])
-
-            split = edge_attn_backward(graph, P1, P2, P3, geom, ctx.alpha, ctx.apply_elu, ctx.mask_csr, out, dout, den, sw,
-                                       dP1, dP2_all, dP3, after_columns=start_main if mode == "proj" else None, colsum=colsum)
-            if mode == "proj":
-                if split:
-                    qs_pad = torch.empty(mr, geom.H, dtype=torch.float32, device=dev)
-                    hq = dist.reduce_scatter_start(colsum, qs_pad)
-                else:
-                    start_main()
-                h3 = dist.all_reduce_start(dP3)
-                if ghost is not None:
-                    gsum = ghost.sum_partials(dP1[n:].contiguous())
-                    dP1[ghost.mine_local] = gsum[ghost.mine]
-                    dP1 = dP1[:n]
-                if need_x:
-                    dX = gemm_nn(dP1, WnT[:Wd])
-                if need_w:
-                    dWn = torch.empty_like(Wn)
-                    gemm_tn(X, dP1, out=dWn[:, :Wd])
-                pend["h"].wait()
-                dP2 = pend["pad"][:n]
-                if split:
-                    hq.wait()
-                    dP2[:, geom.Dt:geom.Dt + geom.H].copy_(qs_pad[:n])
-                del dP2_all
-                if need_x:
-                    gemm_nn(dP2, WnT[Wd:], out=dX, accumulate=True)
-                if need_w:
-                    gemm_tn(X, dP2, out=dWn[:, Wd:])
-                    dist.all_reduce(dWn)
-                h3.wait()
-            else:
-                h3 = dist.all_reduce_start(dP3)
-                F = X.shape[1]
-                Fp = (F + 3) // 4 * 4
-                if need_x:
-                    dX2_all = torch.empty(P2.shape[0], Fp, dtype=torch.float32, device=dev)
-                    gemm_nn(dP2_all, WnT[Wd:], out=dX2_all[:, :F])
-                    if Fp != F:
-                        dX2_all[:, F:].zero_()
-                    pad = torch.empty(mr, Fp, dtype=torch.float32, device=dev)
-                    h = dist.reduce_scatter_start(dX2_all, pad)
-                    dX1 = gemm_nn(dP1, WnT[:Wd])
-                    h.wait()
-                    dX = dX1.add_(pad[:n, :F])
-                    del dX2_all
-                if need_w:
-                    dWn = torch.empty_like(Wn)
-                    gemm_tn(X, dP1, out=dWn[:, :Wd])
-                    gemm_tn(X_all, dP2_all, out=dWn[:, Wd:])
-                    dist.all_reduce(dWn)
-                h3.wait()
-        dRel = gemm_nn(dP3, Wr.t().contiguous()) if ctx.needs_input_grad[2] else None
-        dWr = gemm_tn(Rel, dP3) if ctx.needs_input_grad[3] else None
-        return dX, dWn, dRel, dWr, None, None, None, None, None, None
+            h3 = dist.all_reduce_start(dP3)
+            F = X.shape[1]
+            Fp = (F + 3) // 4 * 4
+            if need_x:
+                dX2_all = torch.empty(P2.shape[0], Fp, dtype=torch.float32, device=dev)
+                gemm_nn(dP2_all, WnT[Wd:], out=dX2_all[:, :F])
+                if Fp != F:
+                    dX2_all[:, F:].zero_()
+                pad = torch.empty(mr, Fp, dtype=torch.float32, device=dev)
+                h = dist.reduce_scatter_start(dX2_all, pad)
+                dX1 = gemm_nn(dP1, WnT[:Wd])
+                h.wait()
+                dX = dX1.add_(pad[:n, :F])
+                del dX2_all
+            if need_w:
+                dWn = torch.empty_like(Wn)
+                gemm_tn(X, dP1, out=dWn[:, :Wd])
+                gemm_tn(X_all, dP2_all, out=dWn[:, Wd:])
+                dist.all_reduce(dWn)
+            h3.wait()
+    dRel = gemm_nn(dP3, Wr.t().contiguous()) if ctx.needs_input_grad[2] else None
+    dWr = gemm_tn(Rel, dP3) if ctx.needs_input_grad[3] else None
+    return dX, dWn, dRel, dWr, None, None, None, None, None, None
 
 
 
@@ -691,16 +695,23 @@
 
     @staticmethod
     def backward(ctx, dout):
-        lib = _lib.load()
-        geom, graph = ctx.geom, ctx.graph
-        X, Rel, Wa, V, V3, Xt, Rt, Z, out, den, sw, Xc = ctx.saved_tensors
-        dist = getattr(graph, "dist", None)
-        graph.build_backward()
-        n, dev = graph.n_nodes, X.device
-        n_loc = X.shape[0]
-        ghost = dist.ghost if dist is not None else None
-        H, D, LZ, Fp, Rp = geom.H, geom.D, geom.LZ, geom.Fp, geom.Rp
-        f32 = dict(dtype=torch.float32, device=dev)
+        return _agg_backward(ctx, dout)
+
+
+def _agg_backward(ctx, dout, pre=None):
+    lib = _lib.load()
+    geom, graph = ctx.geom, ctx.graph
+    X, Rel, Wa, V, V3, Xt, Rt, Z, out, den, sw, Xc = ctx.saved_tensors
+    dist = getattr(graph, "dist", None)
+    graph.build_backward()
+    n, dev = graph.n_nodes, X.device
+    n_loc = X.shape[0]
+    ghost = dist.ghost if dist is not None else None
+    H, D, LZ, Fp, Rp = geom.H, geom.D, geom.LZ, geom.Fp, geom.Rp
+    f32 = dict(dtype=torch.float32, device=dev)
+    if pre is not None:
+        dhn, dden = pre
+    else:
         dout = dout.contiguous()
         if ghost is not None:
             dout = _ghost_dout(ghost, dout, n_loc, n)
@@ -709,147 +720,146 @@
         _lib.check(lib.spk_agg_bwd_pre(_lib.ptr(out), _lib.ptr(dout), out.stride(0), _lib.ptr(den), H, D,
                                        int(ctx.apply_elu), _lib.ptr(dhn), dhn.stride(0), _lib.ptr(dden), n,
                                        _lib.stream_ptr()), "agg_bwd_pre")
-        dZ = torch.empty(n, H * LZ, **f32)
-        dWa = torch.empty_like(Wa)
-        for h in range(H):
-            dh = dhn[:, h * D:(h + 1) * D]
-            gemm_nn(dh, Wa[h].t().contiguous(), out=dZ[:, h * LZ:(h + 1) * LZ])
-            if ghost is None:
-                gemm_tn(Z[:, h * LZ:(h + 1) * LZ], dh, out=dWa[h])
-            else:
-                gemm_tn(Z[:n_loc, h * LZ:(h + 1) * LZ], dh[:n_loc], out=dWa[h])
-                gemm_tn((Z[n_loc:, h * LZ:(h + 1) * LZ] * ghost.mine.unsqueeze(1)).contiguous(), dh[n_loc:], out=dWa[h],
-                        accumulate=True)
-        Gx = torch.empty(n, _row_stride(H * Fp, GX_ALIGN), **f32)[:, :H * Fp]
-        Gr = torch.empty(n, _row_stride(H * Rp, GX_ALIGN), **f32)[:, :H * Rp]
-        rowout = torch.empty(n, Fp + 4, **f32)
-        a = _lib.AggBwdArgs()
-        a.xrow = Xt.data_ptr(); a.ldxr = Xt.stride(0)
-        a.dz = dZ.data_ptr(); a.ldz = dZ.stride(0)
-        a.den = den.data_ptr(); a.sw = sw.data_ptr(); a.dden = dden.data_ptr()
-        a.gx = Gx.data_ptr(); a.ldgx = Gx.stride(0); a.gr = Gr.data_ptr(); a.ldgr = Gr.stride(0)
-        a.rowout = rowout.data_ptr(); a.ldro = rowout.stride(0)
-        a.n_rows = n; a.alpha = float(ctx.alpha); a.geom = geom.struct()
-        gx_geom, gr_geom = Geometry(H, Fp), Geometry(H, Rp)
-        dXc = torch.empty(graph.n_cols, gx_geom.Wd, **f32)
-        dRc = torch.empty(graph.n_rel, gr_geom.Wd, **f32)
-        split = AGG_BWD_MODE == "split" and graph.t2 is None and Fp == Rp
+    dZ = torch.empty(n, H * LZ, **f32)
+    dWa = torch.empty_like(Wa)
+    for h in range(H):
+        dh = dhn[:, h * D:(h + 1) * D]
+        gemm_nn(dh, Wa[h].t().contiguous(), out=dZ[:, h * LZ:(h + 1) * LZ])
+        if ghost is None:
+            gemm_tn(Z[:, h * LZ:(h + 1) * LZ], dh, out=dWa[h])
+        else:
+            gemm_tn(Z[:n_loc, h * LZ:(h + 1) * LZ], dh[:n_loc], out=dWa[h])
+            gemm_tn((Z[n_loc:, h * LZ:(h + 1) * LZ] * ghost.mine.unsqueeze(1)).contiguous(), dh[n_loc:], out=dWa[h],
+                    accumulate=True)
+    Gx = torch.empty(n, _row_stride(H * Fp, GX_ALIGN), **f32)[:, :H * Fp]
+    Gr = torch.empty(n, _row_stride(H * Rp, GX_ALIGN), **f32)[:, :H * Rp]
+    rowout = torch.empty(n, Fp + 4, **f32)
+    a = _lib.AggBwdArgs()
+    a.xrow = Xt.data_ptr(); a.ldxr = Xt.stride(0)
+    a.dz = dZ.data_ptr(); a.ldz = dZ.stride(0)
+    a.den = den.data_ptr(); a.sw = sw.data_ptr(); a.dden = dden.data_ptr()
+    a.gx = Gx.data_ptr(); a.ldgx = Gx.stride(0); a.gr = Gr.data_ptr(); a.ldgr = Gr.stride(0)
+    a.rowout = rowout.data_ptr(); a.ldro = rowout.stride(0)
+    a.n_rows = n; a.alpha = float(ctx.alpha); a.geom = geom.struct()
+    gx_geom, gr_geom = Geometry(H, Fp), Geometry(H, Rp)
+    dXc = torch.empty(graph.n_cols, gx_geom.Wd, **f32)
+    dRc = torch.empty(graph.n_rel, gr_geom.Wd, **f32)
+    split = AGG_BWD_MODE == "split" and graph.t2 is None and Fp == Rp
+    if split:
+        rowsc = torch.empty(max(1, n), H, 4, **f32)
+        a.rowsc = rowsc.data_ptr()
+        _lib.check(lib.spk_agg_bwd_ctx(C.byref(a), _lib.stream_ptr()), "agg_bwd_ctx")
+        del dZ
+        ne = max(1, graph.n_edges)
+        q = _lib.EdgeBwdSplitArgs()
+        b = q.base
+        b.rowptr = graph.rowptr.data_ptr()
+        b.colptr = graph.colptr.data_ptr(); b.csc_row = graph.csc_row.data_ptr(); b.csc_pos = graph.csc_pos.data_ptr()
+        b.csc_t1 = graph.csc_t1.data_ptr()
+        b.P1 = Xc.data_ptr(); b.ld1 = Xc.stride(0)
+        b.P2 = Xc.data_ptr(); b.ld2 = Xc.stride(0); b.P3 = Rt.data_ptr(); b.ld3 = Rt.stride(0)
+        if ctx.mask_csr is not None:
+            b.mask = ctx.mask_csr.data_ptr(); b.mask_stride = ctx.mask_csr.stride(0)
+        b.G = Gx.data_ptr(); b.ldg = Gx.stride(0); b.rowsc = rowsc.data_ptr()
+        b.dP1 = dXc.data_ptr(); b.ldd1 = dXc.stride(0)
+        b.dP2 = dXc.data_ptr(); b.ldd2 = dXc.stride(0)
+        b.n_rows = n; b.n_cols = graph.n_cols; b.apply_elu = 0; b.alpha = float(ctx.alpha)
+        b.geom = gx_geom.struct()
+        graph.row_hubs.fill(b.row_hub, None, 0)
+        partc = _hub_partial(graph.col_hubs, gx_geom.Wd, dev)
+        graph.col_hubs.fill(b.col_hub, partc, gx_geom.Wd)
+        q.relptr = graph.relptr.data_ptr(); q.rel_row = graph.rel_row.data_ptr(); q.rel_pos = graph.rel_pos.data_ptr()
+        rec4 = torch.empty(ne, H, 4, **f32); dsv = torch.empty(ne, H, **f32)
+        q.rec4 = rec4.data_ptr(); q.dsv = dsv.data_ptr()
+        q.dP3 = dRc.data_ptr(); q.ldd3 = dRc.stride(0); q.n_rel = graph.n_rel
+        part3 = _hub_partial(graph.rel_hubs, gr_geom.Wd, dev)
+        graph.rel_hubs.fill(q.rel_hub, part3, gr_geom.Wd)
+        part1 = _hub_partial(graph.row_hubs, 4, dev)
+        graph.row_hubs.fill(q.base.row_hub, part1, 4)
+        rowsum = torch.empty(max(1, n), H, **f32)
+        q.rowsum = rowsum.data_ptr(); q.ld_rowsum = H
+        q.G_rel = Gr.data_ptr(); q.ldg_rel = Gr.stride(0)
+        q.dup = 1
+
+        def run(phases, tag):
+            q.phases = phases
+            _lib.current_tag = tag + f":w{gx_geom.Wd}"
+            try:
+                _lib.check(lib.spk_edge_attn_bwd_split(C.byref(q), _lib.stream_ptr()), "edge_attn_bwd_split")
+            finally:
+                _lib.current_tag = ""
+    else:
+        rec = torch.empty(max(1, graph.n_edges), 2 * H, **f32)
+        a.segptr = graph.rowptr.data_ptr(); a.col = graph.col.data_ptr(); a.t1 = graph.t1.data_ptr()
+        a.t2 = graph.t2.data_ptr() if graph.t2 is not None else None
+        a.xcol = Xc.data_ptr(); a.ldxc = Xc.stride(0)
+        a.rel = Rt.data_ptr(); a.ldr = Rt.stride(0)
+        if ctx.mask_csr is not None:
+            a.mask = ctx.mask_csr.data_ptr(); a.mask_stride = ctx.mask_csr.stride(0)
+        rowsc = torch.empty(max(1, n), 8, **f32)
+        a.rowsc = rowsc.data_ptr(); a.rec = rec.data_ptr()
+        part = _hub_partial(graph.row_hubs, 8, dev)
+        graph.row_hubs.fill(a.hub, part, 8)
+        _lib.check(lib.spk_agg_bwd_rows(C.byref(a), _lib.stream_ptr()), "agg_bwd_rows")
+        del dZ
+    if split:
+        run(2, "cols")
+    else:
+        seg_gather(graph.colptr, graph.csc_row, graph.csc_pos, graph.col_hubs, Gx, Gx.stride(0), rec, gx_geom, dXc,
+                   graph.n_cols, "cols")
+    if dist is not None:
+        dXc_all = dXc
+        dXc_pad = torch.empty(dist.part.max_rows, gx_geom.Wd, **f32)
+        hx = dist.reduce_scatter_start(dXc_all, dXc_pad)
+    if split:
+        run(4, "rels")
+        rowout[:, Fp:Fp + H] = rowsum[:n]
+        if dist is not None:
+            colsum = torch.empty(graph.n_cols, H, **f32)
+            q.colsum = colsum.data_ptr(); q.ld_colsum = H
+        run(8, "colsums")
+        if dist is not None:
+            qs_pad = torch.empty(dist.part.max_rows, H, **f32)
+            hq = dist.reduce_scatter_start(colsum, qs_pad)
+    else:
+        seg_gather(graph.relptr, graph.rel_row, graph.rel_pos, graph.rel_hubs, Gr, Gr.stride(0), rec, gr_geom, dRc,
+                   graph.n_rel, "rels")
+    if dist is not None:
+        dist.all_reduce(dRc)
+        dist.all_reduce(dWa)
+        if ghost is not None:
+            gsum = ghost.sum_partials(rowout[n_loc:].contiguous())
+            rowout[ghost.mine_local] = gsum[ghost.mine]
+        hx.wait()
+        dXc = dXc_pad[:n_loc]
+        del dXc_all
         if split:
-            rowsc = torch.empty(max(1, n), H, 4, **f32)
-            a.rowsc = rowsc.data_ptr()
-            _lib.check(lib.spk_agg_bwd_ctx(C.byref(a), _lib.stream_ptr()), "agg_bwd_ctx")
-            del dZ
-            ne = max(1, graph.n_edges)
-            q = _lib.EdgeBwdSplitArgs()
-            b = q.base
-            b.rowptr = graph.rowptr.data_ptr()
-            b.colptr = graph.colptr.data_ptr(); b.csc_row = graph.csc_row.data_ptr(); b.csc_pos = graph.csc_pos.data_ptr()
-            b.csc_t1 = graph.csc_t1.data_ptr()
-            b.P1 = Xc.data_ptr(); b.ld1 = Xc.stride(0)
-            b.P2 = Xc.data_ptr(); b.ld2 = Xc.stride(0); b.P3 = Rt.data_ptr(); b.ld3 = Rt.stride(0)
-            if ctx.mask_csr is not None:
-                b.mask = ctx.mask_csr.data_ptr(); b.mask_stride = ctx.mask_csr.stride(0)
-            b.G = Gx.data_ptr(); b.ldg = Gx.stride(0); b.rowsc = rowsc.data_ptr()
-            b.dP1 = dXc.data_ptr(); b.ldd1 = dXc.stride(0)
-            b.dP2 = dXc.data_ptr(); b.ldd2 = dXc.stride(0)
-            b.n_rows = n; b.n_cols = graph.n_cols; b.apply_elu = 0; b.alpha = float(ctx.alpha)
-            b.geom = gx_geom.struct()
-            graph.row_hubs.fill(b.row_hub, None, 0)
-            partc = _hub_partial(graph.col_hubs, gx_geom.Wd, dev)
-            graph.col_hubs.fill(b.col_hub, partc, gx_geom.Wd)
-            q.relptr = graph.relptr.data_ptr(); q.rel_row = graph.rel_row.data_ptr(); q.rel_pos = graph.rel_pos.data_ptr()
-            rec4 = torch.empty(ne, H, 4, **f32); dsv = torch.empty(ne, H, **f32)
-            q.rec4 = rec4.data_ptr(); q.dsv = dsv.data_ptr()
-            q.dP3 = dRc.data_ptr(); q.ldd3 = dRc.stride(0); q.n_rel = graph.n_rel
-            part3 = _hub_partial(graph.rel_hubs, gr_geom.Wd, dev)
-            graph.rel_hubs.fill(q.rel_hub, part3, gr_geom.Wd)
-            part1 = _hub_partial(graph.row_hubs, 4, dev)
-            graph.row_hubs.fill(q.base.row_hub, part1, 4)
-            rowsum = torch.empty(max(1, n), H, **f32)
-            q.rowsum = rowsum.data_ptr(); q.ld_rowsum = H
-            q.G_rel = Gr.data_ptr(); q.ldg_rel = Gr.stride(0)
-            q.dup = 1
-
-            def run(phases, tag):
-                q.phases = phases
-                _lib.current_tag = tag + f":w{gx_geom.Wd}"
-                try:
-                    _lib.check(lib.spk_edge_attn_bwd_split(C.byref(q), _lib.stream_ptr()), "edge_attn_bwd_split")
-                finally:
-                    _lib.current_tag = ""
-        else:
-            rec = torch.empty(max(1, graph.n_edges), 2 * H, **f32)
-            a.segptr = graph.rowptr.data_ptr(); a.col = graph.col.data_ptr(); a.t1 = graph.t1.data_ptr()
-            a.t2 = graph.t2.data_ptr() if graph.t2 is not None else None
-            a.xcol = Xc.data_ptr(); a.ldxc = Xc.stride(0)
-            a.rel = Rt.data_ptr(); a.ldr = Rt.stride(0)
-            if ctx.mask_csr is not None:
-                a.mask = ctx.mask_csr.data_ptr(); a.mask_stride = ctx.mask_csr.stride(0)
-            rowsc = torch.empty(max(1, n), 8, **f32)
-            a.rowsc = rowsc.data_ptr(); a.rec = rec.data_ptr()
-            part = _hub_partial(graph.row_hubs, 8, dev)
-            graph.row_hubs.fill(a.hub, part, 8)
-            _lib.check(lib.spk_agg_bwd_rows(C.byref(a), _lib.stream_ptr()), "agg_bwd_rows")
-            del dZ
-        if split:
-            run(2, "cols")
-        else:
-            seg_gather(graph.colptr, graph.csc_row, graph.csc_pos, graph.col_hubs, Gx, Gx.stride(0), rec, gx_geom, dXc,
-                       graph.n_cols, "cols")
-        if dist is not None:
-            dXc_all = dXc
-            dXc_pad = torch.empty(dist.part.max_rows, gx_geom.Wd, **f32)
-            hx = dist.reduce_scatter_start(dXc_all, dXc_pad)
-        if split:
-            run(4, "rels")
-            rowout[:, Fp:Fp + H] = rowsum[:n]
-            if dist is not None:
-                colsum = torch.empty(graph.n_cols, H, **f32)
-                q.colsum = colsum.data_ptr(); q.ld_colsum = H
-            run(8, "colsums")
-            if dist is not None:
-                qs_pad = torch.empty(dist.part.max_rows, H, **f32)
-                hq = dist.reduce_scatter_start(colsum, qs_pad)
-        else:
-            seg_gather(graph.relptr, graph.rel_row, graph.rel_pos, graph.rel_hubs, Gr, Gr.stride(0), rec, gr_geom, dRc,
-                       graph.n_rel, "rels")
-        if dist is not None:
-            dist.all_reduce(dRc)
-            dist.all_reduce(dWa)
-            if ghost is not None:
-                gsum = ghost.sum_partials(rowout[n_loc:].contiguous())
-                rowout[ghost.mine_local] = gsum[ghost.mine]
-            hx.wait()
-            dXc = dXc_pad[:n_loc]
-            del dXc_all
-            if split:
-                hq.wait()
-                dXc[:, H * Fp:H * Fp + H].copy_(qs_pad[:n_loc])
-        n = n_loc
-        dX = torch.empty(n, geom.F, **f32)
-        dq = torch.empty(n, 4, **f32)
-        _lib.check(lib.spk_agg_dx(_lib.ptr(rowout), rowout.stride(0), _lib.ptr(dXc), dXc.stride(0), _lib.ptr(V), n,
-                                  geom.F, geom.Fx4, H, _lib.ptr(dX), dX.stride(0), _lib.ptr(dq), _lib.stream_ptr()),
-                   "agg_dx")
-        dV = gemm_tn(Xt[:n, :geom.F], dq) if ctx.needs_input_grad[3] else None
-        if dV is not None and dist is not None:
-            dist.all_reduce(dV)
-        dq3 = dRc[:, H * Rp:H * Rp + H].contiguous()
-        dRel = None
-        if ctx.needs_input_grad[1]:
-            dRel = dRc[:, :geom.Rd].clone()
-            for h in range(1, H):
-                dRel += dRc[:, h * Rp:h * Rp + geom.Rd]
-            dRel = gemm_nn(dq3, V3[:, :H].t().contiguous(), out=dRel, accumulate=True)
-        dV3 = None
-        if ctx.needs_input_grad[4]:
-            dV3 = torch.zeros_like(V3)
-            dV3[:, :H] = gemm_tn(Rel, dq3)
-        return dX, dRel, dWa, dV, dV3, None, None, None, None, None, None
-
-
-def attention_group(X, Rel, a_list, a2_list, graph, alpha, apply_elu, mask_csr, nanflag):
-    outs = []
+            hq.wait()
+            dXc[:, H * Fp:H * Fp + H].copy_(qs_pad[:n_loc])
+    n = n_loc
+    dX = torch.empty(n, geom.F, **f32)
+    dq = torch.empty(n, 4, **f32)
+    _lib.check(lib.spk_agg_dx(_lib.ptr(rowout), rowout.stride(0), _lib.ptr(dXc), dXc.stride(0), _lib.ptr(V), n,
+                              geom.F, geom.Fx4, H, _lib.ptr(dX), dX.stride(0), _lib.ptr(dq), _lib.stream_ptr()),
+               "agg_dx")
+    dV = gemm_tn(Xt[:n, :geom.F], dq) if ctx.needs_input_grad[3] else None
+    if dV is not None and dist is not None:
+        dist.all_reduce(dV)
+    dq3 = dRc[:, H * Rp:H * Rp + H].contiguous()
+    dRel = None
+    if ctx.needs_input_grad[1]:
+        dRel = dRc[:, :geom.Rd].clone()
+        for h in range(1, H):
+            dRel += dRc[:, h * Rp:h * Rp + geom.Rd]
+        dRel = gemm_nn(dq3, V3[:, :H].t().contiguous(), out=dRel, accumulate=True)
+    dV3 = None
+    if ctx.needs_input_grad[4]:
+        dV3 = torch.zeros_like(V3)
+        dV3[:, :H] = gemm_tn(Rel, dq3)
+    return dX, dRel, dWa, dV, dV3, None, None, None, None, None, None
+
+
+def _check_tables(X, Rel, graph):
     if X.shape[0] != graph.n_nodes - getattr(graph, "n_ghost", 0):
         raise IndexError(f"entity table has {X.shape[0]} rows but the graph was built for "
                          f"{graph.n_nodes - getattr(graph, 'n_ghost', 0)} nodes")
@@ -859,6 +869,11 @@
         raise IndexError(f"relation table has {Rel.shape[0]} rows but the graph uses {graph.n_rel} relations")
     if X.device != graph.device or Rel.device != graph.device:
         raise RuntimeError(f"tables on {X.device} / {Rel.device} but the graph layouts live on {graph.device}")
+
+
+def attention_group(X, Rel, a_list, a2_list, graph, alpha, apply_elu, mask_csr, nanflag):
+    outs = []
+    _check_tables(X, Rel, graph)
     F = X.shape[1]
     D = a_list[0].shape[0]
     Rd = a_list[0].shape[1] - 2 * F
@@ -880,6 +895,88 @@
     return outs[0] if len(outs) == 1 else torch.cat(outs, dim=1)
 
 
+class _FnCtx:
+
+    def __init__(self):
+        self.saved_tensors = ()
+        self.needs_input_grad = ()
+
+    def save_for_backward(self, *tensors):
+        self.saved_tensors = tensors
+
+    def mark_non_differentiable(self, *tensors):
+        pass
+
+
+class AggAttentionFn(torch.autograd.Function):
+
+    @staticmethod
+    def forward(ctx, X, Rel, Wa, V, V3, Wn, Rel2, Wr, graph, geom1, geom2, alpha, m1, m2, nanflag):
+        c1, c2 = _FnCtx(), _FnCtx()
+        x1 = AggGroupFn.forward(c1, X, Rel, Wa, V, V3, graph, geom1, alpha, True, m1, nanflag)
+        x2, _, _ = AttentionGroupFn.forward(c2, x1, Wn, Rel2, Wr, graph, geom2, alpha, True, m2, nanflag)
+        ctx.layers = (c1, c2)
+        return x2
+
+    @staticmethod
+    def backward(ctx, dout):
+        c1, c2 = ctx.layers
+        need = ctx.needs_input_grad
+        c1.needs_input_grad = need[:5]
+        c2.needs_input_grad = (any(need[:5]),) + need[5:8]
+        pre = []
+
+        def project_dx(dP, WnT):
+            out1, den1 = c1.saved_tensors[8], c1.saved_tensors[9]
+            geom = c1.geom
+            M, K = dP.shape
+            N = WnT.shape[1]
+            dhn = torch.empty(M, N, dtype=torch.float32, device=dP.device)
+            dden = torch.empty(M, geom.H, dtype=torch.float32, device=dP.device)
+            lib = _lib.load()
+            if lib.timing is not None:
+                _lib.current_tag = f"{M}x{K}x{N}"
+            ws = torch.empty(lib.spk_gemm_tc_workspace_floats(N, K), dtype=torch.float32, device=dP.device)
+            _lib.check(lib.spk_gemm_nn_tc_aggpre(_lib.ptr(dP), dP.stride(0), _lib.ptr(WnT), WnT.stride(0), _lib.ptr(dhn),
+                                                 dhn.stride(0), M, N, K, _lib.ptr(out1), out1.stride(0), _lib.ptr(den1),
+                                                 geom.H, geom.D, 1, _lib.ptr(dden), _lib.ptr(ws), _lib.stream_ptr()),
+                       "gemm_nn_tc_aggpre")
+            pre.append((dhn, dden))
+            return None
+
+        _, dWn, dRel2, dWr = _attention_backward(c2, dout, project_dx)[:4]
+        dX, dRel, dWa, dV, dV3 = _agg_backward(c1, None, pre[0])[:5] if pre else (None,) * 5
+        return (dX, dRel, dWa, dV, dV3, dWn, dRel2, dWr) + (None,) * 7
+
+
+def _agg_attention_fusable(X, l1, l2, graph):
+    if not (ROW_EPILOGUES and USE_TC and getattr(graph, "dist", None) is None and X.shape[0] >= TC_MIN_ROWS):
+        return False
+    a1, a2 = l1[0], l2[0]
+    F, D1 = X.shape[1], a1[0].shape[0]
+    Rd = a1[0].shape[1] - 2 * F
+    H1 = len(a1)
+    return (H1 <= AGG_MAX_HEADS and use_agg_path(H1, F, Rd, D1, graph) and H1 * D1 <= 256 and D1 % 4 == 0
+            and len(a2) <= MAX_HEADS)
+
+
+def attention_layers(X, Rel, W, l1, l2, graph, alpha, m_att, m_out, nanflag):
+    Rel2 = matmul(Rel, W)
+    if not _agg_attention_fusable(X, l1, l2, graph):
+        x = attention_group(X, Rel, l1[0], l1[1], graph, alpha, True, m_att, nanflag)
+        return attention_group(x, Rel2, l2[0], l2[1], graph, alpha, True, m_out, nanflag), Rel2
+    _check_tables(X, Rel, graph)
+    F, D1, H1 = X.shape[1], l1[0][0].shape[0], len(l1[0])
+    geom1 = AggGeometry(H1, F, l1[0][0].shape[1] - 2 * F, D1)
+    Wa, V, V3 = agg_weights(l1[0], l1[1], geom1)
+    geom2 = Geometry(len(l2[0]), l2[0][0].shape[0])
+    Wn, Wr = extended_weights(l2[0], l2[1], H1 * D1, geom2)
+    m1 = None if m_att is None else m_att.contiguous()
+    m2 = None if m_out is None else m_out.contiguous()
+    x = AggAttentionFn.apply(X, Rel, Wa, V, V3, Wn, Rel2, Wr, graph, geom1, geom2, alpha, m1, m2, nanflag)
+    return x, Rel2
+
+
 
 def rownorm_(x):
     assert x.dim() == 2 and x.stride(1) == 1
@@ -929,16 +1026,69 @@
 
     @staticmethod
     def backward(ctx, g):
-        out, mask, inv = ctx.saved_tensors
-        g = g.contiguous()
-        n, w = out.shape
-        dew = torch.empty_like(out)
-        dx2 = torch.empty_like(out)
-        _lib.check(_lib.load().spk_residual_norm_bwd(_lib.ptr(g), g.stride(0), _lib.ptr(out), out.stride(0),
-                                                     _lib.ptr(mask), _lib.ptr(inv), _lib.ptr(dew), dew.stride(0),
-                                                     _lib.ptr(dx2), dx2.stride(0), n, w, _lib.stream_ptr()),
-                   "residual_norm_bwd")
-        return dew, dx2, None
+        return _residual_norm_bwd(g, *ctx.saved_tensors) + (None,)
+
+
+def _residual_norm_bwd(g, out, mask, inv):
+    g = g.contiguous()
+    n, w = out.shape
+    dew = torch.empty_like(out)
+    dx2 = torch.empty_like(out)
+    _lib.check(_lib.load().spk_residual_norm_bwd(_lib.ptr(g), g.stride(0), _lib.ptr(out), out.stride(0),
+                                                 _lib.ptr(mask), _lib.ptr(inv), _lib.ptr(dew), dew.stride(0),
+                                                 _lib.ptr(dx2), dx2.stride(0), n, w, _lib.stream_ptr()),
+               "residual_norm_bwd")
+    return dew, dx2
+
+
+ROW_EPILOGUES = True
+
+
+def _resnorm_fusable(X, W, x2):
+    M, N = X.shape[0], W.shape[1]
+    return (USE_TC and M >= TC_MIN_ROWS and X.shape[1] >= 1 and 1 <= N <= 256 and N % 4 == 0 and x2.stride(0) % 4 == 0
+            and x2.data_ptr() % 16 == 0
+            and _lib.load().spk_gemm_nn_tc_supported(_lib.ptr(X), X.stride(0), M, N, X.shape[1]))
+
+
+class ProjResidualNormFn(torch.autograd.Function):
+
+    @staticmethod
+    def forward(ctx, X, W, x2, mask):
+        X = _tma_operand(X); W = W.contiguous(); x2 = x2.contiguous()
+        M, K = X.shape
+        N = W.shape[1]
+        out = torch.empty(M, N, dtype=torch.float32, device=X.device)
+        inv = torch.empty(M, dtype=torch.float32, device=X.device)
+        lib = _lib.load()
+        if _resnorm_fusable(X, W, x2):
+            if lib.timing is not None:
+                _lib.current_tag = f"{M}x{K}x{N}"
+            ws = torch.empty(lib.spk_gemm_tc_workspace_floats(N, K), dtype=torch.float32, device=X.device)
+            _lib.check(lib.spk_gemm_nn_tc_resnorm(_lib.ptr(X), X.stride(0), _lib.ptr(W), W.stride(0), _lib.ptr(out),
+                                                  out.stride(0), M, N, K, _lib.ptr(x2), x2.stride(0), _lib.ptr(mask),
+                                                  _lib.ptr(inv), _lib.ptr(ws), _lib.stream_ptr()), "gemm_nn_tc_resnorm")
+        else:
+            EW = gemm_nn(X, W)
+            _lib.check(lib.spk_residual_norm_fwd(_lib.ptr(EW), EW.stride(0), _lib.ptr(x2), x2.stride(0), _lib.ptr(mask),
+                                                 _lib.ptr(out), out.stride(0), _lib.ptr(inv), M, N, _lib.stream_ptr()),
+                       "residual_norm_fwd")
+        ctx.save_for_backward(X, W, out, mask, inv)
+        return out
+
+    @staticmethod
+    def backward(ctx, g):
+        X, W, out, mask, inv = ctx.saved_tensors
+        dew, dx2 = _residual_norm_bwd(g, out, mask, inv)
+        dX = gemm_nn(dew, W.t().contiguous()) if ctx.needs_input_grad[0] else None
+        dW = gemm_tn(X, dew) if ctx.needs_input_grad[1] else None
+        return dX, dW, dx2, None
+
+
+def proj_residual_norm(X, W, x2, mask, dist=None):
+    if ROW_EPILOGUES and dist is None:
+        return ProjResidualNormFn.apply(X, W, x2, mask)
+    return ResidualNormFn.apply(matmul(X, W, dist), x2, mask)
 
 
 
diff --git a/recon_b200/models.py b/recon_b200/models.py
--- a/recon_b200/models.py
+++ b/recon_b200/models.py
@@ -71,13 +71,16 @@
             m_out = edge_dropout_mask(p, 1, e, dev)
             m_x = (torch.rand(x.shape[0], nheads * self.attentions[0].out_features, device=dev) >= p).float().mul_(1.0 / (1.0 - p))
 
-        x = SF.attention_group(x, relation_embed, [att.a for att in self.attentions],
-                               [att.a_2 for att in self.attentions], graph, self.alpha, True, m_att, nanflag)
-        if m_x is not None:
+        l1 = ([att.a for att in self.attentions], [att.a_2 for att in self.attentions])
+        l2 = ([self.out_att.a], [self.out_att.a_2])
+        if m_x is None:
+            x, out_relation_1 = SF.attention_layers(x, relation_embed, self.W, l1, l2, graph, self.alpha, m_att, m_out,
+                                                    nanflag)
+        else:
+            x = SF.attention_group(x, relation_embed, l1[0], l1[1], graph, self.alpha, True, m_att, nanflag)
             x = x * m_x
-        out_relation_1 = SF.matmul(relation_embed, self.W)
-        x = SF.attention_group(x, out_relation_1, [self.out_att.a], [self.out_att.a_2], graph, self.alpha,
-                               True, m_out, nanflag)
+            out_relation_1 = SF.matmul(relation_embed, self.W)
+            x = SF.attention_group(x, out_relation_1, l2[0], l2[1], graph, self.alpha, True, m_out, nanflag)
         if own_flag:
             check_nanflag(nanflag)
         return x, out_relation_1
@@ -168,8 +171,10 @@
             graph=graph, dropout_masks=dropout_masks, nanflag=nanflag)
         mask = SF.mask_from_index(torch.as_tensor(batch_entities), entity_embeddings.shape[0], dev, flag=nanflag)
         if entities_upgraded is None:
-            entities_upgraded = SF.matmul(entity_embeddings, self.W_entities, getattr(graph, "dist", None))
-        out_entity_1 = SF.ResidualNormFn.apply(entities_upgraded, out_entity_1, mask)
+            out_entity_1 = SF.proj_residual_norm(entity_embeddings, self.W_entities, out_entity_1, mask,
+                                                 getattr(graph, "dist", None))
+        else:
+            out_entity_1 = SF.ResidualNormFn.apply(entities_upgraded, out_entity_1, mask)
         check_nanflag(nanflag)
         return out_entity_1, out_relation_1, mask
 
```

Result: slower. 461.0 million (median of 6 runs) (-7.0%).
